# kwea123/nsff_pl

Hardware: AMD Instinct MI355X
Metric: ray-samples/sec (coarse+fine, static+dynamic) (higher is better)
Workload: dtype f16x3 (fp32 operands split into 2 halfs, 3 f16 MFMAs per product, fp32 accumulate; same 1e-4 parity as f32); 1 GPU; C2 (BASELINE.json configs[1]): static+dynamic NSFF, 1024 rays/GPU x (64 coarse + 64 importance -> 192 fine pts), train-mode fwd, fw/bw flow warp t+-1, perturb=1 noise_std=1, 8x256 MLPs, N_tau=48, all 47 outputs on device.  `value` is render_rays' throughput with autograd DISABLED (the train-mode FLAGS, inference launches: nothing kept for a backward pass); what a trainer's forward costs is aux.tra; rays_per_gpu=1024, N_samples=64, N_importance=64, parallelism=single GPU, field_launch=persistent (one workgroup per CU)

## Files before the change

### include/nsff_render.h

```cpp
#ifndef NSFF_RENDER_H
#define NSFF_RENDER_H

#include <stddef.h>
#include <stdint.h>

#ifdef __cplusplus
extern "C" {
#endif

#define NSFF_OK               0
#define NSFF_ERR_INVALID     -1
#define NSFF_ERR_NULL        -2
#define NSFF_ERR_ALIGN       -3
#define NSFF_ERR_HIP         -4

#define NSFF_ABI_VERSION      32
#define NSFF_RAW_STRIDE      16
#define NSFF_MAX_FREQS       24
#define NSFF_MAX_LAYERS       8


typedef struct NsffModelDesc {
    int32_t D;
    int32_t W;
// ... 401 lines not shown
    int32_t col_a, col_b;
    int32_t pad_;
    const float* g_a[4];
    const float* g_b[4];
    float* out;
} NsffFlowGradArgs;
int nsff_flow_grad(const NsffFlowGradArgs* args, void* stream);

#define NSFF_RAY_RECORD      16

typedef struct NsffSsimArgs {
    int32_t n_frames, H, W, window;
    const float* gt;  const float* pred;  const uint8_t* mask;
    float* map;  float* mean_map;  double* sums;
    void* scratch;  int64_t scratch_bytes;
} NsffSsimArgs;
int64_t nsff_ssim_scratch_bytes(int32_t n_frames, int32_t H, int32_t W);
int nsff_ssim(const NsffSsimArgs* args, void* stream);

typedef struct NsffFrameFinishArgs {
    int32_t n_frames, H, W, pad_;
    const float* rgb;  const float* gt;  const uint8_t* valid;  const float* depth;  const uint8_t* lut;
    float* rgb_clipped;  uint8_t* rgb_u8;  double* sums;  float* depth_range;  uint8_t* depth_u8;  uint8_t* depth_rgb_u8;
    void* scratch;  int64_t scratch_bytes;
} NsffFrameFinishArgs;
int64_t nsff_frame_finish_scratch_bytes(int32_t n_frames, int32_t H, int32_t W);
int nsff_frame_finish(const NsffFrameFinishArgs* args, void* stream);

typedef struct NsffValPanelsArgs {
    int32_t n_frames, H, W, pad_;
    const float* gt;  const float* pred;  const float* depth;  const float* transient_alpha;  const float* static_rgb;
    const float* static_depth;  const float* mask;  const float* disp;  const float* ssim_loss;
    const uint8_t* lut_depth;  const uint8_t* lut_mask;
    float* ranges;  uint8_t* grid_u8;  uint8_t* rmse_u8;  uint8_t* ssim_u8;  uint8_t* rmse_blend_u8;  uint8_t* ssim_blend_u8;
    void* scratch;  int64_t scratch_bytes;
} NsffValPanelsArgs;
int64_t nsff_val_panels_scratch_bytes(int32_t n_frames, int32_t H, int32_t W);
int nsff_val_panels(const NsffValPanelsArgs* args, void* stream);

#define NSFF_FLOW_UNKNOWN    1e10f
typedef struct NsffFlowMapsArgs {
    int32_t n_frames, H, W, n_poses, max_t, share_gt_scale;
    float   fx, fy, cx, cy;
    const float* xyz[2];  const float* Ps;  const int32_t* ts;
    float* flow[2];  const float* gt[2];  const uint8_t* mask;
    double* epe_sums;  int64_t* epe_counts;  float* maxrad;  const float* scale;
    uint8_t* image[2];  uint8_t* gt_image[2];
    void* scratch;  int64_t scratch_bytes;
} NsffFlowMapsArgs;
int64_t nsff_flow_maps_scratch_bytes(int32_t n_frames, int32_t H, int32_t W);
int nsff_flow_maps(const NsffFlowMapsArgs* args, void* stream);

#define NSFF_TRACK_MAX_POINTS 0x7fffffffLL
typedef struct NsffTrackStepArgs {
    int64_t n_rows;
    int32_t pts_per_row, direction, max_t, n_poses, fixed_view, pad_;
    float   fx, fy, cx, cy;
    const float* raw;  const float* xyz_in;  const int32_t* t_in;  const uint8_t* alive_in;
    float* xyz_out;  int32_t* t_out;  uint8_t* alive_out;
    const float* Ps;  float* uv;  float* depth;
} NsffTrackStepArgs;
int nsff_track_step(const NsffTrackStepArgs* args, void* stream);

#define NSFF_TRACK_MAX_TRACKS (1 << 20)
#define NSFF_TRACK_MAX_STEPS  (1 << 11)
typedef struct NsffTrackDrawArgs {
    int32_t H, W, n_steps, n_tracks;
    const float* uv;  const uint8_t* ok;  const uint8_t* image;  const uint8_t* lut;  uint8_t* out;
    void* scratch;  int64_t scratch_bytes;
} NsffTrackDrawArgs;
int64_t nsff_track_draw_scratch_bytes(int32_t H, int32_t W);
int nsff_track_draw(const NsffTrackDrawArgs* args, void* stream);

int nsff_cdf(const float* weights, int64_t n_frames, int64_t n, double* cdf, void* stream);

typedef struct NsffRayDrawArgs {
    int64_t n_frames, n_pixels, frame, batch;
    const float* records;  const double* cdf;  const float* u;
    float* rays;  float* rgbs;  int64_t* ts;  int64_t* cam_ids;  float* disps;  float* rays_mask;  float* uv_fw;  float* uv_bw;
    int64_t* rand_idx;
} NsffRayDrawArgs;
int nsff_ray_draw(const NsffRayDrawArgs* args, void* stream);

int nsff_prof_enable(int on);
int nsff_prof_collect(int64_t* launches, double* total_ms, double* total_flops, double* executed_flops);
int nsff_prof_collect_clock(int64_t* launches, double* total_ms, double* total_flops, double* executed_flops,
                            double* shader_ticks, double* ticks_ms);

#define NSFF_KERNEL_F32       1
#define NSFF_KERNEL_H3_64     2
#define NSFF_KERNEL_H3_8WAVE  3
#define NSFF_KERNEL_H3A       4
#define NSFF_KERNEL_H3_SAVE   5
#define NSFF_KERNEL_H3A_TBIAS 7
#define NSFF_KERNEL_H3A_SAVE  9
#define NSFF_KERNEL_H3A_SIDE  8
int         nsff_last_field_kernel(void);
int         nsff_last_field_grid(void);
int         nsff_field_mfma_shape(const NsffModelDesc* desc, const NsffFieldArgs* args);
int         nsff_repack_field_weights(const NsffModelDesc* desc, const void* packed, void* repacked, void* stream);
int         nsff_field_query_repacked(const NsffModelDesc* desc, const void* packed, const void* repacked, const NsffFieldArgs* args,
                                      void* stream);
int         nsff_last_field_mfma_shape(void);
int         nsff_field_phase_program(const NsffModelDesc* desc, int static_mode, int transient_mode, int fold_t, uint32_t* steps,
                             int* n_steps, int* n_static_steps, uint32_t* phases_static, uint32_t* phases_dynamic, int* n_phases);

#define NSFF_PLAN_WORDS 12
#define NSFF_LAUNCH_SIDE_TILE      1
#define NSFF_LAUNCH_H3_64          2
#define NSFF_LAUNCH_H3_64_SAVE     3
#define NSFF_LAUNCH_H3_8WAVE       4
#define NSFF_LAUNCH_H3_8WAVE_SAVE  5
#define NSFF_LAUNCH_H3A            6
#define NSFF_LAUNCH_H3A_SAVE       7
int         nsff_field_launch_plan(const NsffModelDesc* desc, const NsffFieldArgs* args, int32_t n_cus, int32_t no_persist,
                                   int32_t* out, int32_t max_launches);

#define NSFF_RANGE_ACT     0x1u
#define NSFF_RANGE_SAVED   0x2u
#define NSFF_RANGE_PARAMS  0x4u
#define NSFF_RANGE_CODES   0x8u
int         nsff_range_flags(uint32_t* out, int32_t clear, void* stream);

#define NSFF_LPIPS_MIN_SIZE  31

typedef struct NsffLpipsWeights {
    const float* conv_w[5];  const float* conv_b[5];  const float* lin[5];
} NsffLpipsWeights;
int64_t nsff_lpips_packed_bytes(void);
int     nsff_lpips_pack(const NsffLpipsWeights* weights, float* packed, void* stream);

int     nsff_lpips_dims(int32_t H, int32_t W, int32_t* hw);

typedef struct NsffLpipsArgs {
    int32_t n_frames, H, W, normalize;
    const float* gt;  const float* pred;  const uint8_t* valid;
    const float* packed;
    float* map;  double* sums;
    void* workspace;  int64_t workspace_bytes;
} NsffLpipsArgs;
int64_t nsff_lpips_workspace_bytes(int32_t n_frames, int32_t H, int32_t W);
int     nsff_lpips(const NsffLpipsArgs* args, void* stream);

typedef struct NsffSceneScaleArgs {
    int32_t n_frames, n_points, H, W;
    int32_t disp_rank[2];
    const double* points;  const uint8_t* vis;  const double* w2c;  const float* K;  const float* disps;
    double* stats;  float* disp_os;  double* depth_os;  int32_t* pix;
    void* work;  int64_t work_bytes;
} NsffSceneScaleArgs;
int64_t nsff_scene_scale_work_bytes(int32_t n_frames, int32_t n_points, int32_t H, int32_t W);
int     nsff_scene_scale(const NsffSceneScaleArgs* args, void* stream);

int         nsff_abi_version(void);
const char* nsff_last_hip_error(void);

#ifdef __cplusplus
}
#endif
#endif
```

### nsff_pl_amd/_lib.py

```python
import ctypes as C
import os

import torch

_HERE = os.path.dirname(os.path.abspath(__file__))
LIB_PATH = os.environ.get("NSFF_LIB") or os.path.join(_HERE, "libnsff_hip.so")

RAW_STRIDE = 16
ABI_VERSION = 32
MAX_FREQS = 24

_ERR = {-1: "NSFF_ERR_INVALID (bad shape/flag/unsupported architecture)",
        -2: "NSFF_ERR_NULL (required pointer missing)",
        -3: "NSFF_ERR_ALIGN (pointer not 16-byte aligned)",
        -4: "NSFF_ERR_HIP",
        -5: "NSFF_ERR_UNSUPPORTED (a valid request outside what the kernels are built for)"}

_fp = C.c_void_p


class ModelDesc(C.Structure):
    _fields_ = [("D", C.c_int32), ("W", C.c_int32), ("skip", C.c_int32),
                ("in_xyz", C.c_int32), ("in_dir", C.c_int32), ("in_a", C.c_int32),
                ("in_t", C.c_int32), ("use_viewdir", C.c_int32),
                ("has_transient", C.c_int32), ("has_flow", C.c_int32),
                ("flow_scale", C.c_float), ("skip_mask", C.c_int32)]


class FieldArgs(C.Structure):
    _fields_ = [("n_points", C.c_int64), ("precision", C.c_int32), ("tile_points", C.c_int32),
                ("pts_per_ray", C.c_int32),
                ("static_mode", C.c_int32), ("transient_mode", C.c_int32),
                ("flow_heads", C.c_int32),
                ("xyz", _fp), ("n_freqs", C.c_int32), ("freqs", C.c_float * MAX_FREQS),
                ("dir_emb", _fp), ("a_emb", _fp), ("t_emb", _fp),
                ("x_emb", _fp), ("ld_emb", C.c_int32),
                ("off_xyz", C.c_int32), ("off_dir", C.c_int32), ("off_a", C.c_int32),
                ("off_t", C.c_int32), ("raw", _fp), ("save_acts", _fp), ("save_xin", _fp), ("save_masks", _fp),
                ("save_side", _fp), ("t_bias", _fp), ("t_bias_rows", C.c_int32), ("reserved0", C.c_int32),
                ("s_bias", _fp), ("s_bias_rows", C.c_int32), ("launch_form", C.c_int32), ("save_lo_delta", C.c_int64 * 3)]


class TimeBiasJob(C.Structure):
    _fields_ = [("desc", C.POINTER(ModelDesc)), ("w", _fp * 8), ("b", _fp * 8), ("t_rows", _fp), ("out", _fp),
                ("table", _fp), ("ts", _fp), ("n_table", C.c_int64), ("max_t", C.c_int64), ("delta", C.c_int32), ("pad_", C.c_int32),
                ("rows_out", _fp)]


MAX_TIME_BIAS_JOBS = 4


class RngJob(C.Structure):
    _fields_ = [("out", _fp), ("numel", C.c_int64), ("offset", C.c_uint64), ("kind", C.c_int32), ("grid", C.c_uint32)]


MAX_RNG_JOBS = 12


class RngCoarse(C.Structure):
    _fields_ = [("rays", _fp), ("z_lin", _fp), ("zs", _fp), ("xyz", _fp), ("n_samples", C.c_int32), ("perturb", C.c_float),
                ("job", C.c_int32), ("pad_", C.c_int32)]


_COMPOSITE_PTRS_IN = ["raw", "raw_fw", "raw_bw", "zs", "xyz", "xyz_fw", "xyz_bw",
                      "noise_static", "noise_transient", "noise_fw", "noise_bw", "visibility"]
_COMPOSITE_PTRS_OUT = ["static_rgbs", "transient_rgbs", "flows_fw", "flows_bw",
                       "static_sigmas", "transient_sigmas", "static_alphas", "transient_alphas",
                       "static_weights", "transient_weights", "weights",
                       "xyzs_fw_bw", "xyzs_bw_fw", "disoccs_fw", "disoccs_bw",
                       "depth", "rgb", "transient_alpha", "transient_rgb",
                       "static_only_rgb", "static_only_depth",
                       "xyz_exp", "flow_fw_exp", "flow_bw_exp", "xyz_fw_exp", "xyz_bw_exp",
                       "rgb_fw", "rgb_bw", "disocc_fw", "disocc_bw"]


class FrustumArgs(C.Structure):
    _fields_ = [("w2c", _fp), ("ts", _fp), ("K4", C.c_float * 4), ("n_cams", C.c_int32), ("n_frames", C.c_int32),
                ("H", C.c_int32), ("W", C.c_int32)]


class CompositeArgs(C.Structure):
    _fields_ = ([("n_rays", C.c_int64), ("n_samples", C.c_int32), ("has_transient", C.c_int32),
                 ("has_rgb", C.c_int32), ("flow_mode", C.c_int32), ("want_disocc", C.c_int32),
                 ("noise_std", C.c_float), ("z_far", C.c_float)]
                + [(n, _fp) for n in _COMPOSITE_PTRS_IN]
                + [(n, _fp) for n in _COMPOSITE_PTRS_OUT]
                + [("vis", FrustumArgs)])


_CBWD_IN = ["raw", "raw_fw", "raw_bw", "zs", "xyz", "f_fw", "f_bw", "noise_static", "noise_transient", "noise_fw", "noise_bw"]
_CBWD_G = ["g_static_sigmas", "g_transient_sigmas", "g_static_weights", "g_transient_weights", "g_weights", "g_depth",
           "g_rgb", "g_transient_alpha", "g_transient_rgb", "g_so_rgb", "g_so_depth", "g_xyz_exp", "g_flow_fw_exp",
           "g_flow_bw_exp", "g_rgb_fw", "g_rgb_bw"]
_CBWD_OUT = ["scratch", "d_raw", "d_raw_fw", "d_raw_bw", "d_f_fw", "d_f_bw"]


class CompositeBwdArgs(C.Structure):
    _fields_ = ([("n_rays", C.c_int64), ("n_samples", C.c_int32), ("has_transient", C.c_int32), ("flow_mode", C.c_int32),
                 ("noise_std", C.c_float)] + [(n, _fp) for n in _CBWD_IN + _CBWD_G + _CBWD_OUT])


class FieldBwdArgs(C.Structure):
    _fields_ = [("n_points", C.c_int64), ("static_mode", C.c_int32), ("transient_mode", C.c_int32),
                ("d_raw", _fp), ("raw", _fp), ("gmax", _fp), ("masks", _fp), ("dpre", _fp), ("dhead", _fp),
                ("d_xin", _fp), ("d_side", _fp), ("dpre_lo_delta", C.c_int64)]


class WgradJob(C.Structure):
    _fields_ = [("a", _fp), ("b", _fp), ("a_rows", C.c_int32), ("b_rows", C.c_int32), ("out_off", C.c_int64), ("trunk", C.c_int32),
                ("pad_", C.c_int32), ("a_lo_delta", C.c_int64), ("b_lo_delta", C.c_int64)]


class FoldGradArgs(C.Structure):
    _fields_ = [("n_rows", C.c_int32), ("pad_", C.c_int32), ("g", _fp), ("gb", _fp), ("w_final", _fp), ("b_final", _fp),
                ("w_head", _fp * 16), ("d_w_head", _fp * 16), ("d_b_head", _fp * 16), ("d_w_final", _fp), ("d_b_final", _fp)]


class FoldDenseArgs(C.Structure):
    _fields_ = [("n_rows", C.c_int32), ("accumulate", C.c_int32), ("ld_head", C.c_int32), ("ld_dhead", C.c_int32),
                ("g", _fp), ("g2", _fp), ("gb", _fp), ("gb2", _fp), ("w_head", _fp), ("w_final", _fp), ("b_final", _fp),
                ("d_w_head", _fp), ("d_b_head", _fp), ("d_w_final", _fp), ("d_b_final", _fp)]


class SplatArgs(C.Structure):
    _fields_ = [("H", C.c_int32), ("W", C.c_int32), ("n_planes", C.c_int32), ("K4", C.c_float * 4),
                ("P", C.c_float * 12), ("scale", C.c_float),
                ("xyz", _fp), ("flow", _fp), ("rgb", _fp), ("alpha", _fp), ("accum", _fp), ("work", _fp),
                ("work_bytes", C.c_int64)]


class MpiArgs(C.Structure):
    _fields_ = [("H", C.c_int32), ("W", C.c_int32), ("n_planes", C.c_int32), ("dt", C.c_float),
                ("accum_fw", _fp), ("accum_bw", _fp), ("static_rgb", _fp), ("static_alpha", _fp), ("zs", _fp),
                ("rgb", _fp), ("depth", _fp)]


_LOSS_IN = ["rgb_fine", "rgb_coarse", "depth_fine", "depth_coarse", "t_weights", "s_weights", "xyz_fw", "xyz_bw", "rgb_fw",
            "rgb_bw", "disocc_fw", "disocc_bw", "disoccs_fw", "disoccs_bw", "xyzs_fw_bw", "xyzs_bw_fw", "xyzs_fine",
            "xyzs_fw", "xyzs_bw", "rgbs", "disps", "ts", "cam_ids", "uv_fw", "uv_bw", "Ks", "Ps", "hyper", "stats", "terms",
            "term_w"]
LOSS_GRADS = ["g_rgb_fine", "g_rgb_coarse", "g_depth_fine", "g_depth_coarse", "g_t_weights", "g_s_weights", "g_xyz_fw",
              "g_xyz_bw", "g_rgb_fw", "g_rgb_bw", "g_xyzs_fw_bw", "g_xyzs_bw_fw", "g_xyzs_fw", "g_xyzs_bw"]


class LossArgs(C.Structure):
    _fields_ = ([("n_rays", C.c_int64), ("n_samples", C.c_int32), ("n_keep", C.c_int32), ("n_frames", C.c_int32),
                 ("max_t", C.c_int32), ("topk", C.c_double), ("thickness", C.c_int32), ("pad_", C.c_int32)]
                + [(n, _fp) for n in _LOSS_IN] + [("weights", _fp), ("per_ray", _fp), ("coef", _fp)]
                + [(n, _fp) for n in LOSS_GRADS])


class FlowGradArgs(C.Structure):
    _fields_ = [("n_points", C.c_int64), ("zs", _fp), ("z_far", C.c_float), ("accumulate", C.c_int32), ("col_a", C.c_int32),
                ("col_b", C.c_int32), ("pad_", C.c_int32), ("g_a", _fp * 4), ("g_b", _fp * 4), ("out", _fp)]


class SsimArgs(C.Structure):
    _fields_ = [("n_frames", C.c_int32), ("H", C.c_int32), ("W", C.c_int32), ("window", C.c_int32),
                ("gt", _fp), ("pred", _fp), ("mask", _fp), ("map", _fp), ("mean_map", _fp), ("sums", _fp),
                ("scratch", _fp), ("scratch_bytes", C.c_int64)]


class LpipsWeights(C.Structure):
    _fields_ = [("conv_w", _fp * 5), ("conv_b", _fp * 5), ("lin", _fp * 5)]


class LpipsArgs(C.Structure):
    _fields_ = [("n_frames", C.c_int32), ("H", C.c_int32), ("W", C.c_int32), ("normalize", C.c_int32),
                ("gt", _fp), ("pred", _fp), ("valid", _fp), ("packed", _fp), ("map", _fp), ("sums", _fp),
                ("workspace", _fp), ("workspace_bytes", C.c_int64)]


_FINISH_PTRS = ["rgb", "gt", "valid", "depth", "lut", "rgb_clipped", "rgb_u8", "sums", "depth_range", "depth_u8", "depth_rgb_u8"]


class FrameFinishArgs(C.Structure):
    _fields_ = ([("n_frames", C.c_int32), ("H", C.c_int32), ("W", C.c_int32), ("pad_", C.c_int32)]
                + [(n, _fp) for n in _FINISH_PTRS] + [("scratch", _fp), ("scratch_bytes", C.c_int64)])


_PANEL_IN = ["gt", "pred", "depth", "transient_alpha", "static_rgb", "static_depth", "mask", "disp", "ssim_loss"]
_PANEL_LUT = ["lut_depth", "lut_mask"]
_PANEL_OUT = ["ranges", "grid_u8", "rmse_u8", "ssim_u8", "rmse_blend_u8", "ssim_blend_u8"]
PANEL_FIELDS = ("depth", "static_depth", "neg_disp", "neg_rmse", "neg_ssim")


class ValPanelsArgs(C.Structure):
    _fields_ = ([("n_frames", C.c_int32), ("H", C.c_int32), ("W", C.c_int32), ("pad_", C.c_int32)]
                + [(n, _fp) for n in _PANEL_IN + _PANEL_LUT + _PANEL_OUT] + [("scratch", _fp), ("scratch_bytes", C.c_int64)])


FLOW_UNKNOWN = 1e10


class FlowMapsArgs(C.Structure):
    _fields_ = [("n_frames", C.c_int32), ("H", C.c_int32), ("W", C.c_int32), ("n_poses", C.c_int32), ("max_t", C.c_int32),
                ("share_gt_scale", C.c_int32), ("fx", C.c_float), ("fy", C.c_float), ("cx", C.c_float), ("cy", C.c_float),
                ("xyz", _fp * 2), ("Ps", _fp), ("ts", _fp), ("flow", _fp * 2), ("gt", _fp * 2), ("mask", _fp),
                ("epe_sums", _fp), ("epe_counts", _fp), ("maxrad", _fp), ("scale", _fp), ("image", _fp * 2), ("gt_image", _fp * 2),
                ("scratch", _fp), ("scratch_bytes", C.c_int64)]


TRACK_MAX_POINTS, TRACK_MAX_TRACKS, TRACK_MAX_STEPS = 0x7fffffff, 1 << 20, 1 << 11


class TrackStepArgs(C.Structure):
    _fields_ = [("n_rows", C.c_int64), ("pts_per_row", C.c_int32), ("direction", C.c_int32), ("max_t", C.c_int32),
                ("n_poses", C.c_int32), ("fixed_view", C.c_int32), ("pad_", C.c_int32),
                ("fx", C.c_float), ("fy", C.c_float), ("cx", C.c_float), ("cy", C.c_float),
                ("raw", _fp), ("xyz_in", _fp), ("t_in", _fp), ("alive_in", _fp), ("xyz_out", _fp), ("t_out", _fp), ("alive_out", _fp),
                ("Ps", _fp), ("uv", _fp), ("depth", _fp)]


class TrackDrawArgs(C.Structure):
    _fields_ = [("H", C.c_int32), ("W", C.c_int32), ("n_steps", C.c_int32), ("n_tracks", C.c_int32),
                ("uv", _fp), ("ok", _fp), ("image", _fp), ("lut", _fp), ("out", _fp), ("scratch", _fp), ("scratch_bytes", C.c_int64)]


RAY_RECORD = 16
_DRAW_OUT = ["rays", "rgbs", "ts", "cam_ids", "disps", "rays_mask", "uv_fw", "uv_bw", "rand_idx"]


class RayDrawArgs(C.Structure):
    _fields_ = ([("n_frames", C.c_int64), ("n_pixels", C.c_int64), ("frame", C.c_int64), ("batch", C.c_int64),
                 ("records", _fp), ("cdf", _fp), ("u", _fp)] + [(n, _fp) for n in _DRAW_OUT])


FRAME_TABLE = 16


class RayRecordArgs(C.Structure):
    _fields_ = [("n_frames", C.c_int32), ("H", C.c_int32), ("W", C.c_int32), ("first_frame", C.c_int32),
                ("frame_count", C.c_int32), ("image_u8", C.c_int32), ("mask_u8", C.c_int32),
                ("fx", C.c_float), ("fy", C.c_float), ("cx", C.c_float), ("cy", C.c_float), ("near", C.c_float),
                ("n_pixels", C.c_int64), ("images", _fp), ("disps", _fp), ("masks", _fp), ("flow_fw", _fp), ("flow_bw", _fp),
                ("frame_table", _fp), ("records", _fp)]


RESIZE_LANCZOS_U8, RESIZE_NEAREST_PIL, RESIZE_NEAREST_CV, RESIZE_LINEAR_CV = range(4)
RESIZE_MAX_KSIZE = 49
ERR_UNSUPPORTED = -5


class FrameResizeArgs(C.Structure):
    _fields_ = [("n_frames", C.c_int32), ("filter", C.c_int32), ("channels", C.c_int32), ("pad_", C.c_int32),
                ("src_h", C.c_int32), ("src_w", C.c_int32), ("dst_h", C.c_int32), ("dst_w", C.c_int32),
                ("ksize_x", C.c_int32), ("ksize_y", C.c_int32), ("ratio", C.c_float * 2), ("src", _fp), ("dst", _fp),
                ("x_start", _fp), ("x_count", _fp), ("x_weights", _fp), ("y_start", _fp), ("y_count", _fp), ("y_weights", _fp)]


class SceneScaleArgs(C.Structure):
    _fields_ = [("n_frames", C.c_int32), ("n_points", C.c_int32), ("H", C.c_int32), ("W", C.c_int32),
                ("disp_rank", C.c_int32 * 2), ("points", _fp), ("vis", _fp), ("w2c", _fp), ("K", _fp), ("disps", _fp),
                ("stats", _fp), ("disp_os", _fp), ("depth_os", _fp), ("pix", _fp), ("work", _fp), ("work_bytes", C.c_int64)]


_SIGNATURES = {
    "nsff_abi_version": (C.c_int, []),
    "nsff_range_flags": (C.c_int, [_fp, C.c_int32, _fp]),
    "nsff_last_field_kernel": (C.c_int, []),
    "nsff_last_field_grid": (C.c_int, []),
    "nsff_field_mfma_shape": (C.c_int, [C.POINTER(ModelDesc), C.POINTER(FieldArgs)]),
    "nsff_repack_field_weights": (C.c_int, [C.POINTER(ModelDesc), _fp, _fp, _fp]),
    "nsff_field_query_repacked": (C.c_int, [C.POINTER(ModelDesc), _fp, _fp, C.POINTER(FieldArgs), _fp]),
    "nsff_last_field_mfma_shape": (C.c_int, []),
    "nsff_field_phase_program": (C.c_int, [C.POINTER(ModelDesc), C.c_int, C.c_int, C.c_int, C.POINTER(C.c_uint32), C.POINTER(C.c_int),
                                   C.POINTER(C.c_int), C.POINTER(C.c_uint32), C.POINTER(C.c_uint32), C.POINTER(C.c_int)]),
    "nsff_field_launch_plan": (C.c_int, [C.POINTER(ModelDesc), C.POINTER(FieldArgs), C.c_int32, C.c_int32, C.POINTER(C.c_int32), C.c_int32]),
    "nsff_time_bias_rows": (C.c_int, [C.POINTER(ModelDesc)]),
    "nsff_time_bias": (C.c_int, [C.POINTER(TimeBiasJob), C.c_int32, C.c_int64, C.c_void_p]),
    "nsff_rng_draws": (C.c_int, [C.POINTER(RngJob), C.c_int32, C.c_uint64, C.c_void_p]),
    "nsff_rng_draws_coarse": (C.c_int, [C.POINTER(RngJob), C.c_int32, C.c_uint64, C.POINTER(RngCoarse), C.c_void_p]),
    "nsff_side_bias": (C.c_int, [C.POINTER(ModelDesc), _fp, _fp, _fp, _fp, C.c_int64, _fp, C.c_void_p]),
    "nsff_last_hip_error": (C.c_char_p, []),
    "nsff_packed_bytes": (C.c_int, [C.POINTER(ModelDesc), C.c_int, C.POINTER(C.c_size_t)]),
    "nsff_param_count": (C.c_int, [C.POINTER(ModelDesc)]),
    "nsff_pack_weights": (C.c_int, [C.POINTER(ModelDesc), C.c_int, C.POINTER(_fp), _fp, _fp]),
    "nsff_pack_weights_ex": (C.c_int, [C.POINTER(ModelDesc), C.c_int, C.POINTER(_fp), _fp, C.c_int32, _fp]),
    "nsff_fold_heads": (C.c_int, [C.POINTER(ModelDesc), C.c_int, C.POINTER(_fp), _fp, _fp]),
    "nsff_posenc": (C.c_int, [_fp, C.c_int64, C.POINTER(C.c_float), C.c_int, _fp, _fp]),
    "nsff_time_rows": (C.c_int, [_fp, C.c_int64, C.c_int32, _fp, C.c_int64, C.c_int64, _fp, _fp, _fp]),
    "nsff_time_rows_backward": (C.c_int, [_fp, _fp, _fp, _fp, C.c_int64, C.c_int64, C.c_int64, C.c_int32, _fp, _fp]),
    "nsff_field_query": (C.c_int, [C.POINTER(ModelDesc), _fp, C.POINTER(FieldArgs), _fp]),
    "nsff_coarse_samples": (C.c_int, [_fp, C.c_int64, _fp, C.c_int32, C.c_float, _fp, _fp, _fp, _fp]),
    "nsff_fine_samples": (C.c_int, [_fp, C.c_int64, _fp, _fp, C.c_int32, C.c_int32, _fp, _fp, _fp, _fp,
                                    C.c_int32, _fp, _fp, _fp, _fp, _fp]),
    "nsff_sample_pdf": (C.c_int, [_fp, _fp, C.c_int64, C.c_int32, _fp, C.c_int32, C.c_int32,
                                  C.c_float, _fp, _fp]),
    "nsff_warp_points": (C.c_int, [_fp, _fp, _fp, C.c_int64, C.c_float, _fp, _fp, _fp]),
    "nsff_composite": (C.c_int, [C.POINTER(CompositeArgs), _fp]),
    "nsff_frustum_visibility": (C.c_int, [C.POINTER(FrustumArgs), _fp, C.c_int64, _fp, _fp]),
    "nsff_frame_rays": (C.c_int, [C.POINTER(C.c_float), C.POINTER(C.c_float), C.c_int32, C.c_int32, C.c_float,
                                  C.c_float, C.c_int64, C.c_int64, _fp, _fp]),
    "nsff_ray_records": (C.c_int, [C.POINTER(RayRecordArgs), _fp]),
    "nsff_resize_ksize": (C.c_int, [C.c_int32, C.c_int32, C.c_int32]),
    "nsff_resize_table": (C.c_int, [C.c_int32, C.c_int32, C.c_int32, C.c_void_p, C.c_void_p, C.c_void_p]),
    "nsff_frame_resize": (C.c_int, [C.POINTER(FrameResizeArgs), _fp]),
    "nsff_scene_scale_work_bytes": (C.c_int64, [C.c_int32, C.c_int32, C.c_int32, C.c_int32]),
    "nsff_scene_scale": (C.c_int, [C.POINTER(SceneScaleArgs), _fp]),
    "nsff_bwd_packed_bytes": (C.c_int, [C.POINTER(ModelDesc), C.POINTER(C.c_size_t)]),
    "nsff_pack_weights_bwd": (C.c_int, [C.POINTER(ModelDesc), C.POINTER(_fp), _fp, _fp]),
    "nsff_field_backward": (C.c_int, [C.POINTER(ModelDesc), _fp, C.POINTER(FieldBwdArgs), _fp]),
    "nsff_field_input_backward": (C.c_int, [_fp, C.c_int32, C.c_int32, _fp, C.c_int64, C.c_int32, C.POINTER(C.c_float), C.c_int32,
                                            C.c_int32, _fp, _fp, _fp]),
    "nsff_train_dims": (C.c_int, [C.POINTER(ModelDesc), C.POINTER(C.c_int32), C.POINTER(C.c_int32), C.POINTER(C.c_int32)]),
    "nsff_weight_grad_scratch": (C.c_int64, [C.POINTER(WgradJob), C.c_int32, C.c_int64, C.c_int32]),
    "nsff_weight_grad": (C.c_int, [C.POINTER(WgradJob), C.c_int32, C.c_int64, C.c_int32, _fp, _fp, _fp, _fp, _fp]),
    "nsff_weight_grad_accumulate": (C.c_int, [C.POINTER(WgradJob), C.c_int32, C.c_int64, C.c_int32, _fp, _fp, C.c_int64,
                                              _fp, _fp, _fp]),
    "nsff_weight_grad_accumulate_aux": (C.c_int, [C.POINTER(WgradJob), C.c_int32, C.c_int64, C.c_int32, _fp, _fp, C.c_int64,
                                                  _fp, _fp, _fp, _fp]),
    "nsff_absmax_raw": (C.c_int, [_fp, C.c_int64, _fp, _fp]),
    "nsff_last_bwd_kernel": (C.c_int, []),
    "nsff_last_bwd_grid": (C.c_int, []),
    "nsff_field_bwd_phase_program": (C.c_int, [C.POINTER(ModelDesc), C.c_int32, C.c_int32, C.c_int64, C.POINTER(C.c_uint32), C.c_int32,
                                                C.POINTER(C.c_uint32), C.c_int32]),
    "nsff_field_bwd_launch_plan": (C.c_int, [C.POINTER(ModelDesc), C.POINTER(FieldBwdArgs), C.c_int32, C.c_int32, C.c_int32,
                                             C.POINTER(C.c_int32), C.c_int32]),
    "nsff_fold_grads": (C.c_int, [C.POINTER(FoldGradArgs), _fp]),
    "nsff_fold_grads_dense": (C.c_int, [C.POINTER(FoldDenseArgs), _fp]),
    "nsff_pack_weights_bwd_ex": (C.c_int, [C.POINTER(ModelDesc), C.POINTER(_fp), _fp, _fp, _fp]),
    "nsff_absmax": (C.c_int, [_fp, C.c_int64, _fp, _fp]),
    "nsff_adam_step": (C.c_int, [_fp, _fp, _fp, _fp, C.c_int64, _fp, _fp, C.c_double, C.c_double, C.c_double, C.c_double, _fp]),
    "nsff_adam_step_segments": (C.c_int, [_fp, _fp, _fp, _fp, C.c_int64, _fp, _fp, C.c_double, C.c_double, C.c_double, C.c_double,
                                          _fp, C.c_int, _fp, _fp]),
    "nsff_sgd_step": (C.c_int, [_fp, _fp, _fp, C.c_int64, _fp, _fp, C.c_double, C.c_double, _fp, C.c_int, _fp, _fp]),
    "nsff_radam_step": (C.c_int, [_fp, _fp, _fp, _fp, C.c_int64, _fp, _fp, C.c_double, C.c_double, C.c_double, C.c_double,
                                  _fp, C.c_int, _fp, _fp]),
    "nsff_composite_backward": (C.c_int, [C.POINTER(CompositeBwdArgs), _fp]),
    "nsff_flow_grad": (C.c_int, [C.POINTER(FlowGradArgs), _fp]),
    "nsff_nerfw_loss": (C.c_int, [C.POINTER(LossArgs), C.c_int, _fp]),
    "nsff_nerfw_loss_work_bytes": (C.c_size_t, [C.c_longlong]),
    "nsff_nerfw_loss_ex": (C.c_int, [C.POINTER(LossArgs), C.c_int, _fp, C.c_size_t, _fp]),
    "nsff_last_loss_path": (C.c_int, []),
    "nsff_splat_planes": (C.c_int, [C.POINTER(SplatArgs), _fp]),
    "nsff_splat_work_bytes": (C.c_int64, [C.c_int32, C.c_int32, C.c_int32]),
    "nsff_mpi_composite": (C.c_int, [C.POINTER(MpiArgs), _fp]),
    "nsff_ssim_scratch_bytes": (C.c_int64, [C.c_int32, C.c_int32, C.c_int32]),
    "nsff_ssim": (C.c_int, [C.POINTER(SsimArgs), _fp]),
    "nsff_lpips_packed_bytes": (C.c_int64, []),
    "nsff_lpips_pack": (C.c_int, [C.POINTER(LpipsWeights), _fp, _fp]),
    "nsff_lpips_dims": (C.c_int, [C.c_int32, C.c_int32, C.POINTER(C.c_int32)]),
    "nsff_lpips_workspace_bytes": (C.c_int64, [C.c_int32, C.c_int32, C.c_int32]),
    "nsff_lpips": (C.c_int, [C.POINTER(LpipsArgs), _fp]),
    "nsff_frame_finish_scratch_bytes": (C.c_int64, [C.c_int32, C.c_int32, C.c_int32]),
    "nsff_frame_finish": (C.c_int, [C.POINTER(FrameFinishArgs), _fp]),
    "nsff_val_panels_scratch_bytes": (C.c_int64, [C.c_int32, C.c_int32, C.c_int32]),
    "nsff_val_panels": (C.c_int, [C.POINTER(ValPanelsArgs), _fp]),
    "nsff_flow_maps_scratch_bytes": (C.c_int64, [C.c_int32, C.c_int32, C.c_int32]),
    "nsff_flow_maps": (C.c_int, [C.POINTER(FlowMapsArgs), _fp]),
    "nsff_track_step": (C.c_int, [C.POINTER(TrackStepArgs), _fp]),
    "nsff_track_draw_scratch_bytes": (C.c_int64, [C.c_int32, C.c_int32]),
    "nsff_track_draw": (C.c_int, [C.POINTER(TrackDrawArgs), _fp]),
    "nsff_cdf": (C.c_int, [_fp, C.c_int64, C.c_int64, _fp, _fp]),
    "nsff_ray_draw": (C.c_int, [C.POINTER(RayDrawArgs), _fp]),
    "nsff_prof_enable": (C.c_int, [C.c_int]),
    "nsff_prof_collect": (C.c_int, [C.POINTER(C.c_int64), C.POINTER(C.c_double), C.POINTER(C.c_double), C.POINTER(C.c_double)]),
    "nsff_prof_collect_clock": (C.c_int, [C.POINTER(C.c_int64)] + [C.POINTER(C.c_double)] * 5),
}
EXPORTED_SYMBOLS = tuple(_SIGNATURES)

_lib = None


def load():
    global _lib
    if _lib is None:
        if not os.path.exists(LIB_PATH):
            raise RuntimeError(
                f"{LIB_PATH} is missing: build it with `python -c 'import __graft_entry__ as g; g.build()'` "
                "(or `make -C nsff_pl_amd/csrc`).  There is no CPU fallback for the render path.")
        lib = C.CDLL(LIB_PATH)
        for name, (res, args) in _SIGNATURES.items():
            fn = getattr(lib, name)
            fn.restype, fn.argtypes = res, args
        if lib.nsff_abi_version() != ABI_VERSION:
            raise RuntimeError("libnsff_hip.so ABI version mismatch")
        _lib = lib
    return _lib


def _check(rc, what):
    if rc != 0:
        msg = _ERR.get(rc, f"error {rc}")
        if rc == -4:
            msg += ": " + load().nsff_last_hip_error().decode()
        raise RuntimeError(f"{what} failed: {msg}")


def require_gpu_tensor(t, what):
    if not isinstance(t, torch.Tensor) or not t.is_cuda:
        raise RuntimeError(f"{what} must be a GPU tensor: the NSFF render path runs only on the "
                           "HIP kernels of libnsff_hip.so (no CPU fallback)")


def _ptr(t):
    if t is None:
        return None
    assert t.is_cuda and t.dtype == torch.float32 and t.is_contiguous(), "need contiguous fp32 GPU tensor"
    return t.data_ptr()


def _stream():
    return torch.cuda.current_stream().cuda_stream


def model_desc(model):
    if model.W != 256:
        raise RuntimeError(f"unsupported NeRF architecture: W={model.W} (the gfx950 field kernels tile W=256 trunks "
                           "into 4 x 64-neuron wave blocks; other widths are not built)")
    skips = sorted(set(int(s) for s in model.skips))
    if not 2 <= model.D <= 8 or any(not 1 <= s < model.D for s in skips):
        raise RuntimeError(f"unsupported NeRF architecture: D={model.D}, skips={list(model.skips)} (need 2 <= D <= 8 "
                           "and every skip layer in 1..D-1; a skip at layer 0 would concatenate the input with itself)")
    mask = sum(1 << s for s in skips)
    return ModelDesc(D=model.D, W=model.W, skip=skips[0] if len(skips) == 1 else 0, skip_mask=mask if len(skips) != 1 else 0,
                     in_xyz=model.in_channels_xyz,
                     in_dir=model.in_channels_dir,
                     in_a=model.in_channels_a if model.use_viewdir else 0,
                     in_t=model.in_channels_t, use_viewdir=int(model.use_viewdir),
                     has_transient=int(model.encode_transient),
                     has_flow=int(getattr(model, "has_flow_heads", hasattr(model, "transient_flow_fw"))),
                     flow_scale=float(getattr(model, "flow_scale", 0.0)))


def param_list(model):
    def lin(m):
        layer = m[0] if isinstance(m, torch.nn.Sequential) else m
        return [layer.weight, layer.bias]
    out = []
    for i in range(model.D):
        out += lin(getattr(model, f"static_xyz_encoding_{i + 1}"))
    out += lin(model.static_xyz_encoding_final)
    if model.use_viewdir:
        out += lin(model.static_dir_encoding)
    out += lin(model.static_sigma) + lin(model.static_rgb)
    if model.encode_transient:
        for i in range(model.D):
            out += lin(getattr(model, f"transient_xyz_encoding_{i + 1}"))
        out += lin(model.transient_xyz_encoding_final)
        out += lin(model.transient_sigma) + lin(model.transient_rgb)
        if hasattr(model, "transient_flow_fw"):
            out += lin(model.transient_flow_fw) + lin(model.transient_flow_bw)
    return out


def packed_bytes(desc, precision=0):
    n = C.c_size_t(0)
    _check(load().nsff_packed_bytes(C.byref(desc), int(precision), C.byref(n)), "nsff_packed_bytes")
    return n.value


PACK_SKIP_FOLD = 1


def pack_weights(desc, params, packed, precision=0, fold=True):
    lib = load()
    if lib.nsff_param_count(C.byref(desc)) != len(params):
        raise RuntimeError("parameter list does not match the model description")
    keep = [p.detach().contiguous().float() for p in params]
    for p in keep:
        require_gpu_tensor(p, "model parameter")
    arr = (_fp * len(keep))(*[p.data_ptr() for p in keep])
    _check(lib.nsff_pack_weights_ex(C.byref(desc), int(precision), arr, _ptr(packed), 0 if fold else PACK_SKIP_FOLD,
                                    _stream()), "nsff_pack_weights_ex")
    return keep


def fold_heads(desc, params, packed, precision):
    keep = [p.detach().contiguous().float() for p in params]
    arr = (_fp * len(keep))(*[p.data_ptr() for p in keep])
    _check(load().nsff_fold_heads(C.byref(desc), int(precision), arr, _ptr(packed), _stream()), "nsff_fold_heads")
    return keep


def time_rows_backward(g_cur, g_next, g_prev, ts, max_t, n_table):
    gs = [None if g is None else g.contiguous() for g in (g_cur, g_next, g_prev)]
    width = next(g for g in gs if g is not None).shape[1]
    assert ts.dtype == torch.int64 and ts.is_cuda and ts.is_contiguous()
    d = torch.empty(int(n_table), width, device=ts.device)
    _check(load().nsff_time_rows_backward(_ptr(gs[0]), _ptr(gs[1]), _ptr(gs[2]), C.c_void_p(ts.data_ptr()), ts.shape[0],
                                          int(max_t), int(n_table), width, _ptr(d), _stream()), "nsff_time_rows_backward")
    return d


def time_rows(table, ts, max_t, want_next=True, want_prev=True):
    n, width = ts.shape[0], table.shape[1]
    if want_next and want_prev:
        both = torch.empty(2, n, width, device=table.device)
        nxt, prv = both[0], both[1]
    else:
        nxt = torch.empty(n, width, device=table.device) if want_next else None
        prv = torch.empty(n, width, device=table.device) if want_prev else None
    assert ts.dtype == torch.int64 and ts.is_cuda and ts.is_contiguous()
    _check(load().nsff_time_rows(_ptr(table), table.shape[0], width, C.c_void_p(ts.data_ptr()), n, int(max_t),
                                 _ptr(nxt), _ptr(prv), _stream()), "nsff_time_rows")
    return nxt, prv


def posenc(x, freqs, out):
    f = [float(v) for v in freqs]
    arr = (C.c_float * len(f))(*f)
    _check(load().nsff_posenc(_ptr(x), x.shape[0], arr, len(f), _ptr(out), _stream()), "nsff_posenc")


def field_query(model, raw, n_points, pts_per_ray, static_mode, transient_mode, flow_heads=0,
                xyz=None, freqs=None, dir_emb=None, a_emb=None, t_emb=None,
                x_emb=None, emb_offsets=(0, -1, -1, -1), save_acts=None, save_xin=None, save_masks=None, save_side=None,
                precision=None, t_bias=None, s_bias=None, save_lo=False):
    from . import config
    desc = model_desc(model)
    prec = config.precision_code(model) if precision is None else precision
    saves = not (save_acts is None and save_xin is None and save_masks is None and save_side is None)
    packed = model.packed(prec)
    a = FieldArgs()
    a.precision, a.tile_points = prec, config.get_tile_points()
    a.launch_form = 0 if config.get_persistent() else 1
    a.n_points, a.pts_per_ray = int(n_points), int(pts_per_ray)
    a.static_mode, a.transient_mode, a.flow_heads = int(static_mode), int(transient_mode), int(flow_heads)
    a.xyz = _ptr(xyz)
    if freqs is not None:
        f = [float(v) for v in freqs]
        if len(f) > MAX_FREQS:
            raise RuntimeError("too many embedding frequencies")
        a.n_freqs = len(f)
        for i, v in enumerate(f):
            a.freqs[i] = v
    a.dir_emb, a.a_emb, a.t_emb = _ptr(dir_emb), _ptr(a_emb), _ptr(t_emb)
    a.x_emb = _ptr(x_emb)
    a.ld_emb = int(x_emb.shape[1]) if x_emb is not None else 0
    a.off_xyz, a.off_dir, a.off_a, a.off_t = [int(v) for v in emb_offsets]
    a.raw = _ptr(raw)
    a.save_acts = None if save_acts is None else save_acts.data_ptr()
    a.save_xin = None if save_xin is None else save_xin.data_ptr()
    a.save_masks = None if save_masks is None else save_masks.data_ptr()
    a.save_side = None if save_side is None else save_side.data_ptr()
    if save_lo:
        for i, t in enumerate((save_acts, save_xin, save_side)):
            a.save_lo_delta[i] = 0 if t is None else lo_delta(t)
    if t_bias is not None:
        a.t_bias, a.t_bias_rows = _ptr(t_bias), int(t_bias.shape[1])
    if s_bias is not None:
        a.s_bias, a.s_bias_rows = _ptr(s_bias), int(s_bias.shape[1])
    if os.environ.get("NSFF_H3A_SHAPE") != "32" and prec == config.PRECISIONS["f16x3"] and not saves and \
            load().nsff_field_mfma_shape(C.byref(desc), C.byref(a)) == 16:
        _check(load().nsff_field_query_repacked(C.byref(desc), _ptr(packed), _ptr(model.packed(REPACKED)), C.byref(a), _stream()),
               "nsff_field_query_repacked")
        return
    _check(load().nsff_field_query(C.byref(desc), _ptr(packed), C.byref(a), _stream()), "nsff_field_query")


def lo_delta(t):
    n = t.numel()
    if t.untyped_storage().nbytes() < (t.storage_offset() + 2 * n) * t.element_size():
        raise RuntimeError("three-product backward: this buffer has no remainder plane behind it (field_grad.alloc_saves(..., x3=True))")
    return n


def side_bias(model, dir_rows, a_rows=None):
    from . import config
    desc = model_desc(model)
    n_rays = int(dir_rows.shape[0])
    assert dir_rows.shape == (n_rays, desc.in_dir) and (desc.in_a == 0 or (a_rows is not None and a_rows.shape == (n_rays, desc.in_a)))
    packed = model.packed(config.PRECISIONS["f16x3"])
    w = model.static_dir_encoding[0].weight.detach()
    out = torch.empty(n_rays, 1, 256, device=dir_rows.device, dtype=torch.float32)
    _check(load().nsff_side_bias(C.byref(desc), _ptr(packed), _ptr(w), _ptr(dir_rows), _ptr(a_rows) if desc.in_a > 0 else None,
                                 n_rays, _ptr(out), _stream()), "nsff_side_bias")
    return out


_DEVICE_RNG_GEOMETRY = {}


def fused_draws(plan, device, values=True, coarse=None):
    dev = torch.device(device)
    idx = dev.index if dev.index is not None else torch.cuda.current_device()
    if idx not in _DEVICE_RNG_GEOMETRY:
        p = torch.cuda.get_device_properties(idx)
        _DEVICE_RNG_GEOMETRY[idx] = p.multi_processor_count * (p.max_threads_per_multi_processor // 256)
    max_grid = _DEVICE_RNG_GEOMETRY[idx]
    gen = torch.cuda.default_generators[idx]
    seed, offset = gen.initial_seed(), gen.get_offset()
    wanted = values if isinstance(values, (list, tuple)) else [bool(values)] * len(plan)
    sizes = []
    for kind, shape in plan:
        n = 1
        for s in shape:
            n *= int(s)
        sizes.append(n)
    total = sum(n for n, w in zip(sizes, wanted) if w)
    buf = torch.empty(max(total, 1), device=dev, dtype=torch.float32)
    outs, jobs, at = [], [], 0
    for (kind, shape), numel, want in zip(plan, sizes, wanted):
        if numel == 0:
            outs.append(torch.empty(*shape, device=dev, dtype=torch.float32))
            continue
        grid = min(max_grid, (numel + 255) // 256)
        if coarse is not None and not outs and not want:
            jobs.append((None, numel, offset, 0, grid))
            outs.append(None)
        elif want:
            t = buf[at:at + numel].view(*shape)
            at += numel
            jobs.append((t, numel, offset, 1 if kind == "randn" else 0, grid))
            outs.append(t)
        else:
            outs.append(None)
        offset += ((numel - 1) // (1024 * grid) + 1) * 4
    hook = None
    if coarse is not None:
        rays, z_lin, perturb, zs, xyz = coarse
        assert plan and plan[0][0] == "rand" and tuple(plan[0][1]) == (rays.shape[0], z_lin.shape[0]) and perturb > 0
        if sizes[0]:
            hook = RngCoarse(_ptr(rays), _ptr(z_lin), _ptr(zs), _ptr(xyz), int(z_lin.shape[0]), float(perturb), 0, 0)
    for k in range(0, len(jobs), MAX_RNG_JOBS):
        part = jobs[k:k + MAX_RNG_JOBS]
        arr = (RngJob * len(part))()
        for j, (t, numel, off, kind, grid) in enumerate(part):
            arr[j].out, arr[j].numel, arr[j].offset, arr[j].kind, arr[j].grid = (None if t is None else t.data_ptr()), numel, off, kind, grid
        with torch.cuda.device(idx):
            _check(load().nsff_rng_draws_coarse(arr, len(part), seed, C.byref(hook) if (hook is not None and k == 0) else None, _stream()),
                   "nsff_rng_draws")
    gen.set_offset(offset)
    return outs


_FUSED_DRAWS_OK = {}


def fused_draws_match_torch(device):
    dev = torch.device(device)
    idx = dev.index if dev.index is not None else torch.cuda.current_device()
    if idx in _FUSED_DRAWS_OK:
        return _FUSED_DRAWS_OK[idx]
    if torch.cuda.is_current_stream_capturing():
        return False
    gen = torch.cuda.default_generators[idx]
    state = gen.get_state()
    ok = True
    try:
        plan = [("rand", (7, 64)), ("randn", (1031,)), ("rand", (3, 5, 2)), ("randn", (70000,)), ("rand", (300001,))]
        gen.manual_seed(0x5EED1234)
        gen.set_offset(8)
        mine = fused_draws(plan, torch.device("cuda", idx))
        end_mine = gen.get_offset()
        gen.manual_seed(0x5EED1234)
        gen.set_offset(8)
        with torch.cuda.device(idx):
            ref = [(torch.rand if k == "rand" else torch.randn)(*shape, device=torch.device("cuda", idx)) for k, shape in plan]
        end_ref = gen.get_offset()
        ok = end_mine == end_ref and all(torch.equal(a.view(torch.int32), b.view(torch.int32)) for a, b in zip(mine, ref))
    except Exception:
        ok = False
    finally:
        gen.set_state(state)
    if not ok:
        import warnings
        warnings.warn("nsff_pl_amd: the fused generator kernel (nsff_rng_draws) no longer reproduces torch.rand / torch.randn on "
                      f"cuda:{idx} (torch {torch.__version__}); render_rays draws with the torch calls instead (slower by ~1 %, same "
                      "numbers as the reference)")
    _FUSED_DRAWS_OK[idx] = ok
    return ok


def time_bias_rows(model):
    return load().nsff_time_bias_rows(C.byref(model_desc(model)))


def time_bias(jobs, index=None):
    assert 1 <= len(jobs) <= MAX_TIME_BIAS_JOBS
    arr = (TimeBiasJob * len(jobs))()
    keep, outs, per_model, pair = [], [], {}, None
    rows_of = {}
    if index is not None:
        table, ts, max_t = index
        assert ts.dtype == torch.int64 and ts.is_cuda and ts.is_contiguous() and ts.dim() == 1, "ts: one int64 frame index per ray"
        n_rays, width = int(ts.shape[0]), int(table.shape[1])
        deltas = sorted({int(d) for _, d in jobs})
        if 1 in deltas and -1 in deltas:
            both = torch.empty(2, n_rays, width, device=table.device, dtype=torch.float32)
            rows_of[1], rows_of[-1] = both[0], both[1]
        for d in deltas:
            if d not in rows_of:
                rows_of[d] = torch.empty(n_rays, width, device=table.device, dtype=torch.float32)
        written = set()
    else:
        n_rays = int(jobs[0][1].shape[0])
    for j, (model, t_rows) in enumerate(jobs):
        if id(model) not in per_model:
            desc = model_desc(model)
            lins = [getattr(model, f"transient_xyz_encoding_{l + 1}")[0] for l in [0] + sorted(set(int(v) for v in model.skips))]
            wb = [(m.weight.detach(), m.bias.detach()) for m in lins]
            for w, b in wb:
                _ptr(w), _ptr(b)
            per_model[id(model)] = (desc, C.pointer(desc), wb)
        desc, pdesc, wb = per_model[id(model)]
        if index is not None:
            delta, t_rows = int(t_rows), None
            assert width == desc.in_t
        else:
            assert t_rows.shape == (n_rays, desc.in_t)
        dev = wb[0][0].device
        if j + 1 < len(jobs) and jobs[j + 1][0] is model and pair is None:
            pair = torch.empty(2, n_rays, len(wb), 256, device=dev, dtype=torch.float32)
            out = pair[0]
        elif pair is not None:
            out, pair = pair[1], None
        else:
            out = torch.empty(n_rays, len(wb), 256, device=dev, dtype=torch.float32)
        arr[j].desc = pdesc
        for i, (w, b) in enumerate(wb):
            arr[j].w[i], arr[j].b[i] = w.data_ptr(), b.data_ptr()
        arr[j].t_rows, arr[j].out = _ptr(t_rows), _ptr(out)
        if index is not None:
            arr[j].table, arr[j].ts = _ptr(table), ts.data_ptr()
            arr[j].n_table, arr[j].max_t, arr[j].delta = int(table.shape[0]), int(max_t), delta
            if delta not in written:
                arr[j].rows_out = _ptr(rows_of[delta])
                written.add(delta)
        outs.append(out)
    keep.append(per_model)
    _check(load().nsff_time_bias(arr, len(jobs), n_rays, _stream()), "nsff_time_bias")
    return outs if index is None else (outs, rows_of)


def coarse_samples(rays, z_lin, perturb, perturb_rand, zs, xyz):
    _check(load().nsff_coarse_samples(_ptr(rays), rays.shape[0], _ptr(z_lin), z_lin.shape[0],
                                      float(perturb), _ptr(perturb_rand), _ptr(zs), _ptr(xyz), _stream()),
           "nsff_coarse_samples")


def fine_samples(rays, z_lin, zs_coarse, n_importance, w_static, w_transient, u_static, u_transient,
                 u_per_ray, samples_static, samples_transient, zs_fine, xyz_fine):
    _check(load().nsff_fine_samples(_ptr(rays), rays.shape[0], _ptr(z_lin), _ptr(zs_coarse),
                                    z_lin.shape[0], int(n_importance), _ptr(w_static), _ptr(w_transient),
                                    _ptr(u_static), _ptr(u_transient), int(u_per_ray),
                                    _ptr(samples_static), _ptr(samples_transient),
                                    _ptr(zs_fine), _ptr(xyz_fine), _stream()), "nsff_fine_samples")


def sample_pdf(bins, weights, u, u_per_ray, eps, samples):
    _check(load().nsff_sample_pdf(_ptr(bins), _ptr(weights), weights.shape[0], weights.shape[1],
                                  _ptr(u), samples.shape[1], int(u_per_ray), float(eps),
                                  _ptr(samples), _stream()), "nsff_sample_pdf")


def warp_points(raw, xyz, zs, z_far, xyz_fw, xyz_bw):
    _check(load().nsff_warp_points(_ptr(raw), _ptr(xyz), _ptr(zs), zs.numel(), float(z_far),
                                   _ptr(xyz_fw), _ptr(xyz_bw), _stream()), "nsff_warp_points")


def frustum_args(w2c, ts, K4, n_cams, n_frames, H, W):
    assert w2c.is_cuda and w2c.dtype == torch.float32 and w2c.is_contiguous() and w2c.shape == (n_cams * n_frames, 12)
    assert ts.is_cuda and ts.dtype == torch.int64 and ts.is_contiguous() and ts.numel() >= 1
    a = FrustumArgs(w2c=w2c.data_ptr(), ts=ts.data_ptr(), n_cams=int(n_cams), n_frames=int(n_frames), H=int(H), W=int(W))
    a.K4[:] = [float(v) for v in K4]
    a._keep = (w2c, ts)
    return a


def frustum_visibility(vis, xyz, out):
    _check(load().nsff_frustum_visibility(C.byref(vis), _ptr(xyz), xyz.shape[0], _ptr(out), _stream()),
           "nsff_frustum_visibility")


def composite(vis=None, **kw):
    a = CompositeArgs()
    for k, v in kw.items():
        if k in _COMPOSITE_PTRS_IN or k in _COMPOSITE_PTRS_OUT:
            setattr(a, k, _ptr(v))
        else:
            setattr(a, k, v)
    if vis is not None:
        a.vis = vis
    _check(load().nsff_composite(C.byref(a), _stream()), "nsff_composite")


def frame_rays(K4, c2w12, H, W, near, shift_near, first, count, rays):
    k = (C.c_float * 4)(*[float(v) for v in K4])
    m = (C.c_float * 12)(*[float(v) for v in c2w12])
    _check(load().nsff_frame_rays(k, m, int(H), int(W), float(near), float(shift_near), int(first), int(count),
                                  _ptr(rays), _stream()), "nsff_frame_rays")


REPACKED = 101


def repack_weights(desc, packed, repacked):
    _check(load().nsff_repack_field_weights(C.byref(desc), _ptr(packed), _ptr(repacked), _stream()), "nsff_repack_field_weights")


def last_field_mfma_shape():
    return int(load().nsff_last_field_mfma_shape())


BWD_PACK = 100


def bwd_packed_bytes(desc):
    n = C.c_size_t(0)
    _check(load().nsff_bwd_packed_bytes(C.byref(desc), C.byref(n)), "nsff_bwd_packed_bytes")
    return n.value


def pack_weights_bwd(desc, params, packed, fwd_packed=None):
    arr = (_fp * len(params))(*[p.data_ptr() for p in params])
    _check(load().nsff_pack_weights_bwd_ex(C.byref(desc), arr, _ptr(packed), _ptr(fwd_packed), _stream()), "nsff_pack_weights_bwd_ex")


def last_bwd_kernel():
    return {0: "c", 1: "h3b", 2: "c+h3b", 3: "x3"}[load().nsff_last_bwd_kernel()]


def last_bwd_grid():
    return load().nsff_last_bwd_grid()


PLAN_WORDS = 12


def field_launch_plan(desc, args, n_cus, no_persist=False):
    out = (C.c_int32 * (3 * PLAN_WORDS))()
    code = load().nsff_field_launch_plan(C.byref(desc), C.byref(args), int(n_cus), int(bool(no_persist)), out, 3)
    recs = [list(out[i * PLAN_WORDS:(i + 1) * PLAN_WORDS]) for i in range(3)]
    return code, [r for r in recs if r[0] != 0]


def field_bwd_launch_plan(desc, args, n_cus, kernel_override=None, persist=True):
    out = (C.c_int32 * (2 * PLAN_WORDS))()
    code = load().nsff_field_bwd_launch_plan(C.byref(desc), C.byref(args), int(n_cus), ord(kernel_override) if kernel_override else 0,
                                                      int(bool(persist)), out, 2)
    recs = [list(out[i * PLAN_WORDS:(i + 1) * PLAN_WORDS]) for i in range(2)]
    return code, [r for r in recs if r[0] != 0]


def field_bwd_phase_program(model, dynamic, want_xin, n_tiles, max_phases=32):
    import numpy as np
    desc = model_desc(model)
    out = (C.c_uint32 * (8 * max_phases))()
    segs = (C.c_uint32 * 48)()
    n = load().nsff_field_bwd_phase_program(C.byref(desc), 1 if dynamic else 0, 1 if want_xin else 0, int(n_tiles), out, max_phases, segs, 48)
    if n < 0:
        raise RuntimeError(f"nsff_field_bwd_phase_program failed ({n})")
    offs = np.array(list(segs), np.uint32)
    return (np.array(list(out), np.uint32).reshape(max_phases, 8)[:n] if n > 0 else None), offs


def field_backward(model, n_points, static, transient, d_raw, raw, gmax, masks, dpre, dhead, d_xin, d_side=None, x3=False):
    desc = model_desc(model)
    a = FieldBwdArgs(n_points=int(n_points), static_mode=2 if static else 0, transient_mode=2 if transient else 0,
                     d_raw=_ptr(d_raw), raw=_ptr(raw), gmax=_ptr(gmax), masks=masks.data_ptr(), dpre=dpre.data_ptr(),
                     dhead=dhead.data_ptr(), d_xin=_ptr(d_xin), d_side=_ptr(d_side), dpre_lo_delta=lo_delta(dpre) if x3 else 0)
    _check(load().nsff_field_backward(C.byref(desc), _ptr(model.packed(BWD_PACK)), C.byref(a), _stream()),
           "nsff_field_backward")


def train_dims(model):
    desc = model_desc(model)
    xr, t0, sr = C.c_int32(0), C.c_int32(0), C.c_int32(0)
    _check(load().nsff_train_dims(C.byref(desc), C.byref(xr), C.byref(t0), C.byref(sr)), "nsff_train_dims")
    return xr.value, t0.value, sr.value


def field_input_backward(d_xin, t_row0, xyz, pts_per_ray, freqs, in_t, want_xyz, want_t):
    P, xin_rows = d_xin.shape
    n_rays = P // pts_per_ray
    d_xyz = torch.empty(P, 3, device=d_xin.device) if want_xyz else None
    d_t = torch.empty(n_rays, in_t, device=d_xin.device) if want_t else None
    f = [float(v) for v in freqs]
    arr = (C.c_float * max(len(f), 1))(*f)
    _check(load().nsff_field_input_backward(_ptr(d_xin), int(xin_rows), int(t_row0), _ptr(xyz), n_rays, int(pts_per_ray), arr,
                                            len(f), int(in_t), _ptr(d_xyz), _ptr(d_t), _stream()), "nsff_field_input_backward")
    return d_xyz, d_t


def _wgrad_jobs(jobs, with_off):
# ... 569 lines not shown
```

### nsff_pl_amd/csrc/field_h3.hip

```cpp
#include <hip/hip_runtime.h>
#include <algorithm>
#include <cstdlib>
#include <vector>
#include "nsff_layout_h3.h"
#include "nsff_common.h"
#include "nsff_internal.h"

typedef float f32x16 __attribute__((ext_vector_type(16)));
typedef _Float16 h8 __attribute__((ext_vector_type(8)));
typedef _Float16 h4 __attribute__((ext_vector_type(4)));
typedef __fp16 h2 __attribute__((ext_vector_type(2)));
typedef _Float16 h2f __attribute__((ext_vector_type(2)));

#ifdef H3_TIMING
__device__ unsigned g_h3_timing[256 * 8 * 32 * 6 + 256 * 4 * 256];
#define H3A_TBASE (256 * 8 * 32 * 6)
__device__ unsigned long long g_h3_span[2] = {~0ull, 0ull};
#define H3_SPAN(k) do { if (lane == 0) { const unsigned long long t_ = __builtin_amdgcn_s_memtime(); \
    if (k) atomicMax(&g_h3_span[1], t_); else atomicMin(&g_h3_span[0], t_); } } while (0)
#define H3_STAMP(k) do { if (lane == 0 && blockIdx.x < 256 && i < 32) \
    g_h3_timing[((blockIdx.x * 8 + wave_id) * 32 + i) * 6 + (k)] = (unsigned)__builtin_amdgcn_s_memtime(); } while (0)
#define H3_HSTAMP(k) do { if (lane == 0 && blockIdx.x < 256) \
    g_h3_timing[((blockIdx.x * 8 + wave) * 32 + 30) * 6 + (k)] = (unsigned)__builtin_amdgcn_s_memtime(); } while (0)
#else
#define H3_STAMP(k) do {} while (0)
#define H3_SPAN(k) do {} while (0)
#define H3_HSTAMP(k) do {} while (0)
#endif

namespace {

#ifndef H3_SAVE_INTERLEAVE
#define H3_SAVE_INTERLEAVE 1
#endif
constexpr int LDH = 264;
__device__ __forceinline__ h8 lds_h8(const _Float16* p) { return *reinterpret_cast<const h8*>(p); }

struct H3Step {
    uint32_t w_off;
    uint32_t bias_off;
    uint16_t nks;
    uint8_t pre;
    uint8_t post;
    uint8_t head;
    uint8_t save;
    uint8_t pad[2];
};
enum { PRE_NONE = 0, PRE_INPUT = 1, PRE_INPUT_T = 2, PRE_SIDE = 3 };
enum { POST_NONE = 0, POST_RELU = 1, POST_LINEAR = 2 };
enum { HEAD_NONE = 0, HEAD_S_SIGMA = 1, HEAD_S_RGB = 2, HEAD_T = 3, HEAD_S_FOLD = 4, HEAD_T_FOLD = 5 };
constexpr int MAX_STEPS = 28;

struct H3KArgs {
    NsffLayoutH3 L;
    H3Step steps[MAX_STEPS];
    int n_steps;
    int n_static_steps;
    int split_trunks;
    long long grid_tiles;
    const uint32_t* packed;
    const float* xyz;
    const float* x_emb;
    const float* dir_emb;
    const float* a_emb;
    const float* t_emb;
    const float* t_bias;
    int tb_rows;
    const float* s_bias;
    int sb_rows;
    float* raw;
    long long lo_delta[3];
    _Float16* save_acts;
    _Float16* save_xin;
    unsigned long long* save_masks;
    _Float16* save_side;
    long long save_stride;
    int xin_rows, side_rows;
    long long n_tiles;
    long long n_points;
    int pts_per_ray;
    int static_mode, transient_mode;
    int D, skip;
    int in_xyz, in_dir, in_a, in_t;
    int use_viewdir;
    float flow_scale;
    int n_freqs;
    int octave_freqs;
    float freqs[NSFF_MAX_FREQS];
    int ld_emb, off_xyz, off_dir, off_a, off_t;
    unsigned long long* span;
    uint32_t* range;
};

struct SpanT { unsigned long long t, r; };
__device__ __forceinline__ SpanT span_begin(const unsigned long long* span) {
    SpanT s{0ull, 0ull};
#ifdef H3_TIMING
    s.t = __builtin_amdgcn_s_memtime();
#endif
    if (span != nullptr && (blockIdx.x & 15) == 0) { s.t = __builtin_amdgcn_s_memtime(); s.r = __builtin_amdgcn_s_memrealtime(); }
    return s;
}
__device__ __forceinline__ void span_end(unsigned long long* span, const SpanT& s0, unsigned tid) {
    if (span == nullptr || (blockIdx.x & 15) != 0 || tid != 0) return;
    const unsigned long long t = __builtin_amdgcn_s_memtime(), r = __builtin_amdgcn_s_memrealtime();
    atomicAdd(span, t - s0.t);
    atomicAdd(span + 1, r - s0.r);
}
__device__ __forceinline__ void span_end(unsigned long long* span, const SpanT& s0) { span_end(span, s0, threadIdx.x); }

#define MFMA_H(a, b, c) __builtin_amdgcn_mfma_f32_32x32x16_f16((a), (b), (c), 0, 0, 0)
#define H3_PIN() __builtin_amdgcn_sched_barrier(0)

__device__ __forceinline__ void split_store(_Float16* xh, _Float16* xl, int idx, float v, float& rm) {
    rm = nsff_absmax3(rm, v, v);
    const _Float16 hi = (_Float16)v;
    xh[idx] = hi;
    xl[idx] = (_Float16)(v - (float)hi);
}

template <int MTW> struct WFrag { h8 wh[MTW], wl[MTW]; };
template <int NT> struct XFrag { h8 xh[NT], xl[NT]; };
template <int MTW> struct WRing { WFrag<MTW> r[4]; };
template <int MTW> struct BiasRegs { float4 b[MTW][4]; };

template <int MTW>
__device__ __forceinline__ void load_w(WFrag<MTW>& f, const uint4* __restrict__& wp) {
    if constexpr (MTW == 2) {
        const uint4 a0 = wp[0], a1 = wp[64], a2 = wp[128], a3 = wp[192];
        wp += 256;
        f.wh[0] = __builtin_bit_cast(h8, a0); f.wl[0] = __builtin_bit_cast(h8, a1);
        f.wh[1] = __builtin_bit_cast(h8, a2); f.wl[1] = __builtin_bit_cast(h8, a3);
    } else {
        const uint4 a0 = wp[0], a1 = wp[64];
        wp += 256;
        f.wh[0] = __builtin_bit_cast(h8, a0); f.wl[0] = __builtin_bit_cast(h8, a1);
    }
}

template <int NT> struct BRows { const _Float16* h[NT]; const _Float16* l[NT]; };
template <int NT>
__device__ __forceinline__ BRows<NT> b_rows(const _Float16* bh, const _Float16* bl, int ld) {
    BRows<NT> b;
#pragma unroll
    for (int nt = 0; nt < NT; ++nt) { b.h[nt] = bh + nt * 32 * ld; b.l[nt] = bl + nt * 32 * ld; }
    return b;
}

template <int NT>
__device__ __forceinline__ void load_x(XFrag<NT>& f, const BRows<NT>& b, int ks) {
#pragma unroll
    for (int nt = 0; nt < NT; ++nt) {
        f.xh[nt] = lds_h8(b.h[nt] + ks * 16);
        f.xl[nt] = lds_h8(b.l[nt] + ks * 16);
    }
}

template <int MTW>
__device__ __forceinline__ const uint4* prefetch_w(WRing<MTW>& ring, const uint4* __restrict__ w) {
// ... 1538 lines not shown
            for (int i = 0; i < 2; ++i) {
                if (off[i] == NSFF_NONE) continue;
                if (nks[i] > REPACK_MAX_NKS || (nks[i] & 1)) { bad = true; continue; }
                ra.off[n] = off[i]; ra.nks[n] = nks[i];
                if (++n == REPACK_BATCH) flush();
            }
        }
    };
    trunk(L.st);
    if (desc->has_transient) trunk(L.tr);
    flush();
    return bad ? NSFF_ERR_INVALID : nsff_launch_status();
}

static int fold_args(const NsffModelDesc& d, const float* const* params, FoldArgs& fs, FoldArgs& ft, FoldArgs& fd) {
    int pi = 2 * d.D;
    fs = FoldArgs{}; ft = FoldArgs{}; fd = FoldArgs{};
    fs.ld_head = ft.ld_head = NSFF_W;
    fs.w_final = params[pi]; fs.b_final = params[pi + 1]; pi += 2;
    if (d.use_viewdir) {
        fd.w_final = fs.w_final; fd.b_final = fs.b_final; fd.plain_row = -1;
        fd.w_head[0] = params[pi]; fd.b_head[0] = params[pi + 1]; fd.row0[0] = 0; fd.nrows[0] = NSFF_W; fd.n_heads = 1;
        fd.ld_head = NSFF_W + d.in_dir + d.in_a;
        pi += 2;
    }
    fs.w_plain = params[pi]; fs.b_plain = params[pi + 1]; fs.plain_row = 3; pi += 2;
    fs.w_head[0] = params[pi]; fs.b_head[0] = params[pi + 1]; fs.row0[0] = 0; fs.nrows[0] = 3; fs.n_heads = 1; pi += 2;
    if (d.has_transient) {
        pi += 2 * d.D;
        ft.w_final = params[pi]; ft.b_final = params[pi + 1]; ft.plain_row = -1; pi += 2;
        ft.w_head[1] = params[pi]; ft.b_head[1] = params[pi + 1]; ft.row0[1] = 3; ft.nrows[1] = 1; pi += 2;
        ft.w_head[0] = params[pi]; ft.b_head[0] = params[pi + 1]; ft.row0[0] = 0; ft.nrows[0] = 3; pi += 2;
        ft.n_heads = 2;
        if (d.has_flow) {
            ft.w_head[2] = params[pi]; ft.b_head[2] = params[pi + 1]; ft.row0[2] = 4; ft.nrows[2] = 3; pi += 2;
            ft.w_head[3] = params[pi]; ft.b_head[3] = params[pi + 1]; ft.row0[3] = 7; ft.nrows[3] = 3; pi += 2;
            ft.n_heads = 4;
        }
    }
    return pi;
}

int nsff_fold_rows_f32(const NsffModelDesc* desc, const float* const* params, float* s_w, float* s_b, float* t_w, float* t_b,
                       hipStream_t st) {
    const NsffModelDesc& d = *desc;
    FoldArgs fs, ft, fd;
    const int pi = fold_args(d, params, fs, ft, fd);
    for (int i = 0; i < pi; ++i) if (!params[i]) return NSFF_ERR_NULL;
    if (!d.use_viewdir) {
        fs.out_w = s_w; fs.out_b = s_b;
        hipLaunchKernelGGL(nsff_fold_kernel_h3, dim3(4), dim3(256), 0, st, fs);
    }
    if (d.has_transient) {
        ft.out_w = t_w; ft.out_b = t_b;
        hipLaunchKernelGGL(nsff_fold_kernel_h3, dim3(d.has_flow ? 10 : 4), dim3(256), 0, st, ft);
    }
    return nsff_launch_status();
}

int nsff_h3_fold_heads(const NsffModelDesc* desc, const float* const* params, void* packed, hipStream_t st) {
    NsffLayoutH3 L;
    const int rc = nsff_make_layout_h3(*desc, L);
    if (rc) return rc;
    const NsffModelDesc& d = *desc;
    FoldArgs fs, ft, fd;
    const int pi = fold_args(d, params, fs, ft, fd);
    for (int i = 0; i < pi; ++i) if (!params[i]) return NSFF_ERR_NULL;
    uint32_t* pw = reinterpret_cast<uint32_t*>(packed);
    PackArgsH3 pf{};
    pf.dst = pw;
    pf.range = nsff_range_word(st);
    int nf = 0;
    auto fold = [&](FoldArgs& f, uint32_t scratch, uint32_t tile, uint32_t bias) {
        f.out_w = reinterpret_cast<float*>(pw + scratch); f.out_b = reinterpret_cast<float*>(pw + bias);
        hipLaunchKernelGGL(nsff_fold_kernel_h3, dim3(32), dim3(256), 0, st, f);
        pf.seg[nf++] = PackSegH3{f.out_w, tile, 2, NSFF_W, NSFF_W, 0, 0, 0, 0, 0, 0, 32};
    };
    if (!d.use_viewdir) fold(fs, L.fold_f32, L.s_fold_w, L.s_fold_b);
    if (d.has_transient) fold(ft, L.fold_f32 + 32 * NSFF_W, L.t_fold_w, L.t_fold_b);
    int max_threads = 8 * NSFF_W;
    if (d.use_viewdir) {
        fd.out_w = reinterpret_cast<float*>(pw + L.dir_fold_f32); fd.out_b = reinterpret_cast<float*>(pw + L.dir_b_fold);
        hipLaunchKernelGGL(nsff_fold_kernel_h3, dim3(NSFF_W), dim3(256), 0, st, fd);
        pf.seg[nf++] = PackSegH3{fd.out_w, L.dir_h_fold, 1, NSFF_W, NSFF_W, NSFF_W, 0, 0, 0, 0, 0, 0};
        max_threads = 64 * NSFF_W;
    }
    if (nf > 0) hipLaunchKernelGGL(nsff_pack_kernel_h3, dim3((max_threads + 255) / 256, nf), dim3(256), 0, st, pf);
    return nsff_launch_status();
}

static int h3_step_program(const NsffModelDesc& d, int static_mode, int transient_mode, bool fold, H3KArgs& k, bool side_fold = false) {
    int n = 0;
    auto push = [&](uint32_t w, uint32_t b, uint32_t kcols, int pre, int post, int head, int slot = -1) {
        H3Step& s = k.steps[n++];
        s.w_off = w; s.bias_off = b; s.nks = (uint16_t)(kcols / 16);
        s.pre = (uint8_t)pre; s.post = (uint8_t)post; s.head = (uint8_t)head;
        s.save = (uint8_t)(slot + 1);
    };
    auto trunk = [&](const NsffTrunkLayoutH3& T, int pre_kind, int last_head, int slot0) {
        for (int l = 0; l < d.D; ++l) {
            const int head = (l == d.D - 1) ? last_head : HEAD_NONE;
            if (l == 0) {
                push(T.seg_x[0], T.bias[0], T.k0, pre_kind, POST_RELU, HEAD_NONE, slot0);
            } else if ((nsff_skip_layers(&d) >> l) & 1u) {
                push(T.seg_h[l], T.bias[l], NSFF_W, PRE_NONE, POST_NONE, HEAD_NONE);
                push(T.seg_x[l], NSFF_NONE, T.k0, pre_kind, POST_RELU, head, slot0 + l);
            } else {
                push(T.seg_h[l], T.bias[l], NSFF_W, PRE_NONE, POST_RELU, head, slot0 + l);
            }
        }
    };
    if (static_mode == 2 && fold && !d.use_viewdir) {
        trunk(k.L.st, PRE_INPUT, HEAD_S_FOLD, 0);
    } else if (static_mode == 2 && fold && side_fold) {
        trunk(k.L.st, PRE_INPUT, HEAD_S_SIGMA, 0);
        push(k.L.dir_h_fold, k.L.dir_b_fold, NSFF_W, PRE_NONE, POST_RELU, HEAD_S_RGB, d.D);
    } else if (static_mode == 2 && fold) {
        trunk(k.L.st, PRE_INPUT, HEAD_S_SIGMA, 0);
        push(k.L.dir_h_fold, k.L.dir_b_fold, NSFF_W, PRE_NONE, POST_NONE, HEAD_NONE);
        push(k.L.dir_x, NSFF_NONE, k.L.side_k, PRE_SIDE, POST_RELU, HEAD_S_RGB, d.D);
    } else if (static_mode) {
        trunk(k.L.st, PRE_INPUT, HEAD_S_SIGMA, 0);
        if (static_mode == 2) {
            push(k.L.st.final_w, k.L.st.final_b, NSFF_W, PRE_NONE, POST_LINEAR, d.use_viewdir ? HEAD_NONE : HEAD_S_RGB, d.D);
            if (d.use_viewdir) {
                push(k.L.dir_h, k.L.dir_b, NSFF_W, PRE_NONE, POST_NONE, HEAD_NONE);
                push(k.L.dir_x, NSFF_NONE, k.L.side_k, PRE_SIDE, POST_RELU, HEAD_S_RGB, d.D);
            }
        }
    }
    k.n_static_steps = n;
    if (transient_mode && fold) {
        trunk(k.L.tr, PRE_INPUT_T, HEAD_T_FOLD, d.D + 1);
    } else if (transient_mode) {
        trunk(k.L.tr, PRE_INPUT_T, HEAD_NONE, d.D + 1);
        push(k.L.tr.final_w, k.L.tr.final_b, NSFF_W, PRE_NONE, POST_LINEAR, HEAD_T, 2 * d.D + 1);
    }
    if (n > MAX_STEPS) return NSFF_ERR_INVALID;
    k.n_steps = n;
    return NSFF_OK;
}

static bool h3a_make_persistent(H3APhase* ph) {
    int at = -1;
    for (int i = 1; i < H3A_MAX_PHASES && !(i > 1 && ph[i].d[0] == H3A_BODY_END); ++i)
        if (ph[i].d[0] == H3A_BODY_B16L) { if (at >= 0) return false; at = i; }
    if (at < 0) return false;
    ph[at].d[0] = H3A_BODY_B16LP;
    for (int j = 3; j < 8; ++j) ph[at].d[j] = ph[0].d[j];
    return true;
}

namespace {
struct TimeBiasJobK { const float* w[NSFF_MAX_LAYERS]; const float* b[NSFF_MAX_LAYERS]; int ld[NSFF_MAX_LAYERS];
                      const float* t_rows; float* out; int rows, in_xyz, in_t;
                      const float* table; const long long* ts; long long n_table, max_t; int delta; float* rows_out; };
struct TimeBiasArgs { TimeBiasJobK job[NSFF_MAX_TIME_BIAS_JOBS]; long long n_rays; };
constexpr int TB_RAYS = 16;
__global__ __launch_bounds__(256) void nsff_time_bias_kernel(const TimeBiasArgs a) {
    const TimeBiasJobK& j = a.job[blockIdx.z];
    const int i = blockIdx.y, n = threadIdx.x;
    if (i >= j.rows) return;
    const long long r0 = (long long)blockIdx.x * TB_RAYS;
    __shared__ __attribute__((aligned(16))) float st[TB_RAYS][64];
    __shared__ float sw[16][NSFF_W + 1];
    const float* __restrict__ wl = j.w[i] + j.in_xyz;
    const int ld = j.ld[i], in_t = j.in_t;
    float tv[TB_RAYS / 4], wv[4][16];
#pragma unroll
    for (int k = 0; k < TB_RAYS / 4; ++k) {
        const int e = threadIdx.x + 256 * k, r = e >> 6, c = e & 63;
        const long long ray = r0 + r < a.n_rays ? r0 + r : a.n_rays - 1;
        const float* row = j.t_rows != nullptr ? j.t_rows + ray * in_t : nullptr;
        if (row == nullptr) {
            long long t = j.ts[ray] + j.delta;
            if (j.delta > 0) t = t < j.max_t ? t : j.max_t;
            if (j.delta < 0) t = t > 0 ? t : 0;
            t = t < 0 ? 0 : (t > j.n_table - 1 ? j.n_table - 1 : t);
            row = j.table + t * in_t;
        }
        tv[k] = c < in_t ? row[c] : 0.f;
        if (j.rows_out != nullptr && i == 0 && c < in_t && r0 + r < a.n_rays) j.rows_out[(r0 + r) * in_t + c] = tv[k];
    }
    const float b = j.b[i][n];
#pragma unroll
    for (int q = 0; q < 4; ++q)
#pragma unroll
        for (int k = 0; k < 16; ++k) {
            const int e = threadIdx.x + 256 * k, row = e >> 4, c = 16 * q + (e & 15);
            wv[q][k] = c < in_t ? wl[row * ld + c] : 0.f;
        }
#pragma unroll
    for (int k = 0; k < TB_RAYS / 4; ++k) { const int e = threadIdx.x + 256 * k; st[e >> 6][e & 63] = tv[k]; }
    float acc[TB_RAYS];
#pragma unroll
    for (int r = 0; r < TB_RAYS; ++r) acc[r] = b;
#pragma unroll
    for (int q = 0; q < 4; ++q) {
        if (16 * q >= in_t) break;
        __syncthreads();
#pragma unroll
        for (int k = 0; k < 16; ++k) { const int e = threadIdx.x + 256 * k; sw[e & 15][e >> 4] = wv[q][k]; }
        __syncthreads();
#pragma unroll
        for (int u = 0; u < 16; u += 4) {
            const float w0 = sw[u][n], w1 = sw[u + 1][n], w2 = sw[u + 2][n], w3 = sw[u + 3][n];
#pragma unroll
            for (int r = 0; r < TB_RAYS; ++r) {
                const float4 t4 = *reinterpret_cast<const float4*>(&st[r][16 * q + u]);
                acc[r] = fmaf(w3, t4.w, fmaf(w2, t4.z, fmaf(w1, t4.y, fmaf(w0, t4.x, acc[r]))));
            }
        }
    }
#pragma unroll
    for (int r = 0; r < TB_RAYS; ++r)
        if (r0 + r < a.n_rays) j.out[((r0 + r) * j.rows + i) * NSFF_W + n] = acc[r];
}
}

extern "C" int nsff_time_bias_rows(const NsffModelDesc* desc) {
    if (!desc || !desc->has_transient || desc->in_t < 1) return 0;
    return 1 + __builtin_popcount(nsff_skip_layers(desc));
}

extern "C" int nsff_time_bias(const NsffTimeBiasJob* jobs, int32_t n_jobs, int64_t n_rays, void* stream) {
    if (!jobs) return NSFF_ERR_NULL;
    if (n_jobs < 1 || n_jobs > NSFF_MAX_TIME_BIAS_JOBS || n_rays < 0) return NSFF_ERR_INVALID;
    if (n_rays == 0) return NSFF_OK;
    TimeBiasArgs a{};
    a.n_rays = n_rays;
    int max_rows = 0;
    for (int q = 0; q < n_jobs; ++q) {
        const NsffTimeBiasJob& jb = jobs[q];
        if (!jb.desc || !jb.out) return NSFF_ERR_NULL;
        if (!jb.t_rows && (!jb.table || !jb.ts || jb.n_table < 1 || jb.delta < -1 || jb.delta > 1)) return NSFF_ERR_NULL;
        const NsffModelDesc& d = *jb.desc;
        NsffLayoutH3 L;
        const int rc = nsff_make_layout_h3(d, L);
        if (rc) return rc;
        TimeBiasJobK& k = a.job[q];
        k.rows = nsff_time_bias_rows(&d);
        if (k.rows < 1) return NSFF_ERR_INVALID;
        if (d.in_t > 64 || (d.in_t & 3) != 0) return NSFF_ERR_INVALID;
        k.in_xyz = d.in_xyz; k.in_t = d.in_t; k.t_rows = jb.t_rows; k.out = jb.out;
        k.table = jb.table; k.ts = reinterpret_cast<const long long*>(jb.ts); k.n_table = jb.n_table; k.max_t = jb.max_t;
        k.delta = jb.delta; k.rows_out = jb.t_rows ? nullptr : jb.rows_out;
        const uint32_t skips = nsff_skip_layers(&d);
        int i = 0;
        for (int l = 0; l < d.D; ++l) {
            if (l != 0 && !((skips >> l) & 1u)) continue;
            k.w[i] = jb.w[i]; k.b[i] = jb.b[i];
            if (!k.w[i] || !k.b[i]) return NSFF_ERR_NULL;
            k.ld[i] = d.in_xyz + d.in_t + (l ? NSFF_W : 0);
            ++i;
        }
        max_rows = std::max(max_rows, k.rows);
    }
    const long long gx = (n_rays + TB_RAYS - 1) / TB_RAYS;
    if (gx > 0x7fffffffLL) return NSFF_ERR_INVALID;
    hipLaunchKernelGGL(nsff_time_bias_kernel, dim3((unsigned)gx, (unsigned)max_rows, (unsigned)n_jobs), dim3(256), 0,
                       reinterpret_cast<hipStream_t>(stream), a);
    return nsff_launch_status();
}

namespace {
struct SideBiasArgs { const float* w; const float* b; const float* dir_rows; const float* a_rows; float* out;
                      int in_dir, in_a, ld; long long n_rays; };
__global__ __launch_bounds__(256) void nsff_side_bias_kernel(const SideBiasArgs a) {
    const int n = threadIdx.x;
    const long long r0 = (long long)blockIdx.x * TB_RAYS;
    const int in = a.in_dir + a.in_a;
    __shared__ __attribute__((aligned(16))) float st[TB_RAYS][NSFF_W];
    __shared__ float sw[16][NSFF_W + 1];
    for (int e = threadIdx.x; e < TB_RAYS * NSFF_W; e += 256) {
        const int r = e >> 8, c = e & 255;
        const long long ray = r0 + r < a.n_rays ? r0 + r : a.n_rays - 1;
        float v = 0.f;
        if (c < a.in_dir) v = a.dir_rows[ray * a.in_dir + c];
        else if (c < in) v = a.a_rows[ray * a.in_a + (c - a.in_dir)];
        st[r][c] = v;
    }
    float acc[TB_RAYS];
    const float b = a.b[n];
#pragma unroll
    for (int r = 0; r < TB_RAYS; ++r) acc[r] = b;
    const float* __restrict__ wl = a.w + NSFF_W;
    for (int c0 = 0; c0 < in; c0 += 16) {
        __syncthreads();
#pragma unroll
        for (int k = 0; k < 16; ++k) {
            const int e = threadIdx.x + 256 * k, row = e >> 4, c = c0 + (e & 15);
            sw[e & 15][row] = c < in ? wl[(long long)row * a.ld + c] : 0.f;
        }
        __syncthreads();
#pragma unroll
        for (int u = 0; u < 16; u += 4) {
            const float w0 = sw[u][n], w1 = sw[u + 1][n], w2 = sw[u + 2][n], w3 = sw[u + 3][n];
#pragma unroll
            for (int r = 0; r < TB_RAYS; ++r) {
                const float4 t4 = *reinterpret_cast<const float4*>(&st[r][c0 + u]);
                acc[r] = fmaf(w3, t4.w, fmaf(w2, t4.z, fmaf(w1, t4.y, fmaf(w0, t4.x, acc[r]))));
            }
        }
    }
#pragma unroll
    for (int r = 0; r < TB_RAYS; ++r)
        if (r0 + r < a.n_rays) a.out[(r0 + r) * NSFF_W + n] = acc[r];
}
}

extern "C" int nsff_side_bias(const NsffModelDesc* desc, const void* packed_f16x3, const float* w_dir, const float* dir_rows,
                              const float* a_rows, int64_t n_rays, float* out, void* stream) {
    if (!desc || !packed_f16x3 || !w_dir || !dir_rows || !out) return NSFF_ERR_NULL;
    const NsffModelDesc& d = *desc;
    NsffLayoutH3 L;
    const int rc = nsff_make_layout_h3(d, L);
    if (rc) return rc;
    if (!d.use_viewdir || d.in_dir < 1 || n_rays < 0) return NSFF_ERR_INVALID;
    if (d.in_a > 0 && !a_rows) return NSFF_ERR_NULL;
    if (n_rays == 0) return NSFF_OK;
    SideBiasArgs a{};
    a.w = w_dir; a.b = reinterpret_cast<const float*>(packed_f16x3) + L.dir_b_fold;
    a.dir_rows = dir_rows; a.a_rows = a_rows; a.out = out;
    a.in_dir = d.in_dir; a.in_a = d.in_a; a.ld = NSFF_W + d.in_dir + d.in_a; a.n_rays = n_rays;
    const long long gx = (n_rays + TB_RAYS - 1) / TB_RAYS;
    if (gx > 0x7fffffffLL) return NSFF_ERR_INVALID;
    hipLaunchKernelGGL(nsff_side_bias_kernel, dim3((unsigned)gx), dim3(256), 0, reinterpret_cast<hipStream_t>(stream), a);
    return nsff_launch_status();
}

int g_nsff_last_h3_kernel = 0;
static int h3a_device_cus() {
    static int cus[64];
    int dev = 0;
    if (hipGetDevice(&dev) != hipSuccess || dev < 0 || dev >= 64) return 0;
    if (cus[dev] == 0) {
        int n = 0;
        cus[dev] = (hipDeviceGetAttribute(&n, hipDeviceAttributeMultiprocessorCount, dev) == hipSuccess && n > 0) ? n : -1;
    }
    return cus[dev] > 0 ? cus[dev] : 0;
}

int g_nsff_last_h3_shape = 0;
int g_nsff_last_h3_grid = 0;

namespace {
struct SideTileArgs { const float* dir_emb; const float* a_emb; _Float16* out; long long n_points; int pts_per_ray, in_dir, in_a, side_rows;
                     uint32_t* range; };
__global__ __launch_bounds__(256) void nsff_side_tile_kernel(const SideTileArgs a) {
    const long long tile = blockIdx.x, p0 = tile * 64;
    const int lane = threadIdx.x & 63, rblocks = a.side_rows >> 5;
    _Float16* dst = a.out + tile * (64LL * a.side_rows);
    float rm = 0.f;
    for (int blk = threadIdx.x >> 6; blk < 4 * rblocks; blk += 4) {
        const int ks = blk / rblocks, rb = blk % rblocks;
        const int row = 32 * rb + (lane & 31), pt0 = 16 * ks + 8 * (lane >> 5);
        h8 out;
#pragma unroll
        for (int t = 0; t < 8; ++t) {
            const long long p = p0 + pt0 + t;
            float v = 0.f;
            if (p < a.n_points) {
                const long long ray = p / a.pts_per_ray;
                if (row < a.in_dir) v = a.dir_emb[ray * a.in_dir + row];
                else if (row < a.in_dir + a.in_a) v = a.a_emb[ray * a.in_a + (row - a.in_dir)];
            }
            rm = nsff_absmax3(rm, v, v);
            out[t] = (_Float16)v;
        }
        *reinterpret_cast<h8*>(dst + (((long long)ks * rblocks + rb) * 64 + lane) * 8) = out;
    }
    nsff_range_flag(a.range, rm, NSFF_RANGE_CODES, (unsigned)lane);
}
}


static int h3_fill_args(const NsffModelDesc& d, const NsffFieldArgs& g, const void* packed, unsigned long long* span, uint32_t* range,
                        H3KArgs& k) {
    const int rc = nsff_make_layout_h3(d, k.L);
    if (rc) return rc;
    if (g.xyz && 3 + 6 * g.n_freqs != d.in_xyz) return NSFF_ERR_INVALID;
    k.packed = reinterpret_cast<const uint32_t*>(packed);
    k.span = span;
    k.range = range;
    k.xyz = g.xyz; k.x_emb = g.x_emb; k.dir_emb = g.dir_emb; k.a_emb = g.a_emb; k.t_emb = g.t_emb;
    k.raw = g.raw; k.n_points = g.n_points; k.pts_per_ray = g.pts_per_ray;
    k.save_acts = reinterpret_cast<_Float16*>(g.save_acts);
    k.save_xin = reinterpret_cast<_Float16*>(g.save_xin);
    k.save_masks = reinterpret_cast<unsigned long long*>(g.save_masks);
    k.save_side = reinterpret_cast<_Float16*>(g.save_side);
    k.n_tiles = (g.n_points + 63) / 64;
    k.save_stride = k.n_tiles * 64 * NSFF_W;
    if ((g.save_acts || g.save_xin || g.save_masks || g.save_side) && !g.xyz) return NSFF_ERR_INVALID;
    const void* const lo_of[3] = {g.save_acts, g.save_xin, g.save_side};
    for (int i = 0; i < 3; ++i) {
        if (g.save_lo_delta[i] < 0 || (g.save_lo_delta[i] & 7) || (g.save_lo_delta[i] != 0 && !lo_of[i])) return NSFF_ERR_INVALID;
        k.lo_delta[i] = g.save_lo_delta[i];
    }
    k.xin_rows = (k.L.k0s + k.L.kt) <= 128 ? 128 : 256;
    k.side_rows = k.L.side_k <= 128 ? 128 : 256;
    k.static_mode = g.static_mode; k.transient_mode = g.transient_mode;
    k.D = d.D; k.skip = d.skip;
    k.in_xyz = d.in_xyz; k.in_dir = d.in_dir; k.in_a = d.in_a; k.in_t = d.in_t;
    k.use_viewdir = d.use_viewdir; k.flow_scale = d.flow_scale;
    k.n_freqs = g.n_freqs;
    for (int i = 0; i < NSFF_MAX_FREQS; ++i) k.freqs[i] = g.freqs[i];
    k.octave_freqs = (g.xyz != nullptr && g.n_freqs >= 1 && g.n_freqs <= 10 && k.L.k0s == 64) ? 1 : 0;
    for (int i = 0; i + 1 < g.n_freqs; ++i)
// ... 285 lines not shown
```

### nsff_pl_amd/csrc/rays.hip

```cpp
#include <hip/hip_runtime.h>
#include <cstdlib>
#include "nsff_common.h"

namespace {

constexpr int WAVES_PER_BLOCK = 4;
constexpr int RS = NSFF_RAW_STRIDE;

__device__ __forceinline__ float wave_sum(float v) {
#pragma unroll
    for (int off = 32; off > 0; off >>= 1) v += __shfl_xor(v, off);
    return v;
}

__device__ __forceinline__ float wave_scan_mul(float v, int lane) {
#pragma unroll
    for (int off = 1; off < 64; off <<= 1) {
        const float u = __shfl_up(v, off);
        if (lane >= off) v *= u;
    }
    return v;
}
__device__ __forceinline__ float wave_scan_add(float v, int lane) {
#pragma unroll
    for (int off = 1; off < 64; off <<= 1) {
        const float u = __shfl_up(v, off);
        if (lane >= off) v += u;
    }
    return v;
}

__device__ __forceinline__ float softplus(float x) { return x > 20.f ? x : log1pf(expf(x)); }

__global__ void coarse_samples_kernel(const float* __restrict__ rays, long long n_rays,
                                      const float* __restrict__ z_lin, int S, float perturb,
                                      const float* __restrict__ rnd, float* __restrict__ zs,
                                      float* __restrict__ xyz) {
    const long long idx = (long long)blockIdx.x * blockDim.x + threadIdx.x;
    if (idx >= n_rays * S) return;
    const long long n = idx / S;
    const int i = (int)(idx - n * S);
    float z = z_lin[i];
    if (perturb > 0.f) {
        const float lower = i > 0 ? 0.5f * (z_lin[i - 1] + z_lin[i]) : z_lin[0];
        const float upper = i < S - 1 ? 0.5f * (z_lin[i] + z_lin[i + 1]) : z_lin[S - 1];
        z = lower + (upper - lower) * (perturb * rnd[idx]);
    }
    zs[idx] = z;
    const float* r = rays + n * 6;
#pragma unroll
    for (int c = 0; c < 3; ++c) xyz[idx * 3 + c] = r[c] + r[3 + c] * z;
}

__device__ __forceinline__ void sample_pdf_ray(const float* w, const float* bins, int M, float eps,
                                               const float* u, int n_imp, float* cdf,
                                               float* out_a, float* out_b, int lane, bool active) {
    float part = 0.f;
    for (int j = lane; j < M; j += 64) part += (active ? w[j] : 0.f) + eps;
    const float total = wave_sum(part);
    float carry = 0.f;
    if (lane == 0) cdf[0] = 0.f;
    for (int base = 0; base < M; base += 64) {
        const int j = base + lane;
        const float pdf = j < M ? ((active ? w[j] : 0.f) + eps) / total : 0.f;
        const float inc = wave_scan_add(pdf, lane) + carry;
        if (j < M) cdf[j + 1] = inc;
        carry = __shfl(inc, 63);
    }
    __syncthreads();
    for (int k = lane; k < n_imp; k += 64) {
        const float uk = active ? u[k] : 0.f;
        int lo = 0, hi = M + 1;
        while (lo < hi) {
            const int mid = (lo + hi) >> 1;
            if (cdf[mid] <= uk) lo = mid + 1; else hi = mid;
        }
        const int below = max(lo - 1, 0), above = min(lo, M);
        const float cb = cdf[below], ca = cdf[above];
        const float bb = bins[below], ba = bins[above];
        float denom = ca - cb;
        if (denom < eps) denom = 1.f;
        const float s = bb + (uk - cb) / denom * (ba - bb);
        if (active) {
            if (out_a) out_a[k] = s;
            if (out_b) out_b[k] = s;
        }
    }
    __syncthreads();
}

struct FineArgs {
    const float* rays; long long n_rays; const float* z_lin; const float* zs_coarse;
    int S, n_imp;
    const float* w_static; const float* w_transient;
    const float* u_static; const float* u_transient; int u_per_ray;
    float* samples_static; float* samples_transient;
    float* zs_fine; float* xyz_fine;
};

__global__ __launch_bounds__(64 * WAVES_PER_BLOCK) void fine_samples_kernel(const FineArgs a) {
    extern __shared__ __attribute__((aligned(16))) float smem[];
    const int lane = threadIdx.x & 63, wave = threadIdx.x >> 6, tid = threadIdx.x;
    constexpr int T = 64 * WAVES_PER_BLOCK;
    const long long ray = blockIdx.x;
    const int S = a.S, n_imp = a.n_imp;
    const int k_sets = a.w_transient ? 2 : 1;
    const int Sf = S + k_sets * n_imp;
    float* cdf = smem + wave * S;
    float* bins = smem + WAVES_PER_BLOCK * S;
    float* merged = bins + ((S + 3) & ~3);
    for (int j = tid; j < S - 1; j += T) bins[j] = 0.5f * (a.z_lin[j] + a.z_lin[j + 1]);
    for (int j = tid; j < S; j += T) merged[j] = a.zs_coarse[ray * S + j];
    __syncthreads();
    {
        const bool mine = wave < k_sets;
        const int set = mine ? wave : 0;
        const float* w = (set == 0 ? a.w_static : a.w_transient) + ray * S + 1;
        const float* ub = set == 0 ? a.u_static : a.u_transient;
        const float* u = a.u_per_ray ? ub + ray * n_imp : ub;
        float* keep = set == 0 ? a.samples_static : a.samples_transient;
        sample_pdf_ray(w, bins, S - 2, 1e-5f, u, n_imp, cdf, merged + S + set * n_imp,
                       keep ? keep + ray * n_imp : nullptr, lane, mine);
    }
    const float* r = a.rays + ray * 6;
    const float o0 = r[0], o1 = r[1], o2 = r[2], d0 = r[3], d1 = r[4], d2 = r[5];
    for (int i = tid; i < Sf; i += T) {
        const float v = merged[i];
        int rank = 0;
        int j = 0;
        for (; j + 4 <= Sf; j += 4) {
            const float4 o = *reinterpret_cast<const float4*>(merged + j);
            rank += (o.x < v || (o.x == v && j < i)) ? 1 : 0;
            rank += (o.y < v || (o.y == v && j + 1 < i)) ? 1 : 0;
            rank += (o.z < v || (o.z == v && j + 2 < i)) ? 1 : 0;
            rank += (o.w < v || (o.w == v && j + 3 < i)) ? 1 : 0;
        }
        for (; j < Sf; ++j) {
            const float o = merged[j];
            rank += (o < v || (o == v && j < i)) ? 1 : 0;
        }
        const long long dst = ray * Sf + rank;
        a.zs_fine[dst] = v;
        a.xyz_fine[dst * 3 + 0] = o0 + d0 * v;
        a.xyz_fine[dst * 3 + 1] = o1 + d1 * v;
        a.xyz_fine[dst * 3 + 2] = o2 + d2 * v;
    }
}

struct PdfArgs {
    const float* bins; const float* weights; long long n_rays; int M;
    const float* u; int n_imp; int u_per_ray; float eps; float* samples;
};

__global__ __launch_bounds__(64 * WAVES_PER_BLOCK) void sample_pdf_kernel(const PdfArgs a) {
    extern __shared__ __attribute__((aligned(16))) float smem[];
    const int lane = threadIdx.x & 63, wave = threadIdx.x >> 6;
    const long long ray_raw = (long long)blockIdx.x * WAVES_PER_BLOCK + wave;
    const bool active = ray_raw < a.n_rays;
    const long long ray = active ? ray_raw : a.n_rays - 1;
    float* cdf = smem + wave * (a.M + 1);
    const float* u = a.u_per_ray ? a.u + ray * a.n_imp : a.u;
    sample_pdf_ray(a.weights + ray * a.M, a.bins + ray * (a.M + 1), a.M, a.eps, u, a.n_imp, cdf,
                   active ? a.samples + ray * a.n_imp : nullptr, nullptr, lane, true);
}

struct FrameRayArgs {
    float fx, fy, cx, cy;
    float c2w[12];
    int W;
    float near, shift_near;
    long long first, count;
    float* rays;
};

__device__ __forceinline__ void ndc_pixel_ray(float fx, float fy, float cx, float cy, const float* c2w, float near,
                                              float shift_near, float i, float j, float* r) {
    const float dc[3] = {(i - cx) / fx, -(j - cy) / fy, -1.0f};
    float d[3];
#pragma unroll
    for (int k = 0; k < 3; ++k) d[k] = dc[0] * c2w[4 * k + 0] + dc[1] * c2w[4 * k + 1] + dc[2] * c2w[4 * k + 2];
    const float nrm = sqrtf(d[0] * d[0] + d[1] * d[1] + d[2] * d[2]);
#pragma unroll
    for (int k = 0; k < 3; ++k) d[k] /= nrm;
    float o[3] = {c2w[3], c2w[7], c2w[11]};
    const float t = -(shift_near + o[2]) / d[2];
#pragma unroll
    for (int k = 0; k < 3; ++k) o[k] = o[k] + t * d[k];
    const float ox_oz = o[0] / o[2], oy_oz = o[1] / o[2];
    const float sx = -1.0f / (cx / fx), sy = -1.0f / (cy / fy);
    const float o2 = 1.0f + 2.0f * near / o[2];
    r[0] = sx * ox_oz;
    r[1] = sy * oy_oz;
    r[2] = o2;
    r[3] = sx * (d[0] / d[2] - ox_oz);
    r[4] = sy * (d[1] / d[2] - oy_oz);
    r[5] = 1.0f - o2;
}

__global__ void frame_rays_kernel(const FrameRayArgs a) {
    const long long idx = (long long)blockIdx.x * blockDim.x + threadIdx.x;
    if (idx >= a.count) return;
    float r[6];
    const long long pix = a.first + idx;
    ndc_pixel_ray(a.fx, a.fy, a.cx, a.cy, a.c2w, a.near, a.shift_near, (float)(pix % a.W), (float)(pix / a.W), r);
    float* out = a.rays + idx * 6;
#pragma unroll
    for (int k = 0; k < 6; ++k) out[k] = r[k];
}

constexpr int REC_THREADS = 256;

__global__ __launch_bounds__(REC_THREADS) void ray_records_kernel(const NsffRayRecordArgs a) {
    const long long n = (long long)a.H * a.W;
    const long long pix = (long long)blockIdx.x * REC_THREADS + threadIdx.x;
    const int frame = a.first_frame + (int)blockIdx.y;
    float4 q[4] = {};
    if (pix < n) {
        const float* tab = a.frame_table + (long long)frame * NSFF_FRAME_TABLE;
        const unsigned row = (unsigned)pix / (unsigned)a.W, col = (unsigned)pix - row * (unsigned)a.W;
        const float u = (float)col, v = (float)row;
        float r[6];
        ndc_pixel_ray(a.fx, a.fy, a.cx, a.cy, tab, a.near, tab[12], u, v, r);
        const long long p = (long long)frame * n + pix;
        float rgb[3];
        if (a.image_u8) {
            const uint8_t* s = static_cast<const uint8_t*>(a.images) + p * 3;
#pragma unroll
            for (int c = 0; c < 3; ++c) rgb[c] = (float)s[c] / 255.0f;
        } else {
            const float* s = static_cast<const float*>(a.images) + p * 3;
#pragma unroll
            for (int c = 0; c < 3; ++c) rgb[c] = s[c];
        }
        const float mask = a.mask_u8 ? (float)static_cast<const uint8_t*>(a.masks)[p] / 255.0f
                                     : static_cast<const float*>(a.masks)[p];
        float2 fw = {0.f, 0.f}, bw = {0.f, 0.f};
        if (a.flow_fw && frame < a.n_frames - 1) fw = reinterpret_cast<const float2*>(a.flow_fw)[p];
        if (a.flow_bw && frame > 0) bw = reinterpret_cast<const float2*>(a.flow_bw)[p];
        q[0] = make_float4(r[0], r[1], r[2], r[3]);
        q[1] = make_float4(r[4], r[5], rgb[0], rgb[1]);
        q[2] = make_float4(rgb[2], (float)frame, a.disps[p], mask);
        q[3] = make_float4(u + fw.x, v + fw.y, u + bw.x, v + bw.y);
    }
    float4* out = reinterpret_cast<float4*>(a.records) + (long long)frame * n * 4;
    __shared__ float4 s_rec[REC_THREADS * 4];
    const int lane = threadIdx.x & 63, wave = threadIdx.x >> 6;
    float4* sw = s_rec + wave * 256;
#pragma unroll
    for (int k = 0; k < 4; ++k) sw[lane * 4 + (k ^ ((lane >> 2) & 3))] = q[k];
    __syncthreads();
    const long long pix0 = (long long)blockIdx.x * REC_THREADS + wave * 64;
#pragma unroll
    for (int k = 0; k < 4; ++k) {
        const int rec = k * 16 + (lane >> 2), c = lane & 3;
        if (pix0 + rec < n) out[(pix0 + rec) * 4 + c] = sw[rec * 4 + (c ^ ((rec >> 2) & 3))];
    }
}

__global__ void warp_points_kernel(const float* __restrict__ raw, const float* __restrict__ xyz,
                                   const float* __restrict__ zs, long long n_points, float z_far,
                                   float* __restrict__ xyz_fw, float* __restrict__ xyz_bw) {
    const long long idx = (long long)blockIdx.x * blockDim.x + threadIdx.x;
    if (idx >= n_points * 3) return;
    const long long p = idx / 3;
    const int c = (int)(idx - p * 3);
    const bool far = zs[p] > z_far;
    const float x = xyz[idx];
    xyz_fw[idx] = x + (far ? 0.f : raw[p * RS + 8 + c]);
    xyz_bw[idx] = x + (far ? 0.f : raw[p * RS + 11 + c]);
}

__device__ __forceinline__ float frustum_count(const NsffFrustumArgs& v, float x, float y, float z) {
    const float fx = v.K4[0], fy = v.K4[1], cx = v.K4[2], cy = v.K4[3];
    const float rz = 2.0f / (z - 1.0f - 1e-6f);
    const float rx = -rz * x * cx / fx;
    const float ry = -rz * y * cy / fy;
    const long long frame = v.ts[0];
    float count = 0.f;
    if (frame < 0 || frame >= v.n_frames) return count;
    for (int c = 0; c < v.n_cams; ++c) {
        const float* m = v.w2c + ((long long)c * v.n_frames + frame) * 12;
        const float cam0 = fmaf(m[2], rz, fmaf(m[1], ry, m[0] * rx)) + m[3];
        const float cam1 = fmaf(m[6], rz, fmaf(m[5], ry, m[4] * rx)) + m[7];
        const float cam2 = fmaf(m[10], rz, fmaf(m[9], ry, m[8] * rx)) + m[11];
        if (!(cam2 < 0.f)) continue;
        const float c1 = -cam1, c2 = -cam2;
        const float u = fmaf(cx, c2, fx * cam0) / c2, w = fmaf(cy, c2, fy * c1) / c2;
        if (u >= 0.f && u < (float)v.W && w >= 0.f && w < (float)v.H) count += 1.f;
    }
    return count;
}

__global__ __launch_bounds__(256) void frustum_visibility_kernel(const NsffFrustumArgs v, const float* __restrict__ xyz,
                                                                 long long n_points, float* __restrict__ out) {
    const long long p = (long long)blockIdx.x * 256 + threadIdx.x;
    if (p < n_points) out[p] = frustum_count(v, xyz[3 * p], xyz[3 * p + 1], xyz[3 * p + 2]);
}

__global__ __launch_bounds__(64 * WAVES_PER_BLOCK) void composite_kernel(const NsffCompositeArgs a) {
// ... 406 lines not shown
        if (a.disocc_fw) a.disocc_fw[ray] = 1.f - fabsf(s[P_OCCFW]);
        if (a.disocc_bw) a.disocc_bw[ray] = 1.f - fabsf(s[P_OCCBW]);
    }
}

__global__ __launch_bounds__(256) void time_rows_kernel(const float* __restrict__ table, long long n_table, int width,
                                                         const long long* __restrict__ ts, long long n, long long max_t,
                                                         float* __restrict__ next, float* __restrict__ prev, int vec) {
    const int per_row = vec ? width / 4 : width;
    const long long i = (long long)blockIdx.x * 256 + threadIdx.x;
    if (i >= n * per_row) return;
    const long long r = i / per_row;
    const int c = (int)(i - r * per_row);
    const long long t = ts[r];
    long long tn = t + 1 < max_t ? t + 1 : max_t, tp = t - 1 > 0 ? t - 1 : 0;
    tn = tn < 0 ? 0 : (tn > n_table - 1 ? n_table - 1 : tn);
    tp = tp > n_table - 1 ? n_table - 1 : tp;
    if (vec) {
        if (next) reinterpret_cast<float4*>(next)[i] = reinterpret_cast<const float4*>(table + tn * width)[c];
        if (prev) reinterpret_cast<float4*>(prev)[i] = reinterpret_cast<const float4*>(table + tp * width)[c];
    } else {
        if (next) next[i] = table[tn * width + c];
        if (prev) prev[i] = table[tp * width + c];
    }
}

constexpr int TRB_CHUNK = 2048;
constexpr int TRB_COLS = 4;
__global__ __launch_bounds__(256) void time_rows_bwd_kernel(const float* __restrict__ g_cur, const float* __restrict__ g_next,
                                                             const float* __restrict__ g_prev, const long long* __restrict__ ts,
                                                             long long n, long long max_t, long long n_table, int width,
                                                             float* __restrict__ d_table) {
    __shared__ int sList[3][TRB_CHUNK];
    __shared__ int sTs[TRB_CHUNK];
    __shared__ int sCnt[3];
    __shared__ float sPart[4][64];
    const long long r = blockIdx.x;
    const int lane = threadIdx.x & 63, part = threadIdx.x >> 6;
    const float* gs[3] = {g_cur, g_next, g_prev};
    for (int cg = 0; cg < width; cg += 64 * TRB_COLS) {
        float acc[TRB_COLS];
#pragma unroll
        for (int j = 0; j < TRB_COLS; ++j) acc[j] = 0.f;
        for (long long base = 0; base < n; base += TRB_CHUNK) {
            const long long end = base + TRB_CHUNK < n ? base + TRB_CHUNK : n;
            for (long long i = base + threadIdx.x; i < end; i += 256) {
                const long long t = ts[i];
                sTs[i - base] = (int)(t < -2 ? -2 : (t > 0x7ffffff0LL ? 0x7ffffff0LL : t));
            }
            __syncthreads();
            if (part == 0) {
                int cnt[3] = {0, 0, 0};
                for (long long i0 = base; i0 < end; i0 += 64) {
                    const long long i = i0 + lane;
                    bool hit[3] = {false, false, false};
                    if (i < end) {
                        const long long t = sTs[i - base];
                        long long tn = t + 1 < max_t ? t + 1 : max_t, tp = t - 1 > 0 ? t - 1 : 0;
                        tn = tn < 0 ? 0 : (tn > n_table - 1 ? n_table - 1 : tn);
                        tp = tp > n_table - 1 ? n_table - 1 : tp;
                        hit[0] = t == r; hit[1] = tn == r; hit[2] = tp == r;
                    }
#pragma unroll
                    for (int l = 0; l < 3; ++l) {
                        const unsigned long long m = __ballot(hit[l] && gs[l] != nullptr);
                        if (hit[l] && gs[l] != nullptr) sList[l][cnt[l] + __popcll(m & ((1ull << lane) - 1ull))] = (int)(i - base);
                        cnt[l] += __popcll(m);
                    }
                }
                if (lane == 0) { sCnt[0] = cnt[0]; sCnt[1] = cnt[1]; sCnt[2] = cnt[2]; }
            }
            __syncthreads();
#pragma unroll
            for (int l = 0; l < 3; ++l) {
                const float* __restrict__ g = gs[l];
                const int cnt = sCnt[l];
                for (int k0 = part; k0 < cnt; k0 += 16) {
                    float v[4][TRB_COLS];
#pragma unroll
                    for (int u = 0; u < 4; ++u) {
                        const int k = k0 + 4 * u;
                        const float* row = g + (base + sList[l][k < cnt ? k : k0]) * width + cg + lane;
#pragma unroll
                        for (int j = 0; j < TRB_COLS; ++j)
                            v[u][j] = (k < cnt && cg + 64 * j + lane < width) ? row[64 * j] : 0.f;
                    }
#pragma unroll
                    for (int u = 0; u < 4; ++u)
#pragma unroll
                        for (int j = 0; j < TRB_COLS; ++j) acc[j] += v[u][j];
                }
            }
            __syncthreads();
        }
#pragma unroll
        for (int j = 0; j < TRB_COLS; ++j) {
            const int c = cg + 64 * j + lane;
            if (cg + 64 * j >= width) break;
            sPart[part][lane] = acc[j];
            __syncthreads();
            if (part == 0 && c < width) d_table[r * width + c] = (sPart[0][lane] + sPart[1][lane]) + (sPart[2][lane] + sPart[3][lane]);
            __syncthreads();
        }
    }
}

}

extern "C" {

int nsff_time_rows_backward(const float* g_cur, const float* g_next, const float* g_prev, const int64_t* ts, int64_t n,
                            int64_t max_t, int64_t n_table, int32_t width, float* d_table, void* stream) {
    if (n < 0 || n_table < 1 || n_table > 0x7fffffffLL || width < 1) return NSFF_ERR_INVALID;
    if (!d_table || (n > 0 && !ts)) return NSFF_ERR_NULL;
    hipLaunchKernelGGL(time_rows_bwd_kernel, dim3((unsigned)n_table), dim3(256), 0, (hipStream_t)stream, g_cur, g_next, g_prev,
                       reinterpret_cast<const long long*>(ts), (long long)n, (long long)max_t, (long long)n_table, (int)width,
                       d_table);
    return nsff_launch_status();
}

int nsff_time_rows(const float* table, int64_t n_table, int32_t width, const int64_t* ts, int64_t n, int64_t max_t,
                   float* next, float* prev, void* stream) {
    if (n < 0 || n_table < 1 || width < 1) return NSFF_ERR_INVALID;
    if (n == 0 || (!next && !prev)) return NSFF_OK;
    if (!table || !ts) return NSFF_ERR_NULL;
    const int vec = (width % 4 == 0) && !(((uintptr_t)table | (uintptr_t)next | (uintptr_t)prev) & 15);
    const long long total = n * (vec ? width / 4 : width);
    hipLaunchKernelGGL(time_rows_kernel, dim3((unsigned)((total + 255) / 256)), dim3(256), 0, (hipStream_t)stream, table,
                       (long long)n_table, (int)width, reinterpret_cast<const long long*>(ts), (long long)n, (long long)max_t,
                       next, prev, vec);
    return nsff_launch_status();
}


int nsff_coarse_samples(const float* rays, int64_t n_rays, const float* z_lin, int32_t n_samples,
                        float perturb, const float* perturb_rand, float* zs, float* xyz, void* stream) {
    if (n_rays < 0 || n_samples < 1) return NSFF_ERR_INVALID;
    if (n_rays == 0) return NSFF_OK;
    if (!rays || !z_lin || !zs || !xyz) return NSFF_ERR_NULL;
    if (perturb > 0.f && !perturb_rand) return NSFF_ERR_NULL;
    const long long total = (long long)n_rays * n_samples;
    hipLaunchKernelGGL(coarse_samples_kernel, dim3((unsigned)((total + 255) / 256)), dim3(256), 0,
                       (hipStream_t)stream, rays, (long long)n_rays, z_lin, n_samples, perturb,
                       perturb_rand, zs, xyz);
    return nsff_launch_status();
}

int nsff_fine_samples(const float* rays, int64_t n_rays, const float* z_lin, const float* zs_coarse,
                      int32_t n_samples, int32_t n_importance,
                      const float* weights_static, const float* weights_transient,
                      const float* u_static, const float* u_transient, int32_t u_per_ray,
                      float* samples_static, float* samples_transient,
                      float* zs_fine, float* xyz_fine, void* stream) {
    if (n_rays < 0 || n_samples < 3 || n_importance < 1) return NSFF_ERR_INVALID;
    if (n_rays == 0) return NSFF_OK;
    if (!rays || !z_lin || !zs_coarse || !weights_static || !u_static || !zs_fine || !xyz_fine) return NSFF_ERR_NULL;
    if (weights_transient && !u_transient) return NSFF_ERR_NULL;
    FineArgs a{rays, (long long)n_rays, z_lin, zs_coarse, n_samples, n_importance,
               weights_static, weights_transient, u_static, u_transient, u_per_ray,
               samples_static, samples_transient, zs_fine, xyz_fine};
    const int Sf = n_samples + (weights_transient ? 2 : 1) * n_importance;
    const size_t lds = (size_t)(WAVES_PER_BLOCK * n_samples + ((n_samples + 3) & ~3) + Sf) * sizeof(float);
    if (lds > 64 * 1024 || n_rays > 0x7fffffffLL) return NSFF_ERR_INVALID;
    const unsigned blocks = (unsigned)n_rays;
    hipLaunchKernelGGL(fine_samples_kernel, dim3(blocks), dim3(64 * WAVES_PER_BLOCK), lds,
                       (hipStream_t)stream, a);
    return nsff_launch_status();
}

int nsff_sample_pdf(const float* bins, const float* weights, int64_t n_rays, int32_t n_bins_minus1,
                    const float* u, int32_t n_importance, int32_t u_per_ray, float eps,
                    float* samples, void* stream) {
    if (n_rays < 0 || n_bins_minus1 < 1 || n_importance < 1) return NSFF_ERR_INVALID;
    if (n_rays == 0) return NSFF_OK;
    if (!bins || !weights || !u || !samples) return NSFF_ERR_NULL;
    PdfArgs a{bins, weights, (long long)n_rays, n_bins_minus1, u, n_importance, u_per_ray, eps, samples};
    const size_t lds = (size_t)WAVES_PER_BLOCK * (n_bins_minus1 + 1) * sizeof(float);
    if (lds > 64 * 1024) return NSFF_ERR_INVALID;
    const unsigned blocks = (unsigned)((n_rays + WAVES_PER_BLOCK - 1) / WAVES_PER_BLOCK);
    hipLaunchKernelGGL(sample_pdf_kernel, dim3(blocks), dim3(64 * WAVES_PER_BLOCK), lds,
                       (hipStream_t)stream, a);
    return nsff_launch_status();
}

int nsff_warp_points(const float* raw, const float* xyz, const float* zs, int64_t n_points,
                     float z_far, float* xyz_fw, float* xyz_bw, void* stream) {
    if (n_points < 0) return NSFF_ERR_INVALID;
    if (n_points == 0) return NSFF_OK;
    if (!raw || !xyz || !zs || !xyz_fw || !xyz_bw) return NSFF_ERR_NULL;
    const long long total = (long long)n_points * 3;
    hipLaunchKernelGGL(warp_points_kernel, dim3((unsigned)((total + 255) / 256)), dim3(256), 0,
                       (hipStream_t)stream, raw, xyz, zs, (long long)n_points, z_far, xyz_fw, xyz_bw);
    return nsff_launch_status();
}

int nsff_frame_rays(const float* K4_host, const float* c2w_host, int32_t H, int32_t W, float near, float shift_near,
                    int64_t first_pixel, int64_t n_pixels, float* rays, void* stream) {
    if (!K4_host || !c2w_host) return NSFF_ERR_NULL;
    if (H < 1 || W < 1 || first_pixel < 0 || n_pixels < 0 || first_pixel + n_pixels > (int64_t)H * W) return NSFF_ERR_INVALID;
    if (n_pixels == 0) return NSFF_OK;
    if (!rays) return NSFF_ERR_NULL;
    FrameRayArgs a{};
    a.fx = K4_host[0]; a.fy = K4_host[1]; a.cx = K4_host[2]; a.cy = K4_host[3];
    for (int i = 0; i < 12; ++i) a.c2w[i] = c2w_host[i];
    a.W = W; a.near = near; a.shift_near = shift_near; a.first = first_pixel; a.count = n_pixels; a.rays = rays;
    hipLaunchKernelGGL(frame_rays_kernel, dim3((unsigned)((n_pixels + 255) / 256)), dim3(256), 0, (hipStream_t)stream, a);
    return nsff_launch_status();
}

int nsff_ray_records(const NsffRayRecordArgs* args, void* stream) {
    if (!args) return NSFF_ERR_NULL;
    const NsffRayRecordArgs& a = *args;
    if (a.n_frames < 0 || a.H < 1 || a.W < 1 || a.n_pixels != (int64_t)a.H * a.W) return NSFF_ERR_INVALID;
    if (a.first_frame < 0 || a.frame_count < 0 || (int64_t)a.first_frame + a.frame_count > a.n_frames) return NSFF_ERR_INVALID;
    if (a.frame_count > 65535 || a.n_pixels > 0x7fffffffLL) return NSFF_ERR_INVALID;
    if (a.frame_count == 0) return NSFF_OK;
    if (!a.images || !a.disps || !a.masks || !a.frame_table || !a.records) return NSFF_ERR_NULL;
    if (((uintptr_t)a.records & 15) || (((uintptr_t)a.flow_fw | (uintptr_t)a.flow_bw) & 7) ||
        (((uintptr_t)a.disps | (uintptr_t)a.frame_table) & 3) || (!a.image_u8 && ((uintptr_t)a.images & 3)) ||
        (!a.mask_u8 && ((uintptr_t)a.masks & 3)))
        return NSFF_ERR_ALIGN;
    const dim3 grid((unsigned)((a.n_pixels + REC_THREADS - 1) / REC_THREADS), (unsigned)a.frame_count);
    hipLaunchKernelGGL(ray_records_kernel, grid, dim3(REC_THREADS), 0, (hipStream_t)stream, a);
    return nsff_launch_status();
}

int nsff_composite(const NsffCompositeArgs* args, void* stream) {
    if (!args) return NSFF_ERR_NULL;
    const NsffCompositeArgs& a = *args;
    if (a.n_rays < 0 || a.n_samples < 1 || a.flow_mode < 0 || a.flow_mode > 2) return NSFF_ERR_INVALID;
    if (a.n_rays == 0) return NSFF_OK;
    if (!a.raw || !a.zs) return NSFF_ERR_NULL;
    if (a.flow_mode && (!a.has_transient || !a.has_rgb)) return NSFF_ERR_INVALID;
    if (a.flow_mode >= 1 && !a.xyz) return NSFF_ERR_NULL;
    if (a.flow_mode == 2 && (!a.raw_fw || !a.raw_bw || !a.xyz_fw || !a.xyz_bw)) return NSFF_ERR_NULL;
    if (a.vis.w2c && (!a.vis.ts || !a.xyz)) return NSFF_ERR_NULL;
    if (a.vis.w2c && (a.vis.n_cams < 1 || a.vis.n_frames < 1)) return NSFF_ERR_INVALID;
    const int nch = (a.n_samples + 63) / 64;
    if (nch >= 2 && nch <= 4 && a.n_rays <= 0x7fffffffLL && getenv("NSFF_SERIAL_COMPOSITE") == nullptr) {
        const dim3 grid((unsigned)a.n_rays);
        if (nch == 2) hipLaunchKernelGGL(composite_kernel_chunks<2>, grid, dim3(128), 0, (hipStream_t)stream, a);
        else if (nch == 3) hipLaunchKernelGGL(composite_kernel_chunks<3>, grid, dim3(192), 0, (hipStream_t)stream, a);
        else hipLaunchKernelGGL(composite_kernel_chunks<4>, grid, dim3(256), 0, (hipStream_t)stream, a);
        return nsff_launch_status();
    }
    const unsigned blocks = (unsigned)((a.n_rays + WAVES_PER_BLOCK - 1) / WAVES_PER_BLOCK);
    hipLaunchKernelGGL(composite_kernel, dim3(blocks), dim3(64 * WAVES_PER_BLOCK), 0,
                       (hipStream_t)stream, a);
    return nsff_launch_status();
}

int nsff_frustum_visibility(const NsffFrustumArgs* vis, const float* xyz, int64_t n_points, float* vis_count,
                            void* stream) {
    if (!vis || !vis->w2c || !vis->ts) return NSFF_ERR_NULL;
    if (n_points < 0 || vis->n_cams < 1 || vis->n_frames < 1) return NSFF_ERR_INVALID;
    if (n_points == 0) return NSFF_OK;
    if (!xyz || !vis_count) return NSFF_ERR_NULL;
    const long long blocks = (n_points + 255) / 256;
    if (blocks > 0x7fffffffLL) return NSFF_ERR_INVALID;
    hipLaunchKernelGGL(frustum_visibility_kernel, dim3((unsigned)blocks), dim3(256), 0, (hipStream_t)stream, *vis, xyz,
                       (long long)n_points, vis_count);
    return nsff_launch_status();
}

}
```

### nsff_pl_amd/csrc/rng.hip

```cpp
#include <hip/hip_runtime.h>
#include <hiprand/hiprand_kernel.h>
#include <cstdint>

#include "../../include/nsff_render.h"
#include "nsff_common.h"

namespace {

struct RngArgs {
    NsffRngJob job[NSFF_MAX_RNG_JOBS];
    unsigned first_block[NSFF_MAX_RNG_JOBS + 1];
    int n;
    unsigned long long seed;
    NsffRngCoarse coarse;
};

__device__ __forceinline__ void coarse_from_draw(const NsffRngCoarse& c, long long idx, float rnd) {
#pragma clang fp contract(off)
    const int S = c.n_samples;
    const long long n = idx / S;
    const int i = (int)(idx - n * S);
    const float* __restrict__ z_lin = c.z_lin;
    const float lower = i > 0 ? 0.5f * (z_lin[i - 1] + z_lin[i]) : z_lin[0];
    const float upper = i < S - 1 ? 0.5f * (z_lin[i] + z_lin[i + 1]) : z_lin[S - 1];
    const float t = c.perturb * rnd;
    const float span = upper - lower;
    const float z = lower + span * t;
    c.zs[idx] = z;
    const float* r = c.rays + n * 6;
#pragma unroll
    for (int k = 0; k < 3; ++k) { const float dz = r[3 + k] * z; c.xyz[idx * 3 + k] = r[k] + dz; }
}

__global__ __launch_bounds__(256) void nsff_rng_kernel(const RngArgs a) {
    int j = 0;
    while (j + 1 < a.n && blockIdx.x >= a.first_block[j + 1]) ++j;
    const NsffRngJob& J = a.job[j];
    const long long idx = (long long)(blockIdx.x - a.first_block[j]) * 256 + threadIdx.x;
    hiprandStatePhilox4_32_10_t state;
    hiprand_init(a.seed, (unsigned long long)idx, J.offset, &state);
    const long long stride = 256LL * J.grid, numel = J.numel;
    const long long rounded = ((numel - 1) / (stride * 4) + 1) * (stride * 4);
    for (long long li = idx; li < rounded; li += stride * 4) {
        const float4 r = J.kind ? hiprand_normal4(&state) : hiprand_uniform4(&state);
        const float v[4] = {r.x, r.y, r.z, r.w};
#pragma unroll
        for (int ii = 0; ii < 4; ++ii) {
            const long long l = li + stride * ii;
            if (l < numel) {
                const float x = v[ii] * 1.0f + 0.0f;
                const float y = J.kind ? x : (x == 1.0f ? 0.0f : x);
                if (J.out) J.out[l] = y;
                if (j == a.coarse.job) coarse_from_draw(a.coarse, l, y);
            }
        }
    }
}

}

extern "C" int nsff_rng_draws(const NsffRngJob* jobs, int32_t n_jobs, uint64_t seed, void* stream) {
    return nsff_rng_draws_coarse(jobs, n_jobs, seed, nullptr, stream);
}

extern "C" int nsff_rng_draws_coarse(const NsffRngJob* jobs, int32_t n_jobs, uint64_t seed, const NsffRngCoarse* coarse, void* stream) {
    if (n_jobs == 0) return coarse ? NSFF_ERR_INVALID : NSFF_OK;
    if (!jobs) return NSFF_ERR_NULL;
    if (n_jobs < 0 || n_jobs > NSFF_MAX_RNG_JOBS) return NSFF_ERR_INVALID;
    RngArgs a{};
    a.coarse.job = -1;
    if (coarse) {
        const NsffRngCoarse& c = *coarse;
        if (c.job < 0 || c.job >= n_jobs || c.n_samples < 1 || !(c.perturb > 0.f)) return NSFF_ERR_INVALID;
        if (!c.rays || !c.z_lin || !c.zs || !c.xyz) return NSFF_ERR_NULL;
        if (jobs[c.job].kind != 0 || jobs[c.job].numel % c.n_samples != 0) return NSFF_ERR_INVALID;
        a.coarse = c;
    }
    unsigned total = 0;
    for (int j = 0; j < n_jobs; ++j) {
        const NsffRngJob& J = jobs[j];
        if (!J.out && j != a.coarse.job) return NSFF_ERR_NULL;
        if (J.numel <= 0 || J.grid == 0 || (J.kind != 0 && J.kind != 1) || (J.offset & 3ull)) return NSFF_ERR_INVALID;
        if ((long long)J.grid > (J.numel + 255) / 256 || total + J.grid < total) return NSFF_ERR_INVALID;
        a.job[j] = J;
        a.first_block[j] = total;
        total += J.grid;
    }
    a.first_block[n_jobs] = total;
    a.n = n_jobs;
    a.seed = seed;
    hipLaunchKernelGGL(nsff_rng_kernel, dim3(total), dim3(256), 0, (hipStream_t)stream, a);
    const hipError_t e = hipGetLastError();
    return e == hipSuccess ? NSFF_OK : nsff_hip_fail(e);
}
```

### nsff_pl_amd/rendering.py

```python
import os

import torch

from . import _lib
from . import autograd
from . import config
from . import range_check
from . import field_grad
from . import ray_geometry

Z_FAR = 0.95

def _new(ref, *shape):
    return torch.empty(*shape, device=ref.device, dtype=torch.float32)


def sample_pdf(bins, weights, N_importance, det=False, eps=1e-5):
    _lib.require_gpu_tensor(bins, "sample_pdf bins")
    bins = bins.contiguous().float()
    weights = weights.contiguous().float()
    n_rays = weights.shape[0]
    if det:
        u = torch.linspace(0, 1, N_importance, device=bins.device)
    else:
        u = torch.rand(n_rays, N_importance, device=bins.device)
    out = _new(bins, n_rays, N_importance)
    if n_rays:
        _lib.sample_pdf(bins, weights, u.contiguous(), 0 if det else 1, eps, out)
    return out


_TORCH_RAND, _TORCH_RANDN = torch.rand, torch.randn


class _Draws:

    def __init__(self, device, n_rays, N_samples, N_importance, perturb, noise_std, test_time, models, kwargs, coarse=None):
        self.device = device
        self.coarse_done = False
        self.fused = (device.type == "cuda" and torch.rand is _TORCH_RAND and torch.randn is _TORCH_RANDN
                      and not os.environ.get("NSFF_TORCH_RNG") and not torch.cuda.is_current_stream_capturing()
                      and _lib.fused_draws_match_torch(device))
        self.at = 0
        if not self.fused:
            return
        first = models["coarse"] if N_importance > 0 else models["fine"]
        transient = bool(kwargs.get("output_transient", True) and first.encode_transient)
        flows = kwargs.get("output_transient_flow", []) if transient else []
        noisy = float(noise_std) != 0
        plan, need = [], []

        def add(kind, need_values, *shape):
            plan.append((kind, shape))
            need.append(bool(need_values))
        hook = None
        if perturb > 0:
            add("rand", coarse is None, n_rays, N_samples)
            if coarse is not None and n_rays:
                hook = (coarse[0], coarse[1], float(perturb), coarse[2], coarse[3])
        S = N_samples
        if N_importance > 0:
            add("randn", noisy, n_rays, S)
            if transient:
                add("randn", noisy, n_rays, S)
            if perturb != 0:
                add("rand", True, n_rays, N_importance)
                if transient:
                    add("rand", True, n_rays, N_importance)
            S = N_samples + (2 if transient else 1) * N_importance
        add("randn", noisy, n_rays, S)
        if transient:
            add("randn", noisy, n_rays, S)
            if flows and not test_time:
                add("randn", noisy, n_rays, S)
                add("randn", noisy, n_rays, S)
        self.plan = plan
        self.values = _lib.fused_draws(plan, device, need, coarse=hook)
        self.coarse_done = hook is not None

    def take(self, kind, *shape):
        if not self.fused:
            return (torch.rand if kind == "rand" else torch.randn)(*shape, device=self.device)
        if self.at >= len(self.plan) or self.plan[self.at] != (kind, shape):
            raise RuntimeError(f"draw {self.at}: {kind}{shape} is not the planned {self.plan[self.at:self.at + 1]}")
        self.at += 1
        return self.values[self.at - 1]


class _Pass:
    __slots__ = ("embeddings", "rays", "ts", "max_t", "noise_std", "test_time", "kwargs",
                 "freqs_xyz", "dir_embedded", "n_rays", "rec", "tbias", "neighbour_rows", "draws")


def _embed_rows(embeddings, key, idx):
    return embeddings[key](idx).detach().contiguous().float()


_LINSPACE = {}


def _unit_linspace(n, device):
    key = (int(n), str(device))
    if key not in _LINSPACE:
        if len(_LINSPACE) > 64:
            _LINSPACE.clear()
        _LINSPACE[key] = torch.linspace(0, 1, n, device=device)
    return _LINSPACE[key]


def _neighbour_time_rows(embeddings, ts, max_t):
    m = embeddings['t']
    if (isinstance(m, torch.nn.Embedding) and m.padding_idx is None and m.max_norm is None and m.weight.is_cuda
            and m.weight.dtype == torch.float32 and m.weight.is_contiguous() and ts.is_cuda and ts.dtype == torch.int64):
        return _lib.time_rows(m.weight.detach(), ts.contiguous(), max_t)
    return (_embed_rows(embeddings, 't', torch.clamp(ts + 1, max=max_t)),
            _embed_rows(embeddings, 't', torch.clamp(ts - 1, min=0)))


def _time_codes(ctx, models, kwargs, N_samples, N_importance, output_transient, flows):
    ctx.tbias, ctx.neighbour_rows = {}, None
    if not output_transient:
        return None
    n_rays, ts, m = ctx.n_rays, ctx.ts, ctx.embeddings.get('t')
    override = kwargs.get('t_embedded') if 't_embedded' in kwargs else None
    plan = []
    if not (ctx.rec is not None or n_rays == 0 or config.get_precision() != "f16x3" or config.get_tile_points() not in (0, 130)):
        passes = [('coarse', N_samples), ('fine', N_samples + 2 * N_importance)] if N_importance > 0 else [('fine', N_samples)]
        for typ, S in passes:
            model = models[typ]
            if not model.encode_transient or S % 64 or (n_rays * S < 32768 and config.get_tile_points() == 0):
                continue
            if model.in_channels_t > 64 or model.in_channels_t % 4:
                continue
            if typ == 'fine' and flows and not ctx.test_time and hasattr(model, "transient_flow_fw"):
                plan += [(typ, 'fw', model, 1), (typ, 'bw', model, -1)]
            plan.append((typ, 't', model, 0))
    plain = (override is None and isinstance(m, torch.nn.Embedding) and m.padding_idx is None and m.max_norm is None
             and m.weight.is_cuda and m.weight.dtype == torch.float32 and m.weight.is_contiguous()
             and torch.is_tensor(ts) and ts.is_cuda and ts.dtype == torch.int64
             and ts.dim() == 1 and ts.shape[0] == n_rays)
    if (plan and plain and all(mod.in_channels_t == m.weight.shape[1] for _, _, mod, _ in plan)
            and not os.environ.get('NSFF_NO_TIME_INDEX')):
        outs, rows = _lib.time_bias([(mod, d) for _, _, mod, d in plan], index=(m.weight.detach(), ts.contiguous(), ctx.max_t))
        for (typ, which, _, _), out in zip(plan, outs):
            ctx.tbias[(typ, which)] = out
        if 1 in rows:
            ctx.neighbour_rows = (rows[1], rows[-1])
        return rows[0]
    t_embedded = override if override is not None else ctx.embeddings['t'](ts)
    t_embedded = t_embedded.detach().contiguous().float()
    plan = [p for p in plan if t_embedded.shape == (n_rays, p[2].in_channels_t)]
    if plan:
        if any(w == 'fw' for _, w, _, _ in plan):
            ctx.neighbour_rows = _neighbour_time_rows(ctx.embeddings, ts, ctx.max_t)
        src = {0: t_embedded, 1: ctx.neighbour_rows[0] if ctx.neighbour_rows else None, -1: ctx.neighbour_rows[1] if ctx.neighbour_rows else None}
        for (typ, which, _, _), out in zip(plan, _lib.time_bias([(mod, src[d]) for _, _, mod, d in plan])):
            ctx.tbias[(typ, which)] = out
    return t_embedded


def _inference(results, ctx, model, xyz, zs, output_transient, output_transient_flow,
               t_embedded, a_embedded):
    typ = model.typ
    n_rays, S = zs.shape
    test_time = ctx.test_time
    results[f'zs_{typ}'] = zs
    results[f'xyzs_{typ}'] = xyz
    P = n_rays * S
    sigma_only = typ == 'coarse' and test_time
    want_flow = bool(output_transient_flow) and output_transient and not sigma_only
    warps = want_flow and not test_time
    disocc = warps and 'disocc' in output_transient_flow
    if want_flow and not hasattr(model, "transient_flow_fw"):
        raise AttributeError(f"{typ} model has no flow heads")

    raw = _new(zs, P, _lib.RAW_STRIDE)
    side = dict(dir_emb=ctx.dir_embedded if model.use_viewdir and not sigma_only else None,
                a_emb=a_embedded if (model.use_viewdir and model.in_channels_a > 0 and not sigma_only) else None)
    big_enough = ctx.rec is not None or config.get_tile_points() == 130 or (config.get_tile_points() == 0 and P >= 32768)
    if (side["dir_emb"] is not None and P and S % 64 == 0 and config.get_precision() == "f16x3" and config.get_tile_points() in (0, 130)
            and big_enough and not os.environ.get('NSFF_NO_SIDE_BIAS')):
        side["s_bias"] = _lib.side_bias(model, side["dir_emb"], side["a_emb"])

    def query(tag, raw_out, pts, static_mode, transient_mode, flow_heads, t_rows, which='t', **extra):
        saves = {}
        if ctx.rec is not None and field_grad.forward_can_save(model, static_mode, transient_mode):
            x3 = config.grad_x3()
            acts, xin, masks, side_rows = field_grad.alloc_saves(model, P, zs.device, bool(transient_mode), bool(static_mode), x3)
            saves = dict(save_acts=acts, save_xin=xin, save_masks=masks, save_side=side_rows, save_lo=x3)
            ctx.rec.setdefault("saved", {})[tag] = (raw_out, acts, xin, masks, pts.view(-1, 3), side_rows, x3)
        t_bias = ctx.tbias.get((typ, which)) if (transient_mode and not saves) else None
        _lib.field_query(model, raw_out, P, S, static_mode=static_mode, transient_mode=transient_mode,
                         flow_heads=flow_heads, xyz=pts, freqs=ctx.freqs_xyz, t_emb=t_rows, t_bias=t_bias, **saves, **extra)
    if P:
        query(typ, raw, xyz, 1 if sigma_only else 2, 0 if not output_transient else (1 if sigma_only else 2),
              2 if want_flow else 0, t_embedded if output_transient else None, **side)

    vis = None
    if test_time and output_transient and 'dataset' in ctx.kwargs and P:
        vis = ray_geometry.frustum_args(ctx.kwargs['dataset'], ctx.ts, zs.device)

    nstd = float(ctx.noise_std)
    noise_s = ctx.draws.take("randn", n_rays, S)
    noise_t = ctx.draws.take("randn", n_rays, S) if output_transient else None
    if ctx.rec is not None and nstd != 0:
        ctx.rec[f"{typ}_static"], ctx.rec[f"{typ}_transient"] = noise_s, noise_t

    args = dict(n_rays=n_rays, n_samples=S, has_transient=int(output_transient),
                has_rgb=int(not sigma_only), flow_mode=0, want_disocc=int(disocc),
                noise_std=nstd, z_far=Z_FAR, raw=raw, zs=zs, xyz=xyz, vis=vis,
                noise_static=noise_s if nstd != 0 else None,
                noise_transient=noise_t if (nstd != 0 and output_transient) else None)

    def out(key, *shape):
        t = _new(zs, *shape)
        results[key] = t
        return t

    if not sigma_only:
        args['static_rgbs'] = out(f'static_rgbs_{typ}', n_rays, S, 3)
        if output_transient:
            args['transient_rgbs'] = out(f'transient_rgbs_{typ}', n_rays, S, 3)
            if want_flow:
                args['flows_fw'] = out('transient_flows_fw', n_rays, S, 3)
                args['flows_bw'] = out('transient_flows_bw', n_rays, S, 3)
    args['static_sigmas'] = out(f'static_sigmas_{typ}', n_rays, S)
    if output_transient:
        args['transient_sigmas'] = out(f'transient_sigmas_{typ}', n_rays, S)

    if warps:
        ts = ctx.ts
        xyz_w = _new(zs, 2, n_rays, S, 3)
        xyz_fw, xyz_bw = xyz_w[0], xyz_w[1]
        results['xyzs_fw'] = xyz_fw
        raw_w = _new(zs, 2 * P, _lib.RAW_STRIDE)
        raw_fw, raw_bw = raw_w[:P], raw_w[P:]
        tp1, tm1 = ctx.neighbour_rows if ctx.neighbour_rows is not None else _neighbour_time_rows(ctx.embeddings, ts, ctx.max_t)
        tb_fw, tb_bw = ctx.tbias.get((typ, 'fw')), ctx.tbias.get((typ, 'bw'))
        def halves(a, b):
            return (a.untyped_storage().data_ptr() == b.untyped_storage().data_ptr()
                    and a.data_ptr() + a.numel() * 4 == b.data_ptr())
        merged = (ctx.rec is None and P > 0 and not os.environ.get('NSFF_NO_MERGED_REQUERY') and halves(tp1, tm1)
                  and (tb_fw is None) == (tb_bw is None) and (tb_fw is None or halves(tb_fw, tb_bw)))
        if P:
            _lib.warp_points(raw, xyz, zs, Z_FAR, xyz_fw, xyz_bw)
            if merged:
                ctx.tbias[(typ, 'fwbw')] = None if tb_fw is None else torch.as_strided(tb_fw, (2 * n_rays,) + tuple(tb_fw.shape[1:]),
                                                                                         tb_fw.stride())
                _lib.field_query(model, raw_w, 2 * P, S, static_mode=0, transient_mode=2, flow_heads=1, xyz=xyz_w,
                                 freqs=ctx.freqs_xyz, t_emb=torch.as_strided(tp1, (2 * n_rays, tp1.shape[1]), tp1.stride()),
                                 t_bias=ctx.tbias[(typ, 'fwbw')])
            else:
                query(f"{typ}_warp_fw", raw_fw, xyz_fw, 0, 2, 1, tp1, which='fw')
        noise_fw = ctx.draws.take("randn", n_rays, S)
        out('rgb_fw', n_rays, 3)
        results['xyzs_bw'] = xyz_bw
        if P and not merged:
            query(f"{typ}_warp_bw", raw_bw, xyz_bw, 0, 2, 1, tm1, which='bw')
        noise_bw = ctx.draws.take("randn", n_rays, S)
        if ctx.rec is not None and nstd != 0:
            ctx.rec[f"{typ}_warp_fw"], ctx.rec[f"{typ}_warp_bw"] = noise_fw, noise_bw
        out('rgb_bw', n_rays, 3)
        args.update(raw_fw=raw_fw, raw_bw=raw_bw, xyz_fw=xyz_fw, xyz_bw=xyz_bw,
                    noise_fw=noise_fw if nstd != 0 else None,
                    noise_bw=noise_bw if nstd != 0 else None,
                    rgb_fw=results['rgb_fw'], rgb_bw=results['rgb_bw'],
                    xyzs_fw_bw=out('xyzs_fw_bw', n_rays, S, 3),
                    xyzs_bw_fw=out('xyzs_bw_fw', n_rays, S, 3))

    if output_transient:
        args['static_weights'] = out(f'static_weights_{typ}', n_rays, S)
        args['transient_weights'] = out(f'transient_weights_{typ}', n_rays, S)
        args['weights'] = out(f'weights_{typ}', n_rays, S)
    else:
        args['static_weights'] = out(f'static_weights_{typ}', n_rays, S)
    if test_time and output_transient:
        args['static_alphas'] = out(f'static_alphas_{typ}', n_rays, S)
        args['transient_alphas'] = out(f'transient_alphas_{typ}', n_rays, S)

    if not sigma_only:
        args['depth'] = out(f'depth_{typ}', n_rays)
        args['rgb'] = out(f'rgb_{typ}', n_rays, 3)
        if output_transient:
            args['transient_alpha'] = out(f'transient_alpha_{typ}', n_rays)
            args['transient_rgb'] = out(f'transient_rgb_{typ}', n_rays, 3)
            args['static_only_rgb'] = out(f'_static_rgb_{typ}', n_rays, 3)
            args['static_only_depth'] = out(f'_static_depth_{typ}', n_rays)
            if want_flow:
                args['flow_mode'] = 2 if warps else 1
                args['xyz_exp'] = out('xyz_fine', n_rays, 3)
                args['flow_fw_exp'] = out('transient_flow_fw', n_rays, 3)
                args['xyz_fw_exp'] = out('xyz_fw', n_rays, 3)
                args['flow_bw_exp'] = out('transient_flow_bw', n_rays, 3)
                args['xyz_bw_exp'] = out('xyz_bw', n_rays, 3)
                if disocc:
                    args['disocc_fw'] = out('disocc_fw', n_rays, 1)
                    args['disoccs_fw'] = out('disoccs_fw', n_rays, S, 1)
                    args['disocc_bw'] = out('disocc_bw', n_rays, 1)
                    args['disoccs_bw'] = out('disoccs_bw', n_rays, S, 1)
    if n_rays:
        _lib.composite(**args)


def render_rays(models,
                embeddings,
                rays,
                ts,
                max_t,
                N_samples=64,
                perturb=0,
                noise_std=0,
                N_importance=0,
                chunk=1024 * 32,
                test_time=False,
                **kwargs):
    _lib.require_gpu_tensor(rays, "rays")
    return range_check.checked(
        "render_rays", rays.device,
        lambda: _render_rays(models, embeddings, rays, ts, max_t, N_samples, perturb, noise_std, N_importance, chunk, test_time, kwargs),
        can_fallback=bool(test_time) and perturb == 0 and noise_std == 0)


def _render_rays(models, embeddings, rays, ts, max_t, N_samples, perturb, noise_std, N_importance, chunk, test_time, kwargs,
                 fine_points=None):
    _lib.require_gpu_tensor(rays, "rays")
    _lib.load()
    want_grad = (torch.is_grad_enabled() and not test_time and
                 bool(autograd.grad_parameters(models, embeddings)))
    rec = {} if want_grad else None
    with torch.cuda.device(rays.device), torch.no_grad():
        results = {}
        rays = rays.contiguous().float()
        n_rays = rays.shape[0]
        embedding_xyz, embedding_dir = embeddings['xyz'], embeddings['dir']

        ctx = _Pass()
        ctx.embeddings, ctx.rays, ctx.ts, ctx.max_t = embeddings, rays, ts, max_t
        ctx.noise_std, ctx.test_time, ctx.kwargs, ctx.n_rays = noise_std, test_time, kwargs, n_rays
        ctx.freqs_xyz = [float(f) for f in embedding_xyz.freqs]
        ctx.rec = rec
        ctx.tbias, ctx.neighbour_rows = {}, None
        ctx.dir_embedded = None
        if any(m.use_viewdir for m in models.values()):
            view_dir = kwargs.get('view_dir', rays[:, 3:6])
            ctx.dir_embedded = embedding_dir(view_dir.contiguous().float())

        z_lin = _unit_linspace(N_samples, rays.device)
        zs = _new(rays, n_rays, N_samples)
        xyz_coarse = _new(rays, n_rays, N_samples, 3)
        ctx.draws = _Draws(rays.device, n_rays, N_samples, N_importance, perturb, noise_std, test_time, models, kwargs,
                           coarse=(rays, z_lin, zs, xyz_coarse))
        perturb_rand = ctx.draws.take("rand", n_rays, N_samples) if perturb > 0 else None
        if n_rays and not ctx.draws.coarse_done:
            _lib.coarse_samples(rays, z_lin, perturb, perturb_rand, zs, xyz_coarse)

        t_embedded = None
        if N_importance > 0:
            model = models['coarse']
            output_transient = bool(kwargs.get('output_transient', True) and model.encode_transient)
            t_embedded = _time_codes(ctx, models, kwargs, N_samples, N_importance, output_transient,
                                     kwargs.get('output_transient_flow', []))
            _inference(results, ctx, model, xyz_coarse, zs, output_transient, [], t_embedded, None)

            det = perturb == 0
            if det:
                u_s = _unit_linspace(N_importance, rays.device)
                u_t = u_s
            else:
                u_s = ctx.draws.take("rand", n_rays, N_importance)
                u_t = ctx.draws.take("rand", n_rays, N_importance) if output_transient else None
            S_fine = N_samples + (2 if output_transient else 1) * N_importance
            zs_static = _new(rays, n_rays, N_importance) if test_time else None
            zs_transient = _new(rays, n_rays, N_importance) if (test_time and output_transient) else None
            zs_fine = _new(rays, n_rays, S_fine)
            xyz_fine = _new(rays, n_rays, S_fine, 3)
            if n_rays:
                _lib.fine_samples(rays, z_lin, zs, N_importance,
                                  results['static_weights_coarse'],
                                  results['transient_weights_coarse'] if output_transient else None,
                                  u_s, u_t if output_transient else None, 0 if det else 1,
                                  zs_static, zs_transient, zs_fine, xyz_fine)
            if test_time:
                results['static_zs_fine'] = zs_static
                if output_transient:
                    results['transient_zs_fine'] = zs_transient
            if fine_points is not None:
                zs_fine, xyz_fine = fine_points(rays, zs_fine, xyz_fine)
                if tuple(zs_fine.shape) != (n_rays, S_fine) or tuple(xyz_fine.shape) != (n_rays, S_fine, 3):
                    raise ValueError(f"fine_points: expected shapes {(n_rays, S_fine)} / {(n_rays, S_fine, 3)}")
            zs, xyz = zs_fine, xyz_fine
        else:
            xyz = xyz_coarse

        model = models['fine']
        a_embedded = None
        if model.encode_appearance:
            a_embedded = kwargs['a_embedded'] if 'a_embedded' in kwargs else embeddings['a'](ts)
            a_embedded = a_embedded.detach().contiguous().float()
        if N_importance == 0:
            output_transient = bool(kwargs.get('output_transient', True) and model.encode_transient)
            t_embedded = _time_codes(ctx, models, kwargs, N_samples, 0, output_transient, kwargs.get('output_transient_flow', []))
        output_transient_flow = [] if not output_transient else kwargs.get('output_transient_flow', [])
        _inference(results, ctx, model, xyz, zs, output_transient, output_transient_flow,
                   t_embedded, a_embedded)
    if rec is None:
        return results
    rec.update(N_importance=N_importance, noise_std=float(noise_std), output_transient=output_transient,
               flows=list(output_transient_flow), zs_coarse=results.get('zs_coarse', results.get('zs_fine')),
               zs_fine=results['zs_fine'], view_dir=kwargs.get('view_dir', rays[:, 3:6]), dir_embedded=ctx.dir_embedded,
               t_embedded_override=kwargs.get('t_embedded'), a_embedded_override=kwargs.get('a_embedded'))
    return autograd.attach(results, models, embeddings, rays, ts, max_t, rec)


from .interpolation import interpolate
```

Before: 71.84 million ray-samples/s.

## Fuse RNG draws, time-bias and fine sampling into staged multi-job launches

Adds a stage-launch API that packs RNG draw jobs, time-bias jobs and the fine-sample ray job into one kernel launch partitioned by block ranges. The render path defers those launches and issues a head stage before the coarse field and a mid stage in place of fine_samples, which also picks up the remaining draws and time-bias jobs. The aim is to cut per-launch and host overhead from several small kernels. The cost is more planning code, a shared LDS budget across heterogeneous jobs, and ordering risk if deferred draws are consumed before they are launched.

```diff
diff --git a/include/nsff_render.h b/include/nsff_render.h
--- a/include/nsff_render.h
+++ b/include/nsff_render.h
@@ -577,6 +577,35 @@
 int64_t nsff_scene_scale_work_bytes(int32_t n_frames, int32_t n_points, int32_t H, int32_t W);
 int     nsff_scene_scale(const NsffSceneScaleArgs* args, void* stream);
 
+#define NSFF_STAGE_RNG        0
+#define NSFF_STAGE_TIME_BIAS  1
+#define NSFF_STAGE_RAY        2
+#define NSFF_MAX_STAGE_JOBS   (NSFF_MAX_RNG_JOBS + NSFF_MAX_TIME_BIAS_JOBS + 1)
+typedef struct NsffStageRay {
+    const float* rays;  int64_t n_rays;  const float* z_lin;  const float* zs_coarse;
+    int32_t n_samples, n_importance;
+    const float* weights_static;  const float* weights_transient;
+    const float* u_static;  const float* u_transient;
+    int32_t u_per_ray, pad_;
+    float* samples_static;  float* samples_transient;  float* zs_fine;  float* xyz_fine;
+} NsffStageRay;
+typedef struct NsffStageArgs {
+    const NsffRngJob* rng;  const NsffRngCoarse* coarse;  uint64_t seed;
+    const NsffTimeBiasJob* time_bias;  int64_t time_bias_rays;
+    const NsffStageRay* ray;
+    int32_t n_rng, n_time_bias;
+} NsffStageArgs;
+typedef struct NsffStagePlan {
+    int32_t  n_jobs;
+    uint32_t n_blocks;
+    int32_t  kind[NSFF_MAX_STAGE_JOBS];
+    int32_t  index[NSFF_MAX_STAGE_JOBS];
+    uint32_t first_block[NSFF_MAX_STAGE_JOBS + 1];
+    uint32_t lds_bytes;
+} NsffStagePlan;
+int nsff_stage_plan(const NsffStageArgs* args, NsffStagePlan* plan);
+int nsff_stage_launch(const NsffStageArgs* args, void* stream);
+
 int         nsff_abi_version(void);
 const char* nsff_last_hip_error(void);
 
diff --git a/nsff_pl_amd/_lib.py b/nsff_pl_amd/_lib.py
--- a/nsff_pl_amd/_lib.py
+++ b/nsff_pl_amd/_lib.py
@@ -60,6 +60,28 @@
 class RngCoarse(C.Structure):
     _fields_ = [("rays", _fp), ("z_lin", _fp), ("zs", _fp), ("xyz", _fp), ("n_samples", C.c_int32), ("perturb", C.c_float),
                 ("job", C.c_int32), ("pad_", C.c_int32)]
+
+
+MAX_STAGE_JOBS = MAX_RNG_JOBS + MAX_TIME_BIAS_JOBS + 1
+STAGE_RNG, STAGE_TIME_BIAS, STAGE_RAY = 0, 1, 2
+
+
+class StageRay(C.Structure):
+    _fields_ = [("rays", _fp), ("n_rays", C.c_int64), ("z_lin", _fp), ("zs_coarse", _fp), ("n_samples", C.c_int32),
+                ("n_importance", C.c_int32), ("weights_static", _fp), ("weights_transient", _fp), ("u_static", _fp),
+                ("u_transient", _fp), ("u_per_ray", C.c_int32), ("pad_", C.c_int32), ("samples_static", _fp),
+                ("samples_transient", _fp), ("zs_fine", _fp), ("xyz_fine", _fp)]
+
+
+class StageArgs(C.Structure):
+    _fields_ = [("rng", C.POINTER(RngJob)), ("coarse", C.POINTER(RngCoarse)), ("seed", C.c_uint64),
+                ("time_bias", C.POINTER(TimeBiasJob)), ("time_bias_rays", C.c_int64), ("ray", C.POINTER(StageRay)),
+                ("n_rng", C.c_int32), ("n_time_bias", C.c_int32)]
+
+
+class StagePlan(C.Structure):
+    _fields_ = [("n_jobs", C.c_int32), ("n_blocks", C.c_uint32), ("kind", C.c_int32 * MAX_STAGE_JOBS),
+                ("index", C.c_int32 * MAX_STAGE_JOBS), ("first_block", C.c_uint32 * (MAX_STAGE_JOBS + 1)), ("lds_bytes", C.c_uint32)]
 
 
 _COMPOSITE_PTRS_IN = ["raw", "raw_fw", "raw_bw", "zs", "xyz", "xyz_fw", "xyz_bw",
@@ -271,6 +293,8 @@
     "nsff_time_bias": (C.c_int, [C.POINTER(TimeBiasJob), C.c_int32, C.c_int64, C.c_void_p]),
     "nsff_rng_draws": (C.c_int, [C.POINTER(RngJob), C.c_int32, C.c_uint64, C.c_void_p]),
     "nsff_rng_draws_coarse": (C.c_int, [C.POINTER(RngJob), C.c_int32, C.c_uint64, C.POINTER(RngCoarse), C.c_void_p]),
+    "nsff_stage_plan": (C.c_int, [C.POINTER(StageArgs), C.POINTER(StagePlan)]),
+    "nsff_stage_launch": (C.c_int, [C.POINTER(StageArgs), C.c_void_p]),
     "nsff_side_bias": (C.c_int, [C.POINTER(ModelDesc), _fp, _fp, _fp, _fp, C.c_int64, _fp, C.c_void_p]),
     "nsff_last_hip_error": (C.c_char_p, []),
     "nsff_packed_bytes": (C.c_int, [C.POINTER(ModelDesc), C.c_int, C.POINTER(C.c_size_t)]),
@@ -573,7 +597,36 @@
 _DEVICE_RNG_GEOMETRY = {}
 
 
-def fused_draws(plan, device, values=True, coarse=None):
+def draw_jobs(sizes, kinds, wanted, offset, max_grid, hooked=False):
+    jobs, seen = [], 0
+    for d, (numel, kind, want) in enumerate(zip(sizes, kinds, wanted)):
+        if numel == 0:
+            seen += 1
+            continue
+        grid = min(max_grid, (numel + 255) // 256)
+        if hooked and not seen and not want:
+            jobs.append((d, numel, offset, 0, grid, False))
+        elif want:
+            jobs.append((d, numel, offset, 1 if kind == "randn" else 0, grid, True))
+        seen += 1
+        offset += ((numel - 1) // (1024 * grid) + 1) * 4
+    return jobs, offset
+
+
+class DrawPlan:
+    __slots__ = ("outs", "jobs", "draw", "seed", "hook", "device_index")
+
+    def job_array(self, which=None):
+        part = [j for j, d in zip(self.jobs, self.draw) if which is None or d in which]
+        assert len(part) <= MAX_RNG_JOBS
+        arr = (RngJob * max(len(part), 1))()
+        for j, (t, numel, off, kind, grid) in enumerate(part):
+            arr[j].out, arr[j].numel, arr[j].offset, arr[j].kind, arr[j].grid = (None if t is None else t.data_ptr()), numel, off, kind, grid
+        hook = self.hook if (self.hook is not None and part and part[0] is self.jobs[0]) else None
+        return arr, len(part), hook
+
+
+def fused_draws(plan, device, values=True, coarse=None, launch=True):
     dev = torch.device(device)
     idx = dev.index if dev.index is not None else torch.cuda.current_device()
     if idx not in _DEVICE_RNG_GEOMETRY:
@@ -591,29 +644,34 @@
         sizes.append(n)
     total = sum(n for n, w in zip(sizes, wanted) if w)
     buf = torch.empty(max(total, 1), device=dev, dtype=torch.float32)
-    outs, jobs, at = [], [], 0
-    for (kind, shape), numel, want in zip(plan, sizes, wanted):
+    planned, offset = draw_jobs(sizes, [k for k, _ in plan], wanted, offset, max_grid, coarse is not None)
+    by_draw = {d: (numel, off, kind, grid, keep) for d, numel, off, kind, grid, keep in planned}
+    outs, jobs, draw, at = [], [], [], 0
+    for d, ((kind, shape), numel) in enumerate(zip(plan, sizes)):
         if numel == 0:
             outs.append(torch.empty(*shape, device=dev, dtype=torch.float32))
-            continue
-        grid = min(max_grid, (numel + 255) // 256)
-        if coarse is not None and not outs and not want:
-            jobs.append((None, numel, offset, 0, grid))
+        elif d not in by_draw:
             outs.append(None)
-        elif want:
-            t = buf[at:at + numel].view(*shape)
-            at += numel
-            jobs.append((t, numel, offset, 1 if kind == "randn" else 0, grid))
+        else:
+            _, off, k01, grid, keep = by_draw[d]
+            t = None
+            if keep:
+                t = buf[at:at + numel].view(*shape)
+                at += numel
+            jobs.append((t, numel, off, k01, grid))
+            draw.append(d)
             outs.append(t)
-        else:
-            outs.append(None)
-        offset += ((numel - 1) // (1024 * grid) + 1) * 4
     hook = None
     if coarse is not None:
         rays, z_lin, perturb, zs, xyz = coarse
         assert plan and plan[0][0] == "rand" and tuple(plan[0][1]) == (rays.shape[0], z_lin.shape[0]) and perturb > 0
         if sizes[0]:
             hook = RngCoarse(_ptr(rays), _ptr(z_lin), _ptr(zs), _ptr(xyz), int(z_lin.shape[0]), float(perturb), 0, 0)
+    if not launch:
+        dp = DrawPlan()
+        dp.outs, dp.jobs, dp.draw, dp.seed, dp.hook, dp.device_index = outs, jobs, draw, seed, hook, idx
+        gen.set_offset(offset)
+        return dp
     for k in range(0, len(jobs), MAX_RNG_JOBS):
         part = jobs[k:k + MAX_RNG_JOBS]
         arr = (RngJob * len(part))()
@@ -668,7 +726,7 @@
     return load().nsff_time_bias_rows(C.byref(model_desc(model)))
 
 
-def time_bias(jobs, index=None):
+def time_bias(jobs, index=None, launch=True):
     assert 1 <= len(jobs) <= MAX_TIME_BIAS_JOBS
     arr = (TimeBiasJob * len(jobs))()
     keep, outs, per_model, pair = [], [], {}, None
@@ -721,8 +779,50 @@
                 written.add(delta)
         outs.append(out)
     keep.append(per_model)
+    if not launch:
+        return (outs, (arr, n_rays, keep)) if index is None else (outs, rows_of, (arr, n_rays, keep))
     _check(load().nsff_time_bias(arr, len(jobs), n_rays, _stream()), "nsff_time_bias")
     return outs if index is None else (outs, rows_of)
+
+
+def stage_args(draws=None, which=None, tb=None, tb_which=None, ray=None):
+    a, keep = StageArgs(), []
+    if draws is not None:
+        arr, n, hook = draws.job_array(which)
+        a.rng, a.n_rng, a.seed = arr, n, draws.seed
+        if hook is not None:
+            a.coarse = C.pointer(hook)
+        keep += [arr, hook]
+    if tb is not None:
+        arr, n_rays, alive = tb
+        sel = list(range(len(arr))) if tb_which is None else list(tb_which)
+        part = (TimeBiasJob * max(len(sel), 1))()
+        for k, q in enumerate(sel):
+            C.memmove(C.byref(part[k]), C.byref(arr[q]), C.sizeof(TimeBiasJob))
+        a.time_bias, a.n_time_bias, a.time_bias_rays = part, len(sel), n_rays
+        keep += [part, alive]
+    if ray is not None:
+        (rays, z_lin, zs_coarse, n_importance, w_static, w_transient, u_static, u_transient, u_per_ray,
+         samples_static, samples_transient, zs_fine, xyz_fine) = ray
+        r = StageRay(_ptr(rays), rays.shape[0], _ptr(z_lin), _ptr(zs_coarse), z_lin.shape[0], int(n_importance),
+                     _ptr(w_static), _ptr(w_transient), _ptr(u_static), _ptr(u_transient), int(u_per_ray), 0,
+                     _ptr(samples_static), _ptr(samples_transient), _ptr(zs_fine), _ptr(xyz_fine))
+        a.ray = C.pointer(r)
+        keep.append(r)
+    return a, keep
+
+
+def stage_plan(args):
+    p = StagePlan()
+    _check(load().nsff_stage_plan(C.byref(args), C.byref(p)), "nsff_stage_plan")
+    return [(p.kind[e], p.index[e], p.first_block[e], p.first_block[e + 1]) for e in range(p.n_jobs)], int(p.lds_bytes)
+
+
+def stage_launch(draws=None, which=None, tb=None, tb_which=None, ray=None):
+    a, keep = stage_args(draws, which, tb, tb_which, ray)
+    if a.n_rng == 0 and a.n_time_bias == 0 and ray is None:
+        return
+    _check(load().nsff_stage_launch(C.byref(a), _stream()), "nsff_stage_launch")
 
 
 def coarse_samples(rays, z_lin, perturb, perturb_rand, zs, xyz):
diff --git a/nsff_pl_amd/csrc/field_h3.hip b/nsff_pl_amd/csrc/field_h3.hip
--- a/nsff_pl_amd/csrc/field_h3.hip
+++ b/nsff_pl_amd/csrc/field_h3.hip
@@ -5,6 +5,7 @@
 #include "nsff_layout_h3.h"
 #include "nsff_common.h"
 #include "nsff_internal.h"
+#include "nsff_time_bias_body.h"
 
 typedef float f32x16 __attribute__((ext_vector_type(16)));
 typedef _Float16 h8 __attribute__((ext_vector_type(8)));
@@ -1849,75 +1850,48 @@
 }
 
 namespace {
-struct TimeBiasJobK { const float* w[NSFF_MAX_LAYERS]; const float* b[NSFF_MAX_LAYERS]; int ld[NSFF_MAX_LAYERS];
-                      const float* t_rows; float* out; int rows, in_xyz, in_t;
-                      const float* table; const long long* ts; long long n_table, max_t; int delta; float* rows_out; };
+using TimeBiasJobK = NsffTimeBiasJobK;
+static_assert(NSFF_TB_W == NSFF_W, "nsff_time_bias_body.h");
 struct TimeBiasArgs { TimeBiasJobK job[NSFF_MAX_TIME_BIAS_JOBS]; long long n_rays; };
-constexpr int TB_RAYS = 16;
+constexpr int TB_RAYS = NSFF_TB_RAYS;
 __global__ __launch_bounds__(256) void nsff_time_bias_kernel(const TimeBiasArgs a) {
     const TimeBiasJobK& j = a.job[blockIdx.z];
-    const int i = blockIdx.y, n = threadIdx.x;
+    const int i = blockIdx.y;
     if (i >= j.rows) return;
-    const long long r0 = (long long)blockIdx.x * TB_RAYS;
     __shared__ __attribute__((aligned(16))) float st[TB_RAYS][64];
     __shared__ float sw[16][NSFF_W + 1];
-    const float* __restrict__ wl = j.w[i] + j.in_xyz;
-    const int ld = j.ld[i], in_t = j.in_t;
-    float tv[TB_RAYS / 4], wv[4][16];
-#pragma unroll
-    for (int k = 0; k < TB_RAYS / 4; ++k) {
-        const int e = threadIdx.x + 256 * k, r = e >> 6, c = e & 63;
-        const long long ray = r0 + r < a.n_rays ? r0 + r : a.n_rays - 1;
-        const float* row = j.t_rows != nullptr ? j.t_rows + ray * in_t : nullptr;
-        if (row == nullptr) {
-            long long t = j.ts[ray] + j.delta;
-            if (j.delta > 0) t = t < j.max_t ? t : j.max_t;
-            if (j.delta < 0) t = t > 0 ? t : 0;
-            t = t < 0 ? 0 : (t > j.n_table - 1 ? j.n_table - 1 : t);
-            row = j.table + t * in_t;
-        }
-        tv[k] = c < in_t ? row[c] : 0.f;
-        if (j.rows_out != nullptr && i == 0 && c < in_t && r0 + r < a.n_rays) j.rows_out[(r0 + r) * in_t + c] = tv[k];
-    }
-    const float b = j.b[i][n];
-#pragma unroll
-    for (int q = 0; q < 4; ++q)
-#pragma unroll
-        for (int k = 0; k < 16; ++k) {
-            const int e = threadIdx.x + 256 * k, row = e >> 4, c = 16 * q + (e & 15);
-            wv[q][k] = c < in_t ? wl[row * ld + c] : 0.f;
-        }
-#pragma unroll
-    for (int k = 0; k < TB_RAYS / 4; ++k) { const int e = threadIdx.x + 256 * k; st[e >> 6][e & 63] = tv[k]; }
-    float acc[TB_RAYS];
-#pragma unroll
-    for (int r = 0; r < TB_RAYS; ++r) acc[r] = b;
-#pragma unroll
-    for (int q = 0; q < 4; ++q) {
-        if (16 * q >= in_t) break;
-        __syncthreads();
-#pragma unroll
-        for (int k = 0; k < 16; ++k) { const int e = threadIdx.x + 256 * k; sw[e & 15][e >> 4] = wv[q][k]; }
-        __syncthreads();
-#pragma unroll
-        for (int u = 0; u < 16; u += 4) {
-            const float w0 = sw[u][n], w1 = sw[u + 1][n], w2 = sw[u + 2][n], w3 = sw[u + 3][n];
-#pragma unroll
-            for (int r = 0; r < TB_RAYS; ++r) {
-                const float4 t4 = *reinterpret_cast<const float4*>(&st[r][16 * q + u]);
-                acc[r] = fmaf(w3, t4.w, fmaf(w2, t4.z, fmaf(w1, t4.y, fmaf(w0, t4.x, acc[r]))));
-            }
-        }
-    }
-#pragma unroll
-    for (int r = 0; r < TB_RAYS; ++r)
-        if (r0 + r < a.n_rays) j.out[((r0 + r) * j.rows + i) * NSFF_W + n] = acc[r];
+    nsff_time_bias_body<16, true>(j, a.n_rays, i, (long long)blockIdx.x * TB_RAYS, st, sw);
 }
 }
 
 extern "C" int nsff_time_bias_rows(const NsffModelDesc* desc) {
     if (!desc || !desc->has_transient || desc->in_t < 1) return 0;
     return 1 + __builtin_popcount(nsff_skip_layers(desc));
+}
+
+int nsff_time_bias_prepare(const NsffTimeBiasJob& jb, NsffTimeBiasJobK& k) {
+    if (!jb.desc || !jb.out) return NSFF_ERR_NULL;
+    if (!jb.t_rows && (!jb.table || !jb.ts || jb.n_table < 1 || jb.delta < -1 || jb.delta > 1)) return NSFF_ERR_NULL;
+    const NsffModelDesc& d = *jb.desc;
+    NsffLayoutH3 L;
+    const int rc = nsff_make_layout_h3(d, L);
+    if (rc) return rc;
+    k.rows = nsff_time_bias_rows(&d);
+    if (k.rows < 1) return NSFF_ERR_INVALID;
+    if (d.in_t > 64 || (d.in_t & 3) != 0) return NSFF_ERR_INVALID;
+    k.in_xyz = d.in_xyz; k.in_t = d.in_t; k.t_rows = jb.t_rows; k.out = jb.out;
+    k.table = jb.table; k.ts = reinterpret_cast<const long long*>(jb.ts); k.n_table = jb.n_table; k.max_t = jb.max_t;
+    k.delta = jb.delta; k.rows_out = jb.t_rows ? nullptr : jb.rows_out;
+    const uint32_t skips = nsff_skip_layers(&d);
+    int i = 0;
+    for (int l = 0; l < d.D; ++l) {
+        if (l != 0 && !((skips >> l) & 1u)) continue;
+        k.w[i] = jb.w[i]; k.b[i] = jb.b[i];
+        if (!k.w[i] || !k.b[i]) return NSFF_ERR_NULL;
+        k.ld[i] = d.in_xyz + d.in_t + (l ? NSFF_W : 0);
+        ++i;
+    }
+    return NSFF_OK;
 }
 
 extern "C" int nsff_time_bias(const NsffTimeBiasJob* jobs, int32_t n_jobs, int64_t n_rays, void* stream) {
@@ -1928,29 +1902,9 @@
     a.n_rays = n_rays;
     int max_rows = 0;
     for (int q = 0; q < n_jobs; ++q) {
-        const NsffTimeBiasJob& jb = jobs[q];
-        if (!jb.desc || !jb.out) return NSFF_ERR_NULL;
-        if (!jb.t_rows && (!jb.table || !jb.ts || jb.n_table < 1 || jb.delta < -1 || jb.delta > 1)) return NSFF_ERR_NULL;
-        const NsffModelDesc& d = *jb.desc;
-        NsffLayoutH3 L;
-        const int rc = nsff_make_layout_h3(d, L);
+        TimeBiasJobK& k = a.job[q];
+        const int rc = nsff_time_bias_prepare(jobs[q], k);
         if (rc) return rc;
-        TimeBiasJobK& k = a.job[q];
-        k.rows = nsff_time_bias_rows(&d);
-        if (k.rows < 1) return NSFF_ERR_INVALID;
-        if (d.in_t > 64 || (d.in_t & 3) != 0) return NSFF_ERR_INVALID;
-        k.in_xyz = d.in_xyz; k.in_t = d.in_t; k.t_rows = jb.t_rows; k.out = jb.out;
-        k.table = jb.table; k.ts = reinterpret_cast<const long long*>(jb.ts); k.n_table = jb.n_table; k.max_t = jb.max_t;
-        k.delta = jb.delta; k.rows_out = jb.t_rows ? nullptr : jb.rows_out;
-        const uint32_t skips = nsff_skip_layers(&d);
-        int i = 0;
-        for (int l = 0; l < d.D; ++l) {
-            if (l != 0 && !((skips >> l) & 1u)) continue;
-            k.w[i] = jb.w[i]; k.b[i] = jb.b[i];
-            if (!k.w[i] || !k.b[i]) return NSFF_ERR_NULL;
-            k.ld[i] = d.in_xyz + d.in_t + (l ? NSFF_W : 0);
-            ++i;
-        }
         max_rows = std::max(max_rows, k.rows);
     }
     const long long gx = (n_rays + TB_RAYS - 1) / TB_RAYS;
diff --git a/nsff_pl_amd/csrc/nsff_ray_body.h b/nsff_pl_amd/csrc/nsff_ray_body.h
--- /dev/null
+++ b/nsff_pl_amd/csrc/nsff_ray_body.h
@@ -0,0 +1,128 @@
+#pragma once
+#include <hip/hip_runtime.h>
+#include <cstddef>
+#include <cstdint>
+
+#include "../../include/nsff_render.h"
+
+constexpr int NSFF_RAY_WAVES = 4;
+
+static __device__ __forceinline__ float wave_sum(float v) {
+#pragma unroll
+    for (int off = 32; off > 0; off >>= 1) v += __shfl_xor(v, off);
+    return v;
+}
+
+static __device__ __forceinline__ float wave_scan_add(float v, int lane) {
+#pragma unroll
+    for (int off = 1; off < 64; off <<= 1) {
+        const float u = __shfl_up(v, off);
+        if (lane >= off) v += u;
+    }
+    return v;
+}
+
+static __device__ __forceinline__ void sample_pdf_ray(const float* w, const float* bins, int M, float eps,
+                                                      const float* u, int n_imp, float* cdf,
+                                                      float* out_a, float* out_b, int lane, bool active) {
+#pragma clang fp contract(off)
+    float part = 0.f;
+    for (int j = lane; j < M; j += 64) part += (active ? w[j] : 0.f) + eps;
+    const float total = wave_sum(part);
+    float carry = 0.f;
+    if (lane == 0) cdf[0] = 0.f;
+    for (int base = 0; base < M; base += 64) {
+        const int j = base + lane;
+        const float pdf = j < M ? ((active ? w[j] : 0.f) + eps) / total : 0.f;
+        const float inc = wave_scan_add(pdf, lane) + carry;
+        if (j < M) cdf[j + 1] = inc;
+        carry = __shfl(inc, 63);
+    }
+    __syncthreads();
+    for (int k = lane; k < n_imp; k += 64) {
+        const float uk = active ? u[k] : 0.f;
+        int lo = 0, hi = M + 1;
+        while (lo < hi) {
+            const int mid = (lo + hi) >> 1;
+            if (cdf[mid] <= uk) lo = mid + 1; else hi = mid;
+        }
+        const int below = max(lo - 1, 0), above = min(lo, M);
+        const float cb = cdf[below], ca = cdf[above];
+        const float bb = bins[below], ba = bins[above];
+        float denom = ca - cb;
+        if (denom < eps) denom = 1.f;
+        const float s = bb + (uk - cb) / denom * (ba - bb);
+        if (active) {
+            if (out_a) out_a[k] = s;
+            if (out_b) out_b[k] = s;
+        }
+    }
+    __syncthreads();
+}
+
+struct NsffFineArgs {
+    const float* rays; long long n_rays; const float* z_lin; const float* zs_coarse;
+    int S, n_imp;
+    const float* w_static; const float* w_transient;
+    const float* u_static; const float* u_transient; int u_per_ray;
+    float* samples_static; float* samples_transient;
+    float* zs_fine; float* xyz_fine;
+};
+
+inline int nsff_fine_args_check(const NsffFineArgs& a, size_t* lds) {
+    if (a.n_rays < 0 || a.S < 3 || a.n_imp < 1) return NSFF_ERR_INVALID;
+    if (!a.rays || !a.z_lin || !a.zs_coarse || !a.w_static || !a.u_static || !a.zs_fine || !a.xyz_fine) return NSFF_ERR_NULL;
+    if (a.w_transient && !a.u_transient) return NSFF_ERR_NULL;
+    const int Sf = a.S + (a.w_transient ? 2 : 1) * a.n_imp;
+    *lds = (size_t)(NSFF_RAY_WAVES * a.S + ((a.S + 3) & ~3) + Sf) * sizeof(float);
+    if (*lds > 64 * 1024 || a.n_rays > 0x7fffffffLL) return NSFF_ERR_INVALID;
+    return NSFF_OK;
+}
+
+static __device__ __forceinline__ void nsff_fine_samples_body(const NsffFineArgs& a, long long ray, float* smem) {
+#pragma clang fp contract(off)
+    const int lane = threadIdx.x & 63, wave = threadIdx.x >> 6, tid = threadIdx.x;
+    constexpr int WAVES_PER_BLOCK = NSFF_RAY_WAVES, T = 64 * WAVES_PER_BLOCK;
+    const int S = a.S, n_imp = a.n_imp;
+    const int k_sets = a.w_transient ? 2 : 1;
+    const int Sf = S + k_sets * n_imp;
+    float* cdf = smem + wave * S;
+    float* bins = smem + WAVES_PER_BLOCK * S;
+    float* merged = bins + ((S + 3) & ~3);
+    for (int j = tid; j < S - 1; j += T) bins[j] = 0.5f * (a.z_lin[j] + a.z_lin[j + 1]);
+    for (int j = tid; j < S; j += T) merged[j] = a.zs_coarse[ray * S + j];
+    __syncthreads();
+    {
+        const bool mine = wave < k_sets;
+        const int set = mine ? wave : 0;
+        const float* w = (set == 0 ? a.w_static : a.w_transient) + ray * S + 1;
+        const float* ub = set == 0 ? a.u_static : a.u_transient;
+        const float* u = a.u_per_ray ? ub + ray * n_imp : ub;
+        float* keep = set == 0 ? a.samples_static : a.samples_transient;
+        sample_pdf_ray(w, bins, S - 2, 1e-5f, u, n_imp, cdf, merged + S + set * n_imp,
+                       keep ? keep + ray * n_imp : nullptr, lane, mine);
+    }
+    const float* r = a.rays + ray * 6;
+    const float o0 = r[0], o1 = r[1], o2 = r[2], d0 = r[3], d1 = r[4], d2 = r[5];
+    for (int i = tid; i < Sf; i += T) {
+        const float v = merged[i];
+        int rank = 0;
+        int j = 0;
+        for (; j + 4 <= Sf; j += 4) {
+            const float4 o = *reinterpret_cast<const float4*>(merged + j);
+            rank += (o.x < v || (o.x == v && j < i)) ? 1 : 0;
+            rank += (o.y < v || (o.y == v && j + 1 < i)) ? 1 : 0;
+            rank += (o.z < v || (o.z == v && j + 2 < i)) ? 1 : 0;
+            rank += (o.w < v || (o.w == v && j + 3 < i)) ? 1 : 0;
+        }
+        for (; j < Sf; ++j) {
+            const float o = merged[j];
+            rank += (o < v || (o == v && j < i)) ? 1 : 0;
+        }
+        const long long dst = ray * Sf + rank;
+        a.zs_fine[dst] = v;
+        a.xyz_fine[dst * 3 + 0] = o0 + d0 * v;
+        a.xyz_fine[dst * 3 + 1] = o1 + d1 * v;
+        a.xyz_fine[dst * 3 + 2] = o2 + d2 * v;
+    }
+}
diff --git a/nsff_pl_amd/csrc/nsff_rng_body.h b/nsff_pl_amd/csrc/nsff_rng_body.h
--- /dev/null
+++ b/nsff_pl_amd/csrc/nsff_rng_body.h
@@ -0,0 +1,70 @@
+#pragma once
+#include <hip/hip_runtime.h>
+#include <hiprand/hiprand_kernel.h>
+#include <cstdint>
+
+#include "../../include/nsff_render.h"
+
+static __device__ __forceinline__ void nsff_coarse_from_draw(const NsffRngCoarse& c, long long idx, float rnd) {
+#pragma clang fp contract(off)
+    const int S = c.n_samples;
+    const long long n = idx / S;
+    const int i = (int)(idx - n * S);
+    const float* __restrict__ z_lin = c.z_lin;
+    const float lower = i > 0 ? 0.5f * (z_lin[i - 1] + z_lin[i]) : z_lin[0];
+    const float upper = i < S - 1 ? 0.5f * (z_lin[i] + z_lin[i + 1]) : z_lin[S - 1];
+    const float t = c.perturb * rnd;
+    const float span = upper - lower;
+    const float z = lower + span * t;
+    c.zs[idx] = z;
+    const float* r = c.rays + n * 6;
+#pragma unroll
+    for (int k = 0; k < 3; ++k) { const float dz = r[3 + k] * z; c.xyz[idx * 3 + k] = r[k] + dz; }
+}
+
+static __device__ __forceinline__ void nsff_rng_job_body(const NsffRngJob& J, unsigned long long seed, long long idx, bool hook,
+                                                         const NsffRngCoarse& c) {
+    hiprandStatePhilox4_32_10_t state;
+    hiprand_init(seed, (unsigned long long)idx, J.offset, &state);
+    const long long stride = 256LL * J.grid, numel = J.numel;
+    const long long rounded = ((numel - 1) / (stride * 4) + 1) * (stride * 4);
+    for (long long li = idx; li < rounded; li += stride * 4) {
+        const float4 r = J.kind ? hiprand_normal4(&state) : hiprand_uniform4(&state);
+        const float v[4] = {r.x, r.y, r.z, r.w};
+#pragma unroll
+        for (int ii = 0; ii < 4; ++ii) {
+            const long long l = li + stride * ii;
+            if (l < numel) {
+                const float x = v[ii] * 1.0f + 0.0f;
+                const float y = J.kind ? x : (x == 1.0f ? 0.0f : x);
+                if (J.out) J.out[l] = y;
+                if (hook) nsff_coarse_from_draw(c, l, y);
+            }
+        }
+    }
+}
+
+inline int nsff_rng_check(const NsffRngJob* jobs, int32_t n_jobs, const NsffRngCoarse* coarse, unsigned* total) {
+    *total = 0;
+    if (n_jobs == 0) return coarse ? NSFF_ERR_INVALID : NSFF_OK;
+    if (!jobs) return NSFF_ERR_NULL;
+    if (n_jobs < 0 || n_jobs > NSFF_MAX_RNG_JOBS) return NSFF_ERR_INVALID;
+    int hook = -1;
+    if (coarse) {
+        const NsffRngCoarse& c = *coarse;
+        if (c.job < 0 || c.job >= n_jobs || c.n_samples < 1 || !(c.perturb > 0.f)) return NSFF_ERR_INVALID;
+        if (!c.rays || !c.z_lin || !c.zs || !c.xyz) return NSFF_ERR_NULL;
+        if (jobs[c.job].kind != 0 || jobs[c.job].numel % c.n_samples != 0) return NSFF_ERR_INVALID;
+        hook = c.job;
+    }
+    unsigned sum = 0;
+    for (int j = 0; j < n_jobs; ++j) {
+        const NsffRngJob& J = jobs[j];
+        if (!J.out && j != hook) return NSFF_ERR_NULL;
+        if (J.numel <= 0 || J.grid == 0 || (J.kind != 0 && J.kind != 1) || (J.offset & 3ull)) return NSFF_ERR_INVALID;
+        if ((long long)J.grid > (J.numel + 255) / 256 || sum + J.grid < sum) return NSFF_ERR_INVALID;
+        sum += J.grid;
+    }
+    *total = sum;
+    return NSFF_OK;
+}
diff --git a/nsff_pl_amd/csrc/nsff_time_bias_body.h b/nsff_pl_amd/csrc/nsff_time_bias_body.h
--- /dev/null
+++ b/nsff_pl_amd/csrc/nsff_time_bias_body.h
@@ -0,0 +1,94 @@
+#pragma once
+#include <hip/hip_runtime.h>
+#include <cstdint>
+
+#include "../../include/nsff_render.h"
+
+struct NsffTimeBiasJobK { const float* w[NSFF_MAX_LAYERS]; const float* b[NSFF_MAX_LAYERS]; int ld[NSFF_MAX_LAYERS];
+                          const float* t_rows; float* out; int rows, in_xyz, in_t;
+                          const float* table; const long long* ts; long long n_table, max_t; int delta; float* rows_out; };
+constexpr int NSFF_TB_W = 256;
+constexpr int NSFF_TB_RAYS = 16;
+constexpr int nsff_time_bias_lds_floats(int cols) { return NSFF_TB_RAYS * 64 + cols * (NSFF_TB_W + 1); }
+
+int nsff_time_bias_prepare(const NsffTimeBiasJob& jb, NsffTimeBiasJobK& k);
+
+template <int COLS, bool UPFRONT>
+static __device__ __forceinline__ void nsff_time_bias_body(const NsffTimeBiasJobK& j, long long n_rays, int i, long long r0,
+                                                           float (*st)[64], float (*sw)[NSFF_TB_W + 1]) {
+    static_assert(COLS % 4 == 0 && 64 % COLS == 0, "whole float4s of the 64 staged columns");
+    constexpr int TB_RAYS = NSFF_TB_RAYS, NQ = 64 / COLS;
+    const int n = threadIdx.x;
+    const float* __restrict__ wl = j.w[i] + j.in_xyz;
+    const int ld = j.ld[i], in_t = j.in_t;
+    float tv[TB_RAYS / 4], wv[UPFRONT ? NQ : 3][COLS];
+#pragma unroll
+    for (int k = 0; k < TB_RAYS / 4; ++k) {
+        const int e = threadIdx.x + 256 * k, r = e >> 6, c = e & 63;
+        const long long ray = r0 + r < n_rays ? r0 + r : n_rays - 1;
+        const float* row = j.t_rows != nullptr ? j.t_rows + ray * in_t : nullptr;
+        if (row == nullptr) {
+            long long t = j.ts[ray] + j.delta;
+            if (j.delta > 0) t = t < j.max_t ? t : j.max_t;
+            if (j.delta < 0) t = t > 0 ? t : 0;
+            t = t < 0 ? 0 : (t > j.n_table - 1 ? j.n_table - 1 : t);
+            row = j.table + t * in_t;
+        }
+        tv[k] = c < in_t ? row[c] : 0.f;
+        if (j.rows_out != nullptr && i == 0 && c < in_t && r0 + r < n_rays) j.rows_out[(r0 + r) * in_t + c] = tv[k];
+    }
+    const float b = j.b[i][n];
+    constexpr int KROWS = 256 / COLS;
+    const int row0 = threadIdx.x / COLS, col0 = threadIdx.x % COLS;
+    const float* __restrict__ wp = wl + row0 * ld + col0;
+    float* swp = &sw[col0][row0];
+    auto request = [&](int q, float* dst) {
+#pragma unroll
+        for (int k = 0; k < COLS; ++k) dst[k] = COLS * q + col0 < in_t ? wp[k * KROWS * ld + COLS * q] : 0.f;
+    };
+    if constexpr (UPFRONT) {
+#pragma unroll
+        for (int q = 0; q < NQ; ++q) request(q, wv[q]);
+    } else {
+        request(0, wv[0]);
+        request(1, wv[1]);
+    }
+#pragma unroll
+    for (int k = 0; k < TB_RAYS / 4; ++k) { const int e = threadIdx.x + 256 * k; st[e >> 6][e & 63] = tv[k]; }
+    float acc[TB_RAYS];
+#pragma unroll
+    for (int r = 0; r < TB_RAYS; ++r) acc[r] = b;
+    auto step = [&](int q, const float* cur) {
+        __syncthreads();
+#pragma unroll
+        for (int k = 0; k < COLS; ++k) swp[k * KROWS] = cur[k];
+        __syncthreads();
+#pragma unroll
+        for (int u = 0; u < COLS; u += 4) {
+            const float w0 = sw[u][n], w1 = sw[u + 1][n], w2 = sw[u + 2][n], w3 = sw[u + 3][n];
+#pragma unroll
+            for (int r = 0; r < TB_RAYS; ++r) {
+                const float4 t4 = *reinterpret_cast<const float4*>(&st[r][COLS * q + u]);
+                acc[r] = fmaf(w3, t4.w, fmaf(w2, t4.z, fmaf(w1, t4.y, fmaf(w0, t4.x, acc[r]))));
+            }
+        }
+    };
+    if constexpr (UPFRONT) {
+#pragma unroll
+        for (int q = 0; q < NQ; ++q) {
+            if (COLS * q >= in_t) break;
+            step(q, wv[q]);
+        }
+    } else {
+#pragma unroll 1
+        for (int q = 0; COLS * q < in_t; ++q) {
+            request(q + 2, wv[2]);
+            step(q, wv[0]);
+#pragma unroll
+            for (int k = 0; k < COLS; ++k) { wv[0][k] = wv[1][k]; wv[1][k] = wv[2][k]; }
+        }
+    }
+#pragma unroll
+    for (int r = 0; r < TB_RAYS; ++r)
+        if (r0 + r < n_rays) j.out[((r0 + r) * j.rows + i) * NSFF_TB_W + n] = acc[r];
+}
diff --git a/nsff_pl_amd/csrc/rays.hip b/nsff_pl_amd/csrc/rays.hip
--- a/nsff_pl_amd/csrc/rays.hip
+++ b/nsff_pl_amd/csrc/rays.hip
@@ -1,17 +1,12 @@
 #include <hip/hip_runtime.h>
 #include <cstdlib>
 #include "nsff_common.h"
+#include "nsff_ray_body.h"
 
 namespace {
 
-constexpr int WAVES_PER_BLOCK = 4;
+constexpr int WAVES_PER_BLOCK = NSFF_RAY_WAVES;
 constexpr int RS = NSFF_RAW_STRIDE;
-
-__device__ __forceinline__ float wave_sum(float v) {
-#pragma unroll
-    for (int off = 32; off > 0; off >>= 1) v += __shfl_xor(v, off);
-    return v;
-}
 
 __device__ __forceinline__ float wave_scan_mul(float v, int lane) {
 #pragma unroll
@@ -21,15 +16,6 @@
     }
     return v;
 }
-__device__ __forceinline__ float wave_scan_add(float v, int lane) {
-#pragma unroll
-    for (int off = 1; off < 64; off <<= 1) {
-        const float u = __shfl_up(v, off);
-        if (lane >= off) v += u;
-    }
-    return v;
-}
-
 __device__ __forceinline__ float softplus(float x) { return x > 20.f ? x : log1pf(expf(x)); }
 
 __global__ void coarse_samples_kernel(const float* __restrict__ rays, long long n_rays,
@@ -52,99 +38,9 @@
     for (int c = 0; c < 3; ++c) xyz[idx * 3 + c] = r[c] + r[3 + c] * z;
 }
 
-__device__ __forceinline__ void sample_pdf_ray(const float* w, const float* bins, int M, float eps,
-                                               const float* u, int n_imp, float* cdf,
-                                               float* out_a, float* out_b, int lane, bool active) {
-    float part = 0.f;
-    for (int j = lane; j < M; j += 64) part += (active ? w[j] : 0.f) + eps;
-    const float total = wave_sum(part);
-    float carry = 0.f;
-    if (lane == 0) cdf[0] = 0.f;
-    for (int base = 0; base < M; base += 64) {
-        const int j = base + lane;
-        const float pdf = j < M ? ((active ? w[j] : 0.f) + eps) / total : 0.f;
-        const float inc = wave_scan_add(pdf, lane) + carry;
-        if (j < M) cdf[j + 1] = inc;
-        carry = __shfl(inc, 63);
-    }
-    __syncthreads();
-    for (int k = lane; k < n_imp; k += 64) {
-        const float uk = active ? u[k] : 0.f;
-        int lo = 0, hi = M + 1;
-        while (lo < hi) {
-            const int mid = (lo + hi) >> 1;
-            if (cdf[mid] <= uk) lo = mid + 1; else hi = mid;
-        }
-        const int below = max(lo - 1, 0), above = min(lo, M);
-        const float cb = cdf[below], ca = cdf[above];
-        const float bb = bins[below], ba = bins[above];
-        float denom = ca - cb;
-        if (denom < eps) denom = 1.f;
-        const float s = bb + (uk - cb) / denom * (ba - bb);
-        if (active) {
-            if (out_a) out_a[k] = s;
-            if (out_b) out_b[k] = s;
-        }
-    }
-    __syncthreads();
-}
-
-struct FineArgs {
-    const float* rays; long long n_rays; const float* z_lin; const float* zs_coarse;
-    int S, n_imp;
-    const float* w_static; const float* w_transient;
-    const float* u_static; const float* u_transient; int u_per_ray;
-    float* samples_static; float* samples_transient;
-    float* zs_fine; float* xyz_fine;
-};
-
-__global__ __launch_bounds__(64 * WAVES_PER_BLOCK) void fine_samples_kernel(const FineArgs a) {
+__global__ __launch_bounds__(64 * WAVES_PER_BLOCK) void fine_samples_kernel(const NsffFineArgs a) {
     extern __shared__ __attribute__((aligned(16))) float smem[];
-    const int lane = threadIdx.x & 63, wave = threadIdx.x >> 6, tid = threadIdx.x;
-    constexpr int T = 64 * WAVES_PER_BLOCK;
-    const long long ray = blockIdx.x;
-    const int S = a.S, n_imp = a.n_imp;
-    const int k_sets = a.w_transient ? 2 : 1;
-    const int Sf = S + k_sets * n_imp;
-    float* cdf = smem + wave * S;
-    float* bins = smem + WAVES_PER_BLOCK * S;
-    float* merged = bins + ((S + 3) & ~3);
-    for (int j = tid; j < S - 1; j += T) bins[j] = 0.5f * (a.z_lin[j] + a.z_lin[j + 1]);
-    for (int j = tid; j < S; j += T) merged[j] = a.zs_coarse[ray * S + j];
-    __syncthreads();
-    {
-        const bool mine = wave < k_sets;
-        const int set = mine ? wave : 0;
-        const float* w = (set == 0 ? a.w_static : a.w_transient) + ray * S + 1;
-        const float* ub = set == 0 ? a.u_static : a.u_transient;
-        const float* u = a.u_per_ray ? ub + ray * n_imp : ub;
-        float* keep = set == 0 ? a.samples_static : a.samples_transient;
-        sample_pdf_ray(w, bins, S - 2, 1e-5f, u, n_imp, cdf, merged + S + set * n_imp,
-                       keep ? keep + ray * n_imp : nullptr, lane, mine);
-    }
-    const float* r = a.rays + ray * 6;
-    const float o0 = r[0], o1 = r[1], o2 = r[2], d0 = r[3], d1 = r[4], d2 = r[5];
-    for (int i = tid; i < Sf; i += T) {
-        const float v = merged[i];
-        int rank = 0;
-        int j = 0;
-        for (; j + 4 <= Sf; j += 4) {
-            const float4 o = *reinterpret_cast<const float4*>(merged + j);
-            rank += (o.x < v || (o.x == v && j < i)) ? 1 : 0;
-            rank += (o.y < v || (o.y == v && j + 1 < i)) ? 1 : 0;
-            rank += (o.z < v || (o.z == v && j + 2 < i)) ? 1 : 0;
-            rank += (o.w < v || (o.w == v && j + 3 < i)) ? 1 : 0;
-        }
-        for (; j < Sf; ++j) {
-            const float o = merged[j];
-            rank += (o < v || (o == v && j < i)) ? 1 : 0;
-        }
-        const long long dst = ray * Sf + rank;
-        a.zs_fine[dst] = v;
-        a.xyz_fine[dst * 3 + 0] = o0 + d0 * v;
-        a.xyz_fine[dst * 3 + 1] = o1 + d1 * v;
-        a.xyz_fine[dst * 3 + 2] = o2 + d2 * v;
-    }
+    nsff_fine_samples_body(a, blockIdx.x, smem);
 }
 
 struct PdfArgs {
@@ -857,16 +753,14 @@
                       const float* u_static, const float* u_transient, int32_t u_per_ray,
                       float* samples_static, float* samples_transient,
                       float* zs_fine, float* xyz_fine, void* stream) {
+    NsffFineArgs a{rays, (long long)n_rays, z_lin, zs_coarse, n_samples, n_importance,
+                   weights_static, weights_transient, u_static, u_transient, u_per_ray,
+                   samples_static, samples_transient, zs_fine, xyz_fine};
     if (n_rays < 0 || n_samples < 3 || n_importance < 1) return NSFF_ERR_INVALID;
     if (n_rays == 0) return NSFF_OK;
-    if (!rays || !z_lin || !zs_coarse || !weights_static || !u_static || !zs_fine || !xyz_fine) return NSFF_ERR_NULL;
-    if (weights_transient && !u_transient) return NSFF_ERR_NULL;
-    FineArgs a{rays, (long long)n_rays, z_lin, zs_coarse, n_samples, n_importance,
-               weights_static, weights_transient, u_static, u_transient, u_per_ray,
-               samples_static, samples_transient, zs_fine, xyz_fine};
-    const int Sf = n_samples + (weights_transient ? 2 : 1) * n_importance;
-    const size_t lds = (size_t)(WAVES_PER_BLOCK * n_samples + ((n_samples + 3) & ~3) + Sf) * sizeof(float);
-    if (lds > 64 * 1024 || n_rays > 0x7fffffffLL) return NSFF_ERR_INVALID;
+    size_t lds = 0;
+    const int rc = nsff_fine_args_check(a, &lds);
+    if (rc) return rc;
     const unsigned blocks = (unsigned)n_rays;
     hipLaunchKernelGGL(fine_samples_kernel, dim3(blocks), dim3(64 * WAVES_PER_BLOCK), lds,
                        (hipStream_t)stream, a);
diff --git a/nsff_pl_amd/csrc/rng.hip b/nsff_pl_amd/csrc/rng.hip
--- a/nsff_pl_amd/csrc/rng.hip
+++ b/nsff_pl_amd/csrc/rng.hip
@@ -1,9 +1,9 @@
 #include <hip/hip_runtime.h>
-#include <hiprand/hiprand_kernel.h>
 #include <cstdint>
 
 #include "../../include/nsff_render.h"
 #include "nsff_common.h"
+#include "nsff_rng_body.h"
 
 namespace {
 
@@ -15,46 +15,10 @@
     NsffRngCoarse coarse;
 };
 
-__device__ __forceinline__ void coarse_from_draw(const NsffRngCoarse& c, long long idx, float rnd) {
-#pragma clang fp contract(off)
-    const int S = c.n_samples;
-    const long long n = idx / S;
-    const int i = (int)(idx - n * S);
-    const float* __restrict__ z_lin = c.z_lin;
-    const float lower = i > 0 ? 0.5f * (z_lin[i - 1] + z_lin[i]) : z_lin[0];
-    const float upper = i < S - 1 ? 0.5f * (z_lin[i] + z_lin[i + 1]) : z_lin[S - 1];
-    const float t = c.perturb * rnd;
-    const float span = upper - lower;
-    const float z = lower + span * t;
-    c.zs[idx] = z;
-    const float* r = c.rays + n * 6;
-#pragma unroll
-    for (int k = 0; k < 3; ++k) { const float dz = r[3 + k] * z; c.xyz[idx * 3 + k] = r[k] + dz; }
-}
-
 __global__ __launch_bounds__(256) void nsff_rng_kernel(const RngArgs a) {
     int j = 0;
     while (j + 1 < a.n && blockIdx.x >= a.first_block[j + 1]) ++j;
-    const NsffRngJob& J = a.job[j];
-    const long long idx = (long long)(blockIdx.x - a.first_block[j]) * 256 + threadIdx.x;
-    hiprandStatePhilox4_32_10_t state;
-    hiprand_init(a.seed, (unsigned long long)idx, J.offset, &state);
-    const long long stride = 256LL * J.grid, numel = J.numel;
-    const long long rounded = ((numel - 1) / (stride * 4) + 1) * (stride * 4);
-    for (long long li = idx; li < rounded; li += stride * 4) {
-        const float4 r = J.kind ? hiprand_normal4(&state) : hiprand_uniform4(&state);
-        const float v[4] = {r.x, r.y, r.z, r.w};
-#pragma unroll
-        for (int ii = 0; ii < 4; ++ii) {
-            const long long l = li + stride * ii;
-            if (l < numel) {
-                const float x = v[ii] * 1.0f + 0.0f;
-                const float y = J.kind ? x : (x == 1.0f ? 0.0f : x);
-                if (J.out) J.out[l] = y;
-                if (j == a.coarse.job) coarse_from_draw(a.coarse, l, y);
-            }
-        }
-    }
+    nsff_rng_job_body(a.job[j], a.seed, (long long)(blockIdx.x - a.first_block[j]) * 256 + threadIdx.x, j == a.coarse.job, a.coarse);
 }
 
 }
@@ -64,27 +28,17 @@
 }
 
 extern "C" int nsff_rng_draws_coarse(const NsffRngJob* jobs, int32_t n_jobs, uint64_t seed, const NsffRngCoarse* coarse, void* stream) {
-    if (n_jobs == 0) return coarse ? NSFF_ERR_INVALID : NSFF_OK;
-    if (!jobs) return NSFF_ERR_NULL;
-    if (n_jobs < 0 || n_jobs > NSFF_MAX_RNG_JOBS) return NSFF_ERR_INVALID;
+    unsigned total = 0;
+    const int rc = nsff_rng_check(jobs, n_jobs, coarse, &total);
+    if (rc != NSFF_OK || n_jobs == 0) return rc;
     RngArgs a{};
     a.coarse.job = -1;
-    if (coarse) {
-        const NsffRngCoarse& c = *coarse;
-        if (c.job < 0 || c.job >= n_jobs || c.n_samples < 1 || !(c.perturb > 0.f)) return NSFF_ERR_INVALID;
-        if (!c.rays || !c.z_lin || !c.zs || !c.xyz) return NSFF_ERR_NULL;
-        if (jobs[c.job].kind != 0 || jobs[c.job].numel % c.n_samples != 0) return NSFF_ERR_INVALID;
-        a.coarse = c;
-    }
-    unsigned total = 0;
+    if (coarse) a.coarse = *coarse;
+    total = 0;
     for (int j = 0; j < n_jobs; ++j) {
-        const NsffRngJob& J = jobs[j];
-        if (!J.out && j != a.coarse.job) return NSFF_ERR_NULL;
-        if (J.numel <= 0 || J.grid == 0 || (J.kind != 0 && J.kind != 1) || (J.offset & 3ull)) return NSFF_ERR_INVALID;
-        if ((long long)J.grid > (J.numel + 255) / 256 || total + J.grid < total) return NSFF_ERR_INVALID;
-        a.job[j] = J;
+        a.job[j] = jobs[j];
         a.first_block[j] = total;
-        total += J.grid;
+        total += jobs[j].grid;
     }
     a.first_block[n_jobs] = total;
     a.n = n_jobs;
diff --git a/nsff_pl_amd/csrc/stage.hip b/nsff_pl_amd/csrc/stage.hip
--- /dev/null
+++ b/nsff_pl_amd/csrc/stage.hip
@@ -0,0 +1,133 @@
+#include <hip/hip_runtime.h>
+#include <algorithm>
+#include <cstdint>
+
+#include "../../include/nsff_render.h"
+#include "nsff_common.h"
+#include "nsff_rng_body.h"
+#include "nsff_time_bias_body.h"
+#include "nsff_ray_body.h"
+
+namespace {
+
+constexpr int TB_COLS_LEAN = 4, TB_COLS = 16;
+constexpr size_t tb_lds(bool lean) { return sizeof(float) * nsff_time_bias_lds_floats(lean ? TB_COLS_LEAN : TB_COLS); }
+
+struct StageArgs {
+    unsigned first_block[NSFF_MAX_STAGE_JOBS + 1];
+    signed char kind[NSFF_MAX_STAGE_JOBS], index[NSFF_MAX_STAGE_JOBS];
+    int n;
+    unsigned tb_gx;
+    long long tb_rays;
+    unsigned long long seed;
+    NsffRngCoarse coarse;
+    NsffRngJob rng[NSFF_MAX_RNG_JOBS];
+    NsffTimeBiasJobK tb[NSFF_MAX_TIME_BIAS_JOBS];
+    NsffFineArgs ray;
+};
+
+template <bool LEAN>
+__device__ __forceinline__ void stage_body(const StageArgs& a) {
+    extern __shared__ __attribute__((aligned(16))) float smem[];
+    int e = 0;
+    while (e + 1 < a.n && blockIdx.x >= a.first_block[e + 1]) ++e;
+    const unsigned local = blockIdx.x - a.first_block[e];
+    const int kind = a.kind[e], q = a.index[e];
+    if (kind == NSFF_STAGE_RAY) {
+        nsff_fine_samples_body(a.ray, (long long)local, smem);
+    } else if (kind == NSFF_STAGE_TIME_BIAS) {
+        const unsigned i = local / a.tb_gx, bx = local - i * a.tb_gx;
+        nsff_time_bias_body<LEAN ? TB_COLS_LEAN : TB_COLS, !LEAN>(a.tb[q], a.tb_rays, (int)i, (long long)bx * NSFF_TB_RAYS,
+                                                                  reinterpret_cast<float (*)[64]>(smem),
+                                                                  reinterpret_cast<float (*)[NSFF_TB_W + 1]>(smem + NSFF_TB_RAYS * 64));
+    } else {
+        nsff_rng_job_body(a.rng[q], a.seed, (long long)local * 256 + threadIdx.x, q == a.coarse.job, a.coarse);
+    }
+}
+
+__global__ __launch_bounds__(256, 8) void nsff_stage_kernel_ray(const StageArgs a) { stage_body<true>(a); }
+__global__ __launch_bounds__(256) void nsff_stage_kernel(const StageArgs a) { stage_body<false>(a); }
+
+NsffFineArgs fine_args(const NsffStageRay& r) {
+    return NsffFineArgs{r.rays, (long long)r.n_rays, r.z_lin, r.zs_coarse, r.n_samples, r.n_importance,
+                        r.weights_static, r.weights_transient, r.u_static, r.u_transient, r.u_per_ray,
+                        r.samples_static, r.samples_transient, r.zs_fine, r.xyz_fine};
+}
+
+int make_plan(const NsffStageArgs& s, NsffStagePlan& p, StageArgs* k) {
+    p = NsffStagePlan{};
+    if (s.n_rng < 0 || s.n_rng > NSFF_MAX_RNG_JOBS || s.n_time_bias < 0 || s.n_time_bias > NSFF_MAX_TIME_BIAS_JOBS
+        || s.time_bias_rays < 0) return NSFF_ERR_INVALID;
+    if ((s.n_rng && !s.rng) || (s.n_time_bias && !s.time_bias)) return NSFF_ERR_NULL;
+    unsigned long long total = 0;
+    size_t lds = 0;
+    auto add = [&](int kind, int index, unsigned long long blocks) {
+        p.kind[p.n_jobs] = kind;
+        p.index[p.n_jobs] = index;
+        p.first_block[p.n_jobs++] = (unsigned)total;
+        total += blocks;
+    };
+    if (k) k->coarse.job = -1;
+    if (s.ray) {
+        const NsffFineArgs f = fine_args(*s.ray);
+        size_t need = 0;
+        const int rc = nsff_fine_args_check(f, &need);
+        if (rc) return rc;
+        if (f.n_rays > 0) {
+            add(NSFF_STAGE_RAY, 0, (unsigned long long)f.n_rays);
+            lds = std::max(lds, need);
+            if (k) k->ray = f;
+        }
+    }
+    const long long gx = (s.time_bias_rays + NSFF_TB_RAYS - 1) / NSFF_TB_RAYS;
+    for (int q = 0; q < s.n_time_bias; ++q) {
+        NsffTimeBiasJobK jk{};
+        const int rc = nsff_time_bias_prepare(s.time_bias[q], jk);
+        if (rc) return rc;
+        if (gx == 0) continue;
+        add(NSFF_STAGE_TIME_BIAS, q, (unsigned long long)gx * jk.rows);
+        lds = std::max(lds, tb_lds(p.n_jobs > 0 && p.kind[0] == NSFF_STAGE_RAY));
+        if (k) k->tb[q] = jk;
+    }
+    unsigned rng_blocks = 0;
+    const int rc = nsff_rng_check(s.rng, s.n_rng, s.coarse, &rng_blocks);
+    if (rc) return rc;
+    for (int j = 0; j < s.n_rng; ++j) {
+        add(NSFF_STAGE_RNG, j, s.rng[j].grid);
+        if (k) k->rng[j] = s.rng[j];
+    }
+    if (total > 0x7fffffffULL || gx > 0x7fffffffLL) return NSFF_ERR_INVALID;
+    p.first_block[p.n_jobs] = p.n_blocks = (unsigned)total;
+    p.lds_bytes = (uint32_t)lds;
+    if (k) {
+        if (s.coarse) k->coarse = *s.coarse;
+        for (int e = 0; e <= p.n_jobs; ++e) k->first_block[e] = p.first_block[e];
+        for (int e = 0; e < p.n_jobs; ++e) { k->kind[e] = (signed char)p.kind[e]; k->index[e] = (signed char)p.index[e]; }
+        k->n = p.n_jobs;
+        k->tb_gx = (unsigned)std::max(gx, 1LL);
+        k->tb_rays = s.time_bias_rays;
+        k->seed = s.seed;
+    }
+    return NSFF_OK;
+}
+
+}
+
+extern "C" int nsff_stage_plan(const NsffStageArgs* args, NsffStagePlan* plan) {
+    if (!args || !plan) return NSFF_ERR_NULL;
+    return make_plan(*args, *plan, nullptr);
+}
+
+extern "C" int nsff_stage_launch(const NsffStageArgs* args, void* stream) {
+    if (!args) return NSFF_ERR_NULL;
+    NsffStagePlan p;
+    StageArgs k{};
+    const int rc = make_plan(*args, p, &k);
+    if (rc) return rc;
+    if (p.n_blocks == 0) return NSFF_OK;
+    if (p.kind[0] == NSFF_STAGE_RAY)
+        hipLaunchKernelGGL(nsff_stage_kernel_ray, dim3(p.n_blocks), dim3(256), p.lds_bytes, (hipStream_t)stream, k);
+    else
+        hipLaunchKernelGGL(nsff_stage_kernel, dim3(p.n_blocks), dim3(256), p.lds_bytes, (hipStream_t)stream, k);
+    return nsff_launch_status();
+}
diff --git a/nsff_pl_amd/rendering.py b/nsff_pl_amd/rendering.py
--- a/nsff_pl_amd/rendering.py
+++ b/nsff_pl_amd/rendering.py
@@ -33,49 +33,63 @@
 _TORCH_RAND, _TORCH_RANDN = torch.rand, torch.randn
 
 
+def _draw_plan(n_rays, N_samples, N_importance, perturb, noise_std, test_time, transient, flows, hooked=True):
+    noisy = float(noise_std) != 0
+    plan, need = [], []
+
+    def add(kind, need_values, *shape):
+        plan.append((kind, shape))
+        need.append(bool(need_values))
+    if perturb > 0:
+        add("rand", not hooked, n_rays, N_samples)
+    S = N_samples
+    if N_importance > 0:
+        add("randn", noisy, n_rays, S)
+        if transient:
+            add("randn", noisy, n_rays, S)
+        if perturb != 0:
+            add("rand", True, n_rays, N_importance)
+            if transient:
+                add("rand", True, n_rays, N_importance)
+        S = N_samples + (2 if transient else 1) * N_importance
+    n_head = len(plan) if N_importance > 0 else None
+    add("randn", noisy, n_rays, S)
+    if transient:
+        add("randn", noisy, n_rays, S)
+        if flows and not test_time:
+            add("randn", noisy, n_rays, S)
+            add("randn", noisy, n_rays, S)
+    return plan, need, len(plan) if n_head is None else n_head
+
+
 class _Draws:
 
-    def __init__(self, device, n_rays, N_samples, N_importance, perturb, noise_std, test_time, models, kwargs, coarse=None):
+    def __init__(self, device, n_rays, N_samples, N_importance, perturb, noise_std, test_time, models, kwargs, coarse=None,
+                 defer=False):
         self.device = device
         self.coarse_done = False
         self.fused = (device.type == "cuda" and torch.rand is _TORCH_RAND and torch.randn is _TORCH_RANDN
                       and not os.environ.get("NSFF_TORCH_RNG") and not torch.cuda.is_current_stream_capturing()
                       and _lib.fused_draws_match_torch(device))
         self.at = 0
+        self.pending, self.head = None, None
         if not self.fused:
             return
         first = models["coarse"] if N_importance > 0 else models["fine"]
         transient = bool(kwargs.get("output_transient", True) and first.encode_transient)
         flows = kwargs.get("output_transient_flow", []) if transient else []
-        noisy = float(noise_std) != 0
-        plan, need = [], []
-
-        def add(kind, need_values, *shape):
-            plan.append((kind, shape))
-            need.append(bool(need_values))
+        plan, need, n_head = _draw_plan(n_rays, N_samples, N_importance, perturb, noise_std, test_time, transient, bool(flows),
+                                        hooked=coarse is not None)
         hook = None
-        if perturb > 0:
-            add("rand", coarse is None, n_rays, N_samples)
-            if coarse is not None and n_rays:
-                hook = (coarse[0], coarse[1], float(perturb), coarse[2], coarse[3])
-        S = N_samples
-        if N_importance > 0:
-            add("randn", noisy, n_rays, S)
-            if transient:
-                add("randn", noisy, n_rays, S)
-            if perturb != 0:
-                add("rand", True, n_rays, N_importance)
-                if transient:
-                    add("rand", True, n_rays, N_importance)
-            S = N_samples + (2 if transient else 1) * N_importance
-        add("randn", noisy, n_rays, S)
-        if transient:
-            add("randn", noisy, n_rays, S)
-            if flows and not test_time:
-                add("randn", noisy, n_rays, S)
-                add("randn", noisy, n_rays, S)
+        if perturb > 0 and coarse is not None and n_rays:
+            hook = (coarse[0], coarse[1], float(perturb), coarse[2], coarse[3])
         self.plan = plan
-        self.values = _lib.fused_draws(plan, device, need, coarse=hook)
+        if defer:
+            self.pending = _lib.fused_draws(plan, device, need, coarse=hook, launch=False)
+            self.values = self.pending.outs
+            self.head = set(range(n_head))
+        else:
+            self.values = _lib.fused_draws(plan, device, need, coarse=hook)
         self.coarse_done = hook is not None
 
     def take(self, kind, *shape):
@@ -89,7 +103,7 @@
 
 class _Pass:
     __slots__ = ("embeddings", "rays", "ts", "max_t", "noise_std", "test_time", "kwargs",
-                 "freqs_xyz", "dir_embedded", "n_rays", "rec", "tbias", "neighbour_rows", "draws")
+                 "freqs_xyz", "dir_embedded", "n_rays", "rec", "tbias", "neighbour_rows", "draws", "stage_tb")
 
 
 def _embed_rows(embeddings, key, idx):
@@ -117,8 +131,15 @@
             _embed_rows(embeddings, 't', torch.clamp(ts - 1, min=0)))
 
 
-def _time_codes(ctx, models, kwargs, N_samples, N_importance, output_transient, flows):
-    ctx.tbias, ctx.neighbour_rows = {}, None
+def _time_bias_head(passes):
+    return [q for q, typ in enumerate(passes) if typ == passes[0]]
+
+
+def _time_codes(ctx, models, kwargs, N_samples, N_importance, output_transient, flows, defer=False):
+    ctx.tbias, ctx.neighbour_rows, ctx.stage_tb = {}, None, None
+
+    def deferred(handle):
+        ctx.stage_tb = (handle, _time_bias_head([typ for typ, _, _, _ in plan]))
     if not output_transient:
         return None
     n_rays, ts, m = ctx.n_rays, ctx.ts, ctx.embeddings.get('t')
@@ -141,7 +162,10 @@
              and ts.dim() == 1 and ts.shape[0] == n_rays)
     if (plan and plain and all(mod.in_channels_t == m.weight.shape[1] for _, _, mod, _ in plan)
             and not os.environ.get('NSFF_NO_TIME_INDEX')):
-        outs, rows = _lib.time_bias([(mod, d) for _, _, mod, d in plan], index=(m.weight.detach(), ts.contiguous(), ctx.max_t))
+        outs, rows, *handle = _lib.time_bias([(mod, d) for _, _, mod, d in plan], index=(m.weight.detach(), ts.contiguous(), ctx.max_t),
+                                             launch=not defer)
+        if defer:
+            deferred(handle[0])
         for (typ, which, _, _), out in zip(plan, outs):
             ctx.tbias[(typ, which)] = out
         if 1 in rows:
@@ -154,9 +178,28 @@
         if any(w == 'fw' for _, w, _, _ in plan):
             ctx.neighbour_rows = _neighbour_time_rows(ctx.embeddings, ts, ctx.max_t)
         src = {0: t_embedded, 1: ctx.neighbour_rows[0] if ctx.neighbour_rows else None, -1: ctx.neighbour_rows[1] if ctx.neighbour_rows else None}
-        for (typ, which, _, _), out in zip(plan, _lib.time_bias([(mod, src[d]) for _, _, mod, d in plan])):
+        outs = _lib.time_bias([(mod, src[d]) for _, _, mod, d in plan], launch=not defer)
+        if defer:
+            outs, handle = outs
+            deferred(handle)
+        for (typ, which, _, _), out in zip(plan, outs):
             ctx.tbias[(typ, which)] = out
     return t_embedded
+
+
+def _stage_head(ctx):
+    draws, tb = ctx.draws.pending, ctx.stage_tb
+    _lib.stage_launch(draws=draws, which=ctx.draws.head if draws is not None else None,
+                      tb=tb[0] if tb else None, tb_which=tb[1] if tb else None)
+
+
+def _stage_mid(ctx, ray):
+    draws, tb = ctx.draws.pending, ctx.stage_tb
+    rest = None
+    if draws is not None:
+        rest = set(draws.draw) - ctx.draws.head
+    later = [q for q in range(len(tb[0][0])) if q not in tb[1]] if tb else []
+    _lib.stage_launch(draws=draws if rest else None, which=rest, tb=tb[0] if later else None, tb_which=later, ray=ray)
 
 
 def _inference(results, ctx, model, xyz, zs, output_transient, output_transient_flow,
@@ -339,7 +382,7 @@
         ctx.noise_std, ctx.test_time, ctx.kwargs, ctx.n_rays = noise_std, test_time, kwargs, n_rays
         ctx.freqs_xyz = [float(f) for f in embedding_xyz.freqs]
         ctx.rec = rec
-        ctx.tbias, ctx.neighbour_rows = {}, None
+        ctx.tbias, ctx.neighbour_rows, ctx.stage_tb = {}, None, None
         ctx.dir_embedded = None
         if any(m.use_viewdir for m in models.values()):
             view_dir = kwargs.get('view_dir', rays[:, 3:6])
@@ -348,8 +391,9 @@
         z_lin = _unit_linspace(N_samples, rays.device)
         zs = _new(rays, n_rays, N_samples)
         xyz_coarse = _new(rays, n_rays, N_samples, 3)
+        stage = rec is None and n_rays > 0 and not os.environ.get('NSFF_NO_STAGE_LAUNCH')
         ctx.draws = _Draws(rays.device, n_rays, N_samples, N_importance, perturb, noise_std, test_time, models, kwargs,
-                           coarse=(rays, z_lin, zs, xyz_coarse))
+                           coarse=(rays, z_lin, zs, xyz_coarse), defer=stage)
         perturb_rand = ctx.draws.take("rand", n_rays, N_samples) if perturb > 0 else None
         if n_rays and not ctx.draws.coarse_done:
             _lib.coarse_samples(rays, z_lin, perturb, perturb_rand, zs, xyz_coarse)
@@ -359,7 +403,9 @@
             model = models['coarse']
             output_transient = bool(kwargs.get('output_transient', True) and model.encode_transient)
             t_embedded = _time_codes(ctx, models, kwargs, N_samples, N_importance, output_transient,
-                                     kwargs.get('output_transient_flow', []))
+                                     kwargs.get('output_transient_flow', []), defer=stage)
+            if stage:
+                _stage_head(ctx)
             _inference(results, ctx, model, xyz_coarse, zs, output_transient, [], t_embedded, None)
 
             det = perturb == 0
@@ -375,11 +421,15 @@
             zs_fine = _new(rays, n_rays, S_fine)
             xyz_fine = _new(rays, n_rays, S_fine, 3)
             if n_rays:
-                _lib.fine_samples(rays, z_lin, zs, N_importance,
-                                  results['static_weights_coarse'],
-                                  results['transient_weights_coarse'] if output_transient else None,
-                                  u_s, u_t if output_transient else None, 0 if det else 1,
-                                  zs_static, zs_transient, zs_fine, xyz_fine)
+                ray = (rays, z_lin, zs, N_importance,
+                       results['static_weights_coarse'],
+                       results['transient_weights_coarse'] if output_transient else None,
+                       u_s, u_t if output_transient else None, 0 if det else 1,
+                       zs_static, zs_transient, zs_fine, xyz_fine)
+                if stage:
+                    _stage_mid(ctx, ray)
+                else:
+                    _lib.fine_samples(*ray)
             if test_time:
                 results['static_zs_fine'] = zs_static
                 if output_transient:
@@ -399,7 +449,10 @@
             a_embedded = a_embedded.detach().contiguous().float()
         if N_importance == 0:
             output_transient = bool(kwargs.get('output_transient', True) and model.encode_transient)
-            t_embedded = _time_codes(ctx, models, kwargs, N_samples, 0, output_transient, kwargs.get('output_transient_flow', []))
+            t_embedded = _time_codes(ctx, models, kwargs, N_samples, 0, output_transient, kwargs.get('output_transient_flow', []),
+                                     defer=stage)
+            if stage:
+                _stage_head(ctx)
         output_transient_flow = [] if not output_transient else kwargs.get('output_transient_flow', [])
         _inference(results, ctx, model, xyz, zs, output_transient, output_transient_flow,
                    t_embedded, a_embedded)
```

Result: no change. 71.84 million ray-samples/s (-0.0%).
